# n00b001/neuro-genetic-pong-self-play

Measured on AMD Instinct MI355X. Metric: env-steps/sec (GA evaluation loop, self-play) + generations/sec at pop=65536 per GPU, higher is better.
Workload: dtype f32 hidden + certified f64 argmax; genomes f64

## Files before the change

include/pong_ga.h:

```cpp
#ifndef PONG_GA_H
#define PONG_GA_H

#include <stddef.h>
#include <stdint.h>

#ifdef __cplusplus
extern "C" {
#endif

#define PG_ABI_VERSION 12
#define PG_MAX_NODES 9

typedef enum pg_status {
  PG_OK = 0,
  PG_ERR_INVALID = -1,
  PG_ERR_HIP = -2,
  PG_ERR_UNSUPPORTED = -3
} pg_status;

typedef enum pg_dtype { PG_F32 = 0, PG_F64 = 1 } pg_dtype;

typedef enum pg_opp_kind {
  PG_OPP_HARDCODED = 0,
  PG_OPP_ROM_CPU = 1,
  PG_OPP_SCORE = 2,
  PG_OPP_NN = 3
} pg_opp_kind;

typedef enum pg_precision {
  PG_PREC_CERTIFIED = 0,
  PG_PREC_F64 = 1
} pg_precision;

typedef enum pg_kernel {
  PG_KERNEL_AUTO = 0,
  PG_KERNEL_GENERAL = 1,
  PG_KERNEL_RESIDENT = 2,
  PG_KERNEL_SPLIT = 3      ,
  PG_KERNEL_WIDE = 4,
  PG_KERNEL_STAGED = 5
} pg_kernel;

typedef enum pg_prep {
  PG_PREP_ALL = 0,
  PG_PREP_GENOMES = 1,
  PG_PREP_REST = 2
} pg_prep;

typedef struct pg_net {
  int32_t n_nodes;
  int32_t nodes[PG_MAX_NODES];
  int32_t bias;
  int32_t dtype;
} pg_net;

typedef struct pg_eval_args {
  uint32_t struct_size;
  pg_net net;
  int32_t n_genomes;
  int32_t n_games;
  const void *genomes;
  int64_t genome_stride;
  const void *opponents;
  int64_t opponent_stride;
  int32_t n_opponents;
  int32_t precision;
  const int32_t *game_kind;
  const int32_t *game_opp;
  const double *game_mult;
  uint64_t seed;
  double *fitness;
  double *rewards;
  int32_t *scores;
  int32_t *frames;
  double *total_frames;
  int32_t *status;
  uint64_t *counters;
  uint8_t *trace;
  int32_t trace_games;
  int32_t trace_cap;
  int32_t kernel;
  int32_t group_lanes;
  void *workspace;
  size_t workspace_bytes;
  uint32_t *hard_log;
  int32_t hard_cap;
  const int32_t *genome_rows;
  const int32_t *n_active;
  int32_t prep;
  int32_t horizon;
  int32_t timeout_thresh;
  int32_t win_score;
} pg_eval_args;


typedef struct pg_forward_args {
  pg_net net;
  int32_t n;
  const void *genomes;
  int64_t genome_stride;
  const int32_t *genome_index;
  const double *x;
  int32_t precision;
  int32_t *index;
  double *act;
  uint64_t *counters;
  double *z_all;
  double *h_all;
} pg_forward_args;

typedef struct pg_decide_args {
  pg_net net;
  int32_t n;
  const void *genomes;
  int64_t genome_stride;
  const int32_t *genome_index;
  const int32_t *k;
  int32_t *index;
  int32_t *stage;
} pg_decide_args;

typedef struct pg_wide_decide_args {
  pg_net net;
  int32_t n;
  const void *genomes;
  int64_t genome_stride;
  const int32_t *genome_index;
  const int32_t *k;
  int32_t *index;
  double *act;
  void *workspace;
  size_t workspace_bytes;
} pg_wide_decide_args;

enum {
  PG_S_BALL_X = 0, PG_S_BALL_Y, PG_S_BALL_VX, PG_S_BALL_VY, PG_S_BALL_VISIBLE,
  PG_S_SERVE_TIMER, PG_S_SERVE_DIR, PG_S_HITS, PG_S_POINT, PG_S_LEFT_Y, PG_S_RIGHT_Y,
  PG_S_SCORE1, PG_S_SCORE2, PG_S_ONE_PLAYER, PG_S_SEED_LO, PG_S_SEED_HI,
  PG_STATE_FIELDS
};

typedef struct pg_ga_args {
  int32_t n;
  int64_t genes;
  int32_t dtype;
  const void *parents;
  int64_t stride;
  int32_t n_parents;
  const int32_t *chosen;
  void *offspring;
  uint8_t *invalid;
  double cxpb, mutpb;
  double alpha;
  double mu, sigma, indpb;
  uint64_t seed;
  uint64_t generation;
  const uint8_t *pair_mask;
  const int32_t *pair_list;
  const int32_t *pair_count;
  int32_t pair_cap;
} pg_ga_args;

typedef struct pg_select_args {
  int32_t n_pop;
  int32_t k;
  int32_t tournsize;
  const double *fitness;
  int32_t *chosen;
  uint64_t seed;
  uint64_t generation;
} pg_select_args;

typedef enum pg_schedule_mode {
  PG_SCHED_REFERENCE = 0,
  PG_SCHED_SELFPLAY = 1
} pg_schedule_mode;

typedef struct pg_schedule_args {
  int32_t mode;
  int32_t n;
  int32_t n_games;
  int64_t row_offset;
  int32_t n_hof;
  const double *hof_fitness;
  uint64_t seed;
  uint64_t generation;
  int32_t *kind;
  int32_t *opp;
  double *mult;
  const int32_t *rows;
  int32_t hof_slices;
  int32_t block_rows;
  int32_t slice_local;
} pg_schedule_args;

typedef struct pg_hof_args {
  int32_t maxsize;
  int32_t hof_n;
  const double *hof_fitness;
  const uint64_t *hof_hash;
  int32_t pop_n;
  const double *pop_fitness;
  const uint64_t *pop_hash;
  const int32_t *rank;
  int32_t *new_n;
  int32_t *new_src;
  double *new_fitness;
} pg_hof_args;

typedef struct pg_hof_packed_args {
  int32_t maxsize;
  int32_t hof_n;
  const double *hof_fitness;
  int32_t k;
  const int64_t *packed;
  int32_t *new_n;
  int32_t *new_src;
  double *new_fitness;
  const int32_t *slot_in;
  int32_t *slot_out;
} pg_hof_packed_args;
int32_t pg_hof_update_packed(const pg_hof_packed_args *args);

typedef struct pg_hof_rank_args {
  int32_t hof_n;
  const double *hof_fitness;
  const uint64_t *hof_hash;
  int32_t k;
  const double *cand_fitness;
  const uint64_t *cand_hash;
  int64_t *packed;
  void *workspace;
  size_t workspace_bytes;
} pg_hof_rank_args;

typedef struct pg_hof_prepare_args {
  const double *fitness;
  int32_t pop_n;
  int32_t filter;
  double worst;
  const void *rows;
  int64_t stride;
  int64_t genes;
  int32_t dtype;
  int32_t hof_n;
  const double *hof_fitness;
  const uint64_t *hof_hash;
  int32_t *k;
  int64_t *cand;
  uint64_t *hashes;
  int64_t *packed;
  void *workspace;
  size_t workspace_bytes;
} pg_hof_prepare_args;

const char *pg_version(void);
int32_t pg_abi_version(void);
int32_t pg_build_flags(void);
const char *pg_last_error(void);
int32_t pg_device_count(void);
size_t pg_eval_workspace_bytes(const pg_eval_args *args);
int32_t pg_gene_count(const pg_net *net);

int32_t pg_eval_population(const pg_eval_args *args, void *stream);
int32_t pg_forward(const pg_forward_args *args, void *stream);
int32_t pg_decide(const pg_decide_args *args, void *stream);
size_t pg_wide_decide_workspace_bytes(const pg_wide_decide_args *args);
int32_t pg_wide_decide(const pg_wide_decide_args *args, void *stream);
int32_t pg_physics_reset(int32_t *state, int32_t n, const uint64_t *seeds,
                         const int32_t *one_player, void *stream);
int32_t pg_physics_step(int32_t *state, int32_t n, const uint8_t *actions, void *stream);
int32_t pg_ga_select_tournament(const pg_select_args *args, void *stream);
int32_t pg_ga_select_tournament_ranked(const pg_select_args *args, const double *sorted_fitness,
                                       const int32_t *order, void *stream);
int32_t pg_ga_vary(const pg_ga_args *args, void *stream);
int32_t pg_ga_mark_pairs(uint8_t *pair_mask, int32_t n_pairs, const int32_t *rows, int32_t n_rows,
                         int32_t skip_lo, int32_t skip_hi, const uint8_t *exclude, void *stream);
int32_t pg_ga_list_pairs(const uint8_t *pair_mask, int32_t n_pairs, int32_t *list, int32_t *count, void *stream);
int32_t pg_ga_schedule(const pg_schedule_args *args, void *stream);
int32_t pg_row_hash(const void *rows, int64_t stride, const int32_t *index, int32_t n, int64_t genes,
                    int32_t dtype, uint64_t *hash, void *stream);
int32_t pg_hof_update(const pg_hof_args *args);
size_t pg_hof_rank_classes_workspace_bytes(int32_t n);
int32_t pg_hof_rank_classes(const pg_hof_rank_args *args, void *stream);
size_t pg_hof_prepare_workspace_bytes(int32_t hof_n, int32_t pop_n);
int32_t pg_hof_prepare(const pg_hof_prepare_args *args, void *stream);

typedef struct pg_scatter_args {
  int32_t n;
  int32_t n_games;
  int32_t row_lo;
  const double *fitness;
  const int32_t *frames;
  const int32_t *rows;
  const int32_t *n_active;
  double *shard_fitness;
  float *lineage;
} pg_scatter_args;
int32_t pg_ga_scatter_fitness(const pg_scatter_args *args, void *stream);

typedef struct pg_merge_args {
  int32_t pop_n;
  const double *fitness;
  const uint8_t *invalid;
  const double *inherited;
  double *new_fitness;
  int32_t filter;
  double worst;
  int32_t *cand;
  double *cand_fitness;
  double *summary;
  void *workspace;
  size_t workspace_bytes;
} pg_merge_args;
size_t pg_ga_merge_workspace_bytes(int32_t pop_n);
int32_t pg_ga_merge_fitness(const pg_merge_args *args, void *stream);

size_t pg_ga_select_workspace_bytes(int32_t n_pop);
int32_t pg_ga_select_ranked(const pg_select_args *args, void *workspace, size_t workspace_bytes, void *stream);

int32_t pg_ga_inherit(const int32_t *chosen, int32_t n, const double *fitness, double *inherited,
                      const float *lineage_in, float *lineage_out, void *stream);

size_t pg_ga_order_workspace_bytes(int32_t n);
int32_t pg_ga_order(int32_t n, int32_t row_lo, const uint8_t *invalid, const float *lineage, int32_t by_length,
                    int32_t *rows, int32_t *count, void *workspace, size_t workspace_bytes, void *stream);

typedef struct pg_hof_cand_args {
  int32_t hof_n;
  const double *hof_fitness;
  const uint64_t *hof_hash;
  int32_t k;
  const int32_t *cand;
  const double *cand_fitness;
  const void *rows;
  int64_t stride;
  int64_t genes;
  int32_t dtype;
  uint64_t *cand_hash;
  int64_t *packed;
  void *workspace;
  size_t workspace_bytes;
} pg_hof_cand_args;
size_t pg_hof_prepare_cand_workspace_bytes(int32_t hof_n, int32_t k);
int32_t pg_hof_prepare_cand(const pg_hof_cand_args *args, void *stream);

typedef struct pg_hof_commit_args {
  void *dst;
  int64_t dst_stride;
  const void *old_rows;
  int64_t old_stride;
  const void *rows;
  int64_t rows_stride;
  const int32_t *cand;
  const int32_t *src;
  int32_t n_old;
  int32_t m;
  int64_t genes;
  int32_t dtype;
  const uint64_t *old_hash;
  const uint64_t *cand_hash;
  uint64_t *new_hash;
  const double *fitness_in;
  double *new_fitness;
  const int32_t *dst_slot;
} pg_hof_commit_args;
int32_t pg_hof_commit(const pg_hof_commit_args *args, void *stream);

int32_t pg_gather_rows(void *dst, int64_t dst_stride, const void *old_rows, int64_t old_stride, const void *rows,
                       int64_t rows_stride, const int64_t *index, const int32_t *src, int32_t n_old, int32_t n,
                       int64_t genes, int32_t dtype, void *stream);
int32_t pg_render_frames(const int32_t *state, int32_t n, uint8_t *frames, void *stream);
int32_t pg_find_stuff(const uint8_t *frames, int64_t frame_stride, int32_t n, double *out, void *stream);

#ifdef __cplusplus
}
#endif
#endif
```

neuro-genetic-pong-self-play_amd/csrc/pg_eval.hpp:

```cpp
#pragma once

#include <hip/hip_runtime.h>
#include <stdint.h>

#include "../../include/pong_ga.h"
#include "pg_device.hpp"

namespace pg {

int32_t fail(int32_t code, const char *fmt, ...);

#define PG_HIP(call)                                                                  \
  do {                                                                                \
    hipError_t e_ = (call);                                                           \
    if (e_ != hipSuccess)                                                             \
      return fail(PG_ERR_HIP, "%s failed: %s", #call, hipGetErrorString(e_));        \
  } while (0)

struct EvalParams {
  const void *genomes;
  const void *opponents;
  const int32_t *rows;
  const int32_t *n_active;
  const int32_t *kind;
  const int32_t *opp;
  const double *mult;
  double *rewards;
  int32_t *scores;
  int32_t *frames;
  double *total_frames;
  int32_t *status_game;
  uint64_t *counters;
  uint8_t *trace;
  uint32_t *hard_log;
  int hard_cap;
  unsigned int *work;
  int64_t gstride, ostride;
  uint64_t seed;
  int n_genomes, n_games, total, n_opponents;
  int trace_games, trace_cap;
  int nodes[PG_MAX_NODES];
  int n_nodes, bias, max_width;
  float *recs;
  int horizon;
  int timeout_thresh;
  int win_score;
  int prep;
  void *wide_scratch;
  int wide_w3_resident;
  const int32_t *wide_probe_k;
  int32_t *wide_probe_index;
  double *wide_probe_act;
};

__device__ inline int active_genomes(const EvalParams &p) {
  if (!p.n_active) return p.n_genomes;
  const int a = __builtin_amdgcn_readfirstlane(*p.n_active);
  return a < 0 ? 0 : (a < p.n_genomes ? a : p.n_genomes);
}
__device__ inline int active_total(const EvalParams &p) {
  return p.n_active ? active_genomes(p) * p.n_games : p.total;
}

__device__ inline int genome_row(const EvalParams &p, int i) { return p.rows ? p.rows[i] : i; }

template <class S>
__device__ inline double episode_reward(const S &st, int total, double mult, int &zero_div) {
  zero_div = 0;
  if (st.s1 == st.s2) return 0.0;
  const double tf = (double)total;
  if (tf == 0.0) {
    zero_div = 1;
    return __builtin_nan("");
  }
  const double diff = (double)(st.s2 - st.s1);
  const double bonus = __dmul_rn((double)st.s2, mult);
  return __dadd_rn(diff, bonus) / (tf / 100.0);
}

template <class S>
__device__ inline void finish_game(const EvalParams &p, int w, const S &st, int frames, int total) {
  int zero_div;
  const double reward = episode_reward(st, total, p.mult[w], zero_div);
  p.rewards[w] = reward;
  p.scores[2 * w] = st.s1;
  p.scores[2 * w + 1] = st.s2;
  p.frames[w] = frames;
  p.total_frames[w] = (double)total;
  p.status_game[w] = zero_div;
}

__device__ inline double feat64(int k) { return __dmul_rn(0.5, (double)k) / 160.0; }
__device__ inline double feat64_flip(int k) { return (160.0 - __dmul_rn(0.5, (double)k)) / 160.0; }


int num_cus();

__device__ inline void log_hard_raw(uint32_t *hard_log, uint64_t *counters, int hard_cap, int row, int is_opp, int idx,
                                    int source, const int k[6]) {
  if (!hard_log || !counters) return;
  const unsigned long long r = atomicAdd((unsigned long long *)&counters[9], 1ull);
  if (r >= (unsigned long long)hard_cap) return;
  uint32_t *rec = hard_log + r * 8;
  rec[0] = (uint32_t)row;
  rec[1] = (uint32_t)(is_opp & 1) | ((uint32_t)(idx & 255) << 8) | ((uint32_t)(source & 255) << 16);
  for (int i = 0; i < 6; ++i) rec[2 + i] = (uint32_t)k[i];
}
__device__ inline void log_hard(const EvalParams &p, int row, int is_opp, int idx, int source, const int k[6]) {
  log_hard_raw(p.hard_log, p.counters, p.hard_cap, row, is_opp, idx, source, k);
}

struct DecideParams {
  const void *genomes;
  const int32_t *gidx;
  const int32_t *k;
  int32_t *index;
  int32_t *stage;
  int64_t gstride;
  int n, H, b;
};
int32_t launch_decide(const DecideParams &p, int L, int O, bool f64, size_t lds, hipStream_t s);

bool wide_shape_ok(const pg_net &n, int n_games);
size_t wide_workspace_bytes(const pg_eval_args *a);
int32_t launch_wide(const EvalParams &p, int dtype, void *scratch, hipStream_t s);


}
```

neuro-genetic-pong-self-play_amd/csrc/pg_service.hpp:

```cpp
#pragma once

#include <hip/hip_runtime.h>

#include "../../include/pong_ga.h"
#include "pg_cascade.hpp"
#include "pg_device.hpp"
#include "pg_eval.hpp"
#include "pg_f64math.h"

namespace pg {

#ifndef PG_SVC_PRIO
#define PG_SVC_PRIO 3
#endif
#ifndef PG_SVC_BATCH
#define PG_SVC_BATCH 1
#endif

#ifndef PG_INLINE_SVC
#define PG_INLINE_SVC 1
#endif
#ifndef PG_INLINE_PRIO
#define PG_INLINE_PRIO 3
#endif
#ifndef PG_INLINE_FRAME_BOUND
#define PG_INLINE_FRAME_BOUND 1
#endif
#ifndef PG_HORIZON_INLINE
#define PG_HORIZON_INLINE 1
#endif
template <int L, int U, bool kHorizon>
__host__ __device__ constexpr bool inline_service() {
  return PG_INLINE_SVC && L == 8 && U == 16 && (PG_HORIZON_INLINE || !kHorizon);
}

struct InlineReq {
  int k[6];
  int kr[6];
  float z[4];
  float e;
  const float *rec;
};
template <int U, int HL, int O, typename WT>
__device__ __forceinline__ int serve_inline(const EvalParams &p, const WT *g, InlineReq r, double *lds,
                                                      int lane64, uint64_t *st_acc = nullptr) {
  const int H = p.nodes[1];
  const int b = p.bias;
  float zf[O];
#pragma unroll
  for (int o = 0; o < O; ++o) zf[o] = r.z[o];
#ifdef PG_INLINE_LOG
  float ef_log = -1.f;
  const auto log_req = [&](int stage, int idx) {
    if (p.hard_log && p.counters && lane64 == 0) {
      const unsigned long long q = atomicAdd((unsigned long long *)&p.counters[9], 1ull);
      if (q < (unsigned long long)p.hard_cap) {
        uint32_t *rec = p.hard_log + q * 8;
        for (int o = 0; o < 4; ++o) rec[o] = __float_as_uint(o < O ? zf[o] : 0.f);
        rec[4] = __float_as_uint(r.e);
        rec[5] = __float_as_uint(ef_log);
        rec[6] = (uint32_t)stage | ((uint32_t)(idx & 255) << 8) |
                 ((uint32_t)(blockIdx.x * (blockDim.x >> 6) + (threadIdx.x >> 6)) << 16);
        rec[7] = (uint32_t)((uint64_t)g >> 3);
      }
    }
  };
#define PG_LOG_REQ(stage, idx) log_req(stage, idx)
#else
#define PG_LOG_REQ(stage, idx)
#endif
#ifdef PG_SERVE_STAGES
  asm volatile("s_waitcnt vmcnt(0) lgkmcnt(0)" ::: "memory");
  uint64_t st_t = __builtin_amdgcn_s_memtime();
  const auto stage_mark = [&](int i) {
    asm volatile("s_waitcnt vmcnt(0) lgkmcnt(0)" ::: "memory");
    const uint64_t now = __builtin_amdgcn_s_memtime();
    st_acc[i] += now - st_t;
    st_acc[6 + i] += 1;
    st_t = now;
  };
#define PG_STAGE(i) stage_mark(i)
#else
#define PG_STAGE(i)
#endif
  int d = PG_INLINE_FRAME_BOUND ? -1 : plateau_decide<O>(zf, r.e, lane64);
  PG_STAGE(0);
  if (d >= 0) PG_LOG_REQ(1, d);
  if (PG_INLINE_FRAME_BOUND && d < 0 && r.e < __builtin_inff()) {
    const float ef = fminf(r.e, frame_bound_wave<HL, U, O>(r.rec, r.kr, lane64));
#ifdef PG_INLINE_LOG
    ef_log = ef;
#endif
    PG_STAGE(1);
    d = certify_c<O>(zf, make_cert(ef));
    if (d < 0) d = plateau_f32<O>(zf, ef);
    if (d < 0) d = plateau_decide<O>(zf, ef, lane64);
    PG_STAGE(2);
    if (d >= 0) {
      PG_LOG_REQ(2, d);
      return d | 1024;
    }
  }
  if (d < 0) {
    d = fast_f64_decide<O, WT>(g, H, b, r.k, lane64);
    PG_STAGE(3);
    if (d >= 0) PG_LOG_REQ(3, d);
  }
  if (d >= 0) return d | 512;
  d = forward_f64_group<64, (U * HL + 63) / 64, O, WT>(g, H, b, r.k, lds, lane64);
  PG_LOG_REQ(4, d);
  PG_STAGE(4);
#undef PG_LOG_REQ
#undef PG_STAGE
#if defined(PG_INLINE_LOG) || defined(PG_SERVE_STAGES)
  if (false) {
#else
  if (p.hard_log && lane64 == 0) {
#endif
    const long oo = g - (const WT *)p.opponents;
    const bool opp = p.opponents != p.genomes && oo >= 0 && oo < (long)p.n_opponents * p.ostride;
    log_hard(p, (int)(opp ? oo / p.ostride : (g - (const WT *)p.genomes) / p.gstride), opp ? 1 : 0, d, 0, r.k);
  }
  return d | 256;
}

template <int L, int U, int O, typename WT>
__global__ __launch_bounds__(256) void k_prep_records(EvalParams p) {
  constexpr int HL = L / 2;
  constexpr int F = rec_floats<U, O>();
  if (p.prep != PG_PREP_GENOMES && blockIdx.x == 0) {
    if (threadIdx.x < 64) p.work[threadIdx.x] = 0u;
    if (p.counters && threadIdx.x < 16) p.counters[threadIdx.x] = 0ull;
  }
  const long t = (long)blockIdx.x * 256 + threadIdx.x;
  const long net = t / HL + (p.prep == PG_PREP_REST ? p.n_genomes : 0);
  const int hl = (int)(t % HL);
  const long end = p.prep == PG_PREP_GENOMES ? (long)p.n_genomes : (long)p.n_genomes + p.n_opponents;
  if (net >= end) return;
  const WT *g;
  int flip;
  if (net < p.n_genomes) {
    if (net >= active_genomes(p)) return;
    g = (const WT *)p.genomes + (long)genome_row(p, (int)net) * p.gstride;
    flip = 0;
  } else {
    g = (const WT *)p.opponents + (net - p.n_genomes) * p.ostride;
    flip = 1;
  }
  NetP<U, O> n;
  load_net_pk<HL, U, O, WT>(n, g, p.nodes[1], p.bias, hl, flip);
  store_rec<U, O>(n, p.recs + (net * HL + hl) * F);
}

#ifdef PG_PROBE_EXTRA
template <int M>
__device__ __forceinline__ void pg_probe_extra(float2v w, float2v w2, float a, float b, float &v, float2v &pp,
                                               int &sv) {
#pragma unroll
  for (int r = 0; r < (M == 4 || M == 9 ? 48 : (M <= 2 ? 16 : 24)); ++r) {
    if constexpr (M == 1) asm volatile("v_rcp_f32 %0, %1" : "=v"(v) : "v"((r & 1) ? a : b));
    if constexpr (M == 2) asm volatile("v_exp_f32 %0, %1" : "=v"(v) : "v"((r & 1) ? a : b));
    if constexpr (M == 3) asm volatile("v_pk_fma_f32 %0, %1, %2, %3" : "=v"(pp) : "v"(w), "v"(w2), "v"((r & 1) ? w : w2));
    if constexpr (M == 4) asm volatile("v_fma_f32 %0, %1, %2, %3" : "=v"(v) : "v"(a), "v"(b), "v"((r & 1) ? a : b));
    if constexpr (M == 5) asm volatile("v_add_u32 %0, %1, %2" : "=v"(v) : "v"(a), "v"(b));
    if constexpr (M == 7) asm volatile("v_mov_b32 %0, %1" : "=v"(v) : "v"((r & 1) ? a : b));
    if constexpr (M == 8) asm volatile("v_pk_add_f32 %0, %1, %2" : "=v"(pp) : "v"(w), "v"((r & 1) ? w : w2));
    if constexpr (M == 9) asm volatile("v_add_f32 %0, %1, %2" : "=v"(v) : "v"(a), "v"((r & 1) ? a : b));
  }
}
#endif

template <int L, int U, int O, typename WT, bool kUntraced = false, bool kHorizon = false>
__global__ __launch_bounds__(svc_threads<U>()) void k_service(EvalParams p) {
  constexpr int kSvcThreads = svc_threads<U>();
  constexpr bool kInline = inline_service<L, U, kHorizon>();
  static_assert(!kInline || O <= 4, "InlineReq.z");
  constexpr int kSvcGameWaves = kSvcThreads / 64 - (kInline ? 0 : 1);
  constexpr int HL = L / 2;
  constexpr int kSlots = kSvcGameWaves * (64 / L) * 2;
  __shared__ SlowSlot slots[kSlots];
  __shared__ HorizonSlot hz[kHorizon ? kSlots / 2 : 1];
  __shared__ int waves_done;
  __shared__ int posted;
  __shared__ uint32_t serve_tab[kServeTabSlots * kServeTabPoints];
  extern __shared__ double lds_svc[];
  const int H = p.nodes[1];
  const int b = p.bias;
  const int wave = threadIdx.x >> 6;
  const int lane64 = threadIdx.x & 63;
  for (int i = threadIdx.x; i < kSlots; i += kSvcThreads) {
    lds_st(&slots[i].flag, 0);
    slots[i].rec = 0;
  }
  const bool tabbed = p.n_games <= kServeTabSlots;
  if (tabbed)
    for (int i = threadIdx.x; i < p.n_games * kServeTabPoints; i += kSvcThreads)
      serve_tab[i] = Pong::serve_entry(game_seed(p.seed, i / kServeTabPoints), i % kServeTabPoints);
  if (threadIdx.x == 0) {
    lds_st(&waves_done, 0);
    lds_st(&posted, 0);
  }
  __syncthreads();

  if (!kInline && wave == kSvcGameWaves) {
    if constexpr (PG_SVC_PRIO > 0) __builtin_amdgcn_s_setprio(PG_SVC_PRIO);
    constexpr int kSvcBatch = U * HL <= 64 ? PG_SVC_BATCH : 1;
    const WT *genomes_svc = (const WT *)p.genomes;
    int seen = 0;
    for (;;) {
      const int now = __builtin_amdgcn_readfirstlane(lds_ld(&posted));
      if (now == seen) {
        if (lds_ld(&waves_done) == kSvcGameWaves) break;
        __builtin_amdgcn_s_sleep(2);
        continue;
      }
      seen = now;
      for (int base = 0; base < kSlots; base += 64) {
        const int sidx = base + lane64;
        const bool posted = sidx < kSlots && lds_ld(&slots[sidx].flag) == 1;
        unsigned long long mask = __ballot(posted);
        while (mask) {
          int sl[kSvcBatch], idx[kSvcBatch], k[kSvcBatch][6];
          const WT *g[kSvcBatch];
          bool need[kSvcBatch];
#pragma unroll
          for (int q = 0; q < kSvcBatch; ++q) {
            sl[q] = -1;
            if (mask) {
              sl[q] = base + __builtin_ctzll(mask);
              mask &= mask - 1;
            }
          }
          __threadfence_block();
#pragma unroll
          for (int q = 0; q < kSvcBatch; ++q) {
            need[q] = false;
            idx[q] = -1;
            g[q] = genomes_svc;
            if (sl[q] >= 0) {
              g[q] = (const WT *)slots[sl[q]].g;
#pragma unroll
              for (int i = 0; i < 6; ++i) k[q][i] = slots[sl[q]].k[i];
              float zf[O];
#pragma unroll
              for (int o = 0; o < O; ++o) zf[o] = slots[sl[q]].z[o];
              idx[q] = plateau_decide<O>(zf, slots[sl[q]].e, lane64);
              need[q] = idx[q] < 0;
            }
          }
          if constexpr (kSvcBatch > 1) {
            int f[kSvcBatch];
            fast_f64_decide_batch<O, WT, kSvcBatch>(g, k, need, H, b, lane64, f);
#pragma unroll
            for (int q = 0; q < kSvcBatch; ++q)
              if (need[q]) idx[q] = f[q];
          } else {
            if (need[0]) idx[0] = fast_f64_decide<O, WT>(g[0], H, b, k[0], lane64);
          }
#pragma unroll
          for (int q = 0; q < kSvcBatch; ++q) {
            if (sl[q] < 0) continue;
            int d = idx[q];
            if (d < 0) {
              d = forward_f64_group<64, (U * HL + 63) / 64, O, WT>(g[q], H, b, k[q], lds_svc, lane64);
              if (p.hard_log && lane64 == 0) {
                const long oo = g[q] - (const WT *)p.opponents;
                const bool opp = p.opponents != p.genomes && oo >= 0 && oo < (long)p.n_opponents * p.ostride;
                log_hard(p, (int)(opp ? oo / p.ostride : (g[q] - (const WT *)p.genomes) / p.gstride), opp ? 1 : 0,
                         d, 0, k[q]);
              }
              d |= 256;
            } else {
              d |= 512;
            }
            if (lane64 == 0) {
              slots[sl[q]].idx = d;
              __threadfence_block();
              lds_st(&slots[sl[q]].flag, 2);
            }
          }
        }
      }
    }
    return;
  }

  const int lig = threadIdx.x & (L - 1);
  const int side = lig >= HL ? 1 : 0;
  const int hl = lig & (HL - 1);
  const int leader = lane64 & ~(L - 1);
  const int wave_slot0 = __builtin_amdgcn_readfirstlane((int)(threadIdx.x >> 6)) * (64 / L) * 2;
  const auto slot_grp = [&]() { return wave_slot0 + (fresh_lane64() / L) * 2; };
  const auto slot_me = [&]() {
    const int l = fresh_lane64();
    return wave_slot0 + (l / L) * 2 + ((l & (L - 1)) >= HL ? 1 : 0);
  };
  const WT *genomes = (const WT *)p.genomes;
  const WT *opponents = (const WT *)p.opponents;

  NetP<U, O> net;
  PongK st;
  int kind = 0, act_r = 0, act_l = 0, total = 0, fstart = 0, tend = 0, c_vis = 0, tab_off = 0;
  int sframe = 0;
#ifndef PG_NO_HIDDEN_JUMP
  constexpr bool kVisByFrames = kUntraced && !kHorizon;
#else
  constexpr bool kVisByFrames = false;
#endif
  const WT *gm = genomes;
  uint32_t slow = 0, c_fwd = 0, c_steps = 0, c_games = 0, fails = 0, plateau = 0, inwave = 0, skipped = 0, hidden = 0;

  const int games_total = active_total(p);
  int w;
  {
    int ww = 0;
    if (lig == 0) ww = (int)atomicAdd(p.work, 1u);
    w = group_broadcast<L>(ww, leader);
  }
  bool fresh = true;
  bool live = w < games_total;
  const auto park = [&]() {
    st.bx2 = 2 * 79 + kBallW - 1;
    st.by2 = 2 * 78 + kBallH - 1;
    st.vx2 = st.vy2 = 0;
    st.vis = 2;
    st.one_player = 0;
    kind = kOppNN;
    tend = 0x7fffffff;
    fstart = 0x3fffffff;
    fresh = false;
  };
  if (kInline && !live) park();
  int w_scripted = 1, w_onep = 1;
  int top = 1;
#ifdef PG_PROBE_EXTRA
  float probe_v = 0.f;
  float2v probe_p = float2v{0.f, 0.f};
  int probe_s = 0;
#endif
#ifdef PG_START_PROBE
  uint64_t probe_fresh = 0;
  const uint64_t probe_t0 = __builtin_amdgcn_s_memtime();
#endif
#ifdef PG_SERVE_STAGES
  uint64_t st_acc[24];
#pragma unroll
  for (int i = 0; i < 24; ++i) st_acc[i] = 0;
#endif
#ifdef PG_DECIDE_PROBE
  uint64_t probe_dec = 0;
  const uint64_t probe_t0 = __builtin_amdgcn_s_memtime();
#endif
#ifdef PG_TIMELINE
  uint64_t t_start = 0;
  uint32_t g_fails = 0, g_slow = 0;
#endif
#ifdef PG_PATH_PROBE
  uint32_t pp_frames = 0, pp_rally = 0, pp_face = 0, pp_fail = 0, pp_hidden = 0;
#define PG_PP(cnt, cond) \
  if (__builtin_amdgcn_ballot_w64(cond) != 0) cnt += 1
#else
#define PG_PP(cnt, cond)
#endif
  if (kInline ? __builtin_amdgcn_ballot_w64(live) != 0 : live) for (;;) {
#ifdef PG_START_PROBE
    const bool any_fresh = __builtin_amdgcn_ballot_w64(fresh) != 0;
    const uint64_t probe_f0 = __builtin_amdgcn_s_memtime();
#endif
    PG_PP(pp_frames, true);
    sframe += 1;
#ifdef PG_TIMELINE
    constexpr bool kJumps = !kHorizon;
#else
    const bool kJumps = !kHorizon && (kUntraced || p.trace == nullptr);
#endif
    if (top) {
    if (fresh) {
      const int i = w / p.n_games;
      const int g = w - i * p.n_games;
      kind = p.kind[w];
      const WT *gr = genomes + (long)genome_row(p, i) * p.gstride;
      const bool nn = side && kind == kOppNN && p.n_opponents > 0;
      const int oj = nn ? min(max(p.opp[w], 0), p.n_opponents - 1) : 0;
      gm = nn ? opponents + (long)oj * p.ostride : gr;
      const int rec = nn ? p.n_genomes + oj : i;
      load_rec<U, O>(net, p.recs + ((long)rec * HL + hl) * rec_floats<U, O>());
      const int sx = slot_me();
      if (kInline && hl == 0) slots[sx].rec = rec;
#pragma unroll
      for (int o = 0; o < O; ++o) net.c[o] = hl == 0 ? 0.5f * net.c[o] : 0.f;
      st.reset(0, kind == kOppRomCpu);
      if (kHorizon || !tabbed) st.seed = game_seed(p.seed, g);
      tab_off = g * kServeTabPoints;
      act_r = act_l = total = 0;
      c_vis = kVisByFrames ? sframe - 1 : 0;
      fstart = sframe - 1;
      tend = sframe + p.timeout_thresh;
      fresh = false;
      if (hl == 0) slots[sx].n_memo = 0;
      if (lig == 0) slots[sx].rally_at = -1;
      if (kHorizon && lig == 0) {
        const int gx = threadIdx.x / L;
        hz[gx].sum = 0.0;
        hz[gx].eps = hz[gx].s1 = hz[gx].s2 = hz[gx].zd = 0;
      }
#ifdef PG_TIMELINE
      t_start = wall_clock64();
      g_fails = g_slow = 0;
#endif
    }
#ifdef PG_START_PROBE
    if (any_fresh) probe_fresh += __builtin_amdgcn_s_memtime() - probe_f0;
#endif
#ifndef PG_NO_HIDDEN_JUMP
    {
      const bool hid = !st.vis && st.timer >= 2;
      PG_PP(pp_hidden, hid);
      if (kJumps && hid) {
        const int h = st.timer - 1;
        st.rc2 = PongK::drift2(st.rc2, h);
        if (!st.one_player) st.lc2 = PongK::drift2(st.lc2, h);
        st.timer = 1;
        act_r = clamp_move(st.rc2, 0);
        act_l = clamp_move(st.lc2, 0);
        fstart -= h;
        tend -= h;
        hidden += h;
      }
    }
#endif
    w_scripted = __builtin_amdgcn_readfirstlane(__builtin_amdgcn_ballot_w64(kind != kOppNN) != 0);
    w_onep = __builtin_amdgcn_readfirstlane(__builtin_amdgcn_ballot_w64(st.one_player != 0) != 0);
    top = 0;
    }
    const int pvis = st.vis, pbx2 = st.bx2, pby2 = st.by2;
#ifdef PG_PATH_PROBE
    const int pt_b = st.point, hits_b = st.hits;
#endif
    const int ev = st.step(act_r, act_l, [&](int pt) {
      return tabbed && pt < kServeTabPoints ? serve_tab[tab_off + pt] : Pong::serve_entry(st.seed, pt);
    }, w_onep != 0);
    PG_PP(pp_face, ev != kStepFly || st.hits != hits_b || st.point != pt_b);
    const int vis = st.vis;
    const int bx2 = st.bx2, by2 = st.by2;
    const int rc2 = st.rc2;
    int lc2 = st.lc2;
    if (__builtin_expect(w_onep, 0)) lc2 = PongK::c2_clip(st.lc2);
    int left, right;
    {
      const int lbx2 = pvis ? pbx2 : bx2, lby2 = pvis ? pby2 : by2;
      const int k[6] = {bx2, by2, lbx2, lby2, rc2, lc2};
      float acc[O], z[O];
      partial_pk<U, O, true>(net, k, acc);
#pragma unroll
      for (int o = 0; o < O; ++o) z[o] = group_sum<HL>(acc[o]);
      int code = certify_c8<O>(z, net.ct);
#ifdef PG_PROBE_EXTRA
      pg_probe_extra<PG_PROBE_EXTRA>(net.w1[0][0], net.w1[1][1], z[0], z[1], probe_v, probe_p, probe_s);
#endif
      const bool left_nn = kind == kOppNN;
      if (side && !left_nn) code = 0;
      if (vis != 1) code = 0;
#ifdef PG_ABLATE_SLOW
      if (code == -1) code = z[1] > z[0] ? 6 : -6;
#endif
      PG_PP(pp_fail, code == -1);
      if (PG_ANY(code == -1)) {
      if (code == -1) {
        fails += 1;
#ifdef PG_TIMELINE
        g_fails += 1;
#endif
#ifndef PG_NO_TIGHT
        int mv = tight_gap_move<O>(z, net.e, net.ct);
        if (mv == -1)
#else
        int mv = -1;
#endif
        {
          const int idx = plateau_f32<O>(z, net.e);
          mv = idx >= 0 ? index_to_move(idx) : -1;
        }
        inwave += mv != -1 ? 1 : 0;
        code = mv;
      }
#ifdef PG_ABLATE_SERVE
      if (code == -1) code = z[1] > z[0] ? 6 : -6;
#endif
      if (kInline && PG_ANY(code == -1)) {
        uint64_t key = 0;
        int nm = 0;
        const int sx = slot_me();
        if (code == -1) {
          key = memo_key(k);
          nm = slots[sx].n_memo;
          int hit = -1;
#pragma unroll 1
          for (int c = 0; c < kMemo && c < nm; ++c)
            if (slots[sx].memo_key[c] == key) hit = slots[sx].memo_idx[c];
          code = hit;
        }
        const int kn[6] = {side ? 320 - bx2 : bx2, by2, side ? 320 - lbx2 : lbx2, lby2, side ? lc2 : rc2,
                           side ? rc2 : lc2};
        const float my_e = net.e;
        uint64_t need = __builtin_amdgcn_ballot_w64(code == -1 && hl == 0);
        if (need) {
#ifdef PG_DECIDE_PROBE
        const uint64_t probe_d0 = __builtin_amdgcn_s_memtime();
#endif
        if constexpr (PG_INLINE_PRIO > 0) __builtin_amdgcn_s_setprio(PG_INLINE_PRIO);
#pragma unroll 1
        do {
          const int src = (int)__builtin_ctzll(need);
          need &= need - 1;
          InlineReq r;
#pragma unroll
          for (int i = 0; i < 6; ++i) r.k[i] = __builtin_amdgcn_readlane(kn[i], src);
#pragma unroll
          for (int i = 0; i < 6; ++i) r.kr[i] = __builtin_amdgcn_readlane(k[i], src);
          r.rec = p.recs + (long)__builtin_amdgcn_readlane(slots[sx].rec, src) * HL * rec_floats<U, O>();
#pragma unroll
          for (int o = O; o < 4; ++o) r.z[o] = 0.f;
#pragma unroll
          for (int o = 0; o < O; ++o) r.z[o] = __int_as_float(__builtin_amdgcn_readlane(__float_as_int(z[o]), src));
          r.e = __int_as_float(__builtin_amdgcn_readlane(__float_as_int(my_e), src));
          const uint64_t ga = (uint64_t)gm;
          const WT *g = (const WT *)(((uint64_t)__builtin_amdgcn_readlane((int)(ga >> 32), src) << 32) |
                                     (uint32_t)__builtin_amdgcn_readlane((int)(uint32_t)ga, src));
#if defined(PG_SERVE_TWICE)
          serve_inline<U, HL, O, WT>(p, g, r, lds_svc + wave * f64_lds_doubles(H, O), lane64, st_acc);
          const int ans = serve_inline<U, HL, O, WT>(p, g, r, lds_svc + wave * f64_lds_doubles(H, O), lane64, st_acc + 12);
#elif defined(PG_SERVE_STAGES)
          const int ans = serve_inline<U, HL, O, WT>(p, g, r, lds_svc + wave * f64_lds_doubles(H, O), lane64, st_acc);
#else
          const int ans = serve_inline<U, HL, O, WT>(p, g, r, lds_svc + wave * f64_lds_doubles(H, O), lane64);
#endif
          if ((lane64 & ~(HL - 1)) == src) {
            slow += (ans >> 8) & 1;
// ... 146 lines not shown
    over = over || sframe > tend;
#endif
    if constexpr (kHorizon) {
      if (over) {
        const int gx = threadIdx.x / L;
        const bool ep_end = st.s1 >= p.win_score || st.s2 >= p.win_score || st.done() || sframe > tend;
        if (lig == 0) {
          if (ep_end) {
            int zd;
            hz[gx].sum = __dadd_rn(hz[gx].sum, episode_reward(st, total, p.mult[w], zd));
            hz[gx].zd |= zd;
            hz[gx].eps += 1;
          }
          hz[gx].s1 += st.s1;
          hz[gx].s2 += st.s2;
        }
        if (ep_end && sframe - fstart < p.horizon) {
          const int pt = st.point;
          st.reset(st.seed, st.one_player);
          st.point = pt;
          act_r = act_l = total = 0;
          tend = sframe + 1 + p.timeout_thresh;
          over = false;
        }
      }
    }
    if (over) {
      if constexpr (kHorizon) {
        if (lig == 0) {
          const int gx = threadIdx.x / L;
          p.rewards[w] = hz[gx].sum;
          p.scores[2 * w] = hz[gx].s1;
          p.scores[2 * w + 1] = hz[gx].s2;
          p.frames[w] = sframe - fstart;
          p.total_frames[w] = (double)hz[gx].eps;
          p.status_game[w] = hz[gx].zd;
        }
      } else {
        if (lig == 0) finish_game(p, w, st, sframe - fstart, total);
      }
#ifdef PG_TIMELINE
      if (p.trace && w < p.trace_games && lig == 0) {
        uint32_t *tl = (uint32_t *)(p.trace + (long)w * p.trace_cap);
        tl[0] = (uint32_t)t_start;
        tl[1] = (uint32_t)wall_clock64();
        tl[2] = g_fails;
        tl[3] = g_slow;
        if (p.trace_cap >= 24) {
          tl[4] = blockIdx.x;
          tl[5] = (uint32_t)wave;
        }
      }
#endif
      c_steps += sframe - fstart;
      const int vis_frames = kVisByFrames ? sframe - c_vis - (st.s1 + st.s2) : c_vis;
      c_fwd += (kind == kOppNN ? 2u : 1u) * (uint32_t)vis_frames;
      c_games += 1;
      int ww = 0;
      if (lig == 0) ww = (int)atomicAdd(p.work, 1u);
      w = group_broadcast<L>(ww, leader);
      if constexpr (kInline) {
        if (w >= games_total) {
          live = false;
          park();
        } else {
          fresh = true;
        }
      } else {
        if (w >= games_total) break;
        fresh = true;
      }
    }
    if constexpr (kInline) {
      if (__builtin_amdgcn_ballot_w64(live) == 0) break;
    }
    top = __builtin_amdgcn_readfirstlane(__builtin_amdgcn_ballot_w64(fresh || (kJumps && !st.vis && st.timer >= 2)) != 0);
    }
  }
  if (p.counters && c_games) {
    if (lig == 0) {
      atomicAdd((unsigned long long *)&p.counters[0], (unsigned long long)(c_steps - skipped - hidden));
      if (hidden) atomicAdd((unsigned long long *)&p.counters[12], (unsigned long long)hidden);
      atomicAdd((unsigned long long *)&p.counters[1], (unsigned long long)c_fwd);
      atomicAdd((unsigned long long *)&p.counters[3], (unsigned long long)c_games);
      if (skipped) atomicAdd((unsigned long long *)&p.counters[8], (unsigned long long)skipped);
    }
    if (hl == 0 && slow) atomicAdd((unsigned long long *)&p.counters[2], (unsigned long long)slow);
    if (hl == 0 && fails) atomicAdd((unsigned long long *)&p.counters[4], (unsigned long long)fails);
    if (hl == 0 && plateau) atomicAdd((unsigned long long *)&p.counters[5], (unsigned long long)plateau);
    if (hl == 0 && inwave) atomicAdd((unsigned long long *)&p.counters[6], (unsigned long long)inwave);
  }
#ifdef PG_DECIDE_PROBE
  if (p.counters && lane64 == 0) {
    atomicAdd((unsigned long long *)&p.counters[13], (unsigned long long)probe_dec);
    atomicAdd((unsigned long long *)&p.counters[14], (unsigned long long)(__builtin_amdgcn_s_memtime() - probe_t0));
    atomicAdd((unsigned long long *)&p.counters[15], 1ull);
  }
#endif
#ifdef PG_START_PROBE
  if (p.counters && lane64 == 0) {
    atomicAdd((unsigned long long *)&p.counters[13], (unsigned long long)probe_fresh);
    atomicAdd((unsigned long long *)&p.counters[14], (unsigned long long)(__builtin_amdgcn_s_memtime() - probe_t0));
    atomicAdd((unsigned long long *)&p.counters[15], 1ull);
  }
#endif
#ifdef PG_PATH_PROBE
  if (p.counters && lane64 == 0) {
    atomicAdd((unsigned long long *)&p.counters[11], (unsigned long long)pp_frames);
    atomicAdd((unsigned long long *)&p.counters[10], (unsigned long long)pp_rally);
    atomicAdd((unsigned long long *)&p.counters[13], (unsigned long long)pp_face);
    atomicAdd((unsigned long long *)&p.counters[14], (unsigned long long)pp_fail);
    atomicAdd((unsigned long long *)&p.counters[15], (unsigned long long)pp_hidden);
  }
#endif
#ifdef PG_PROBE_EXTRA
  if (p.counters && probe_v == 1234.5f && probe_p.x == 1234.5f && probe_s == 1234567) p.counters[15] = 1;
#endif
#ifdef PG_SERVE_STAGES
  if (p.hard_log && lane64 == 0)
#pragma unroll
    for (int i = 0; i < 24; ++i)
      if (st_acc[i]) atomicAdd((unsigned long long *)&((uint64_t *)p.hard_log)[i], (unsigned long long)st_acc[i]);
#endif
  if (lane64 == 0) atomicAdd(&waves_done, 1);
}

inline size_t service_records_bytes(int n_genomes, int n_opponents, int L, int U, int O) {
  const int F = ((U + 1) / 2 * 2 * (7 + O) + O + 1 + 3) / 4 * 4;
  return ((size_t)n_genomes + (size_t)(n_opponents > 0 ? n_opponents : 0)) * (size_t)(L / 2) * F * sizeof(float);
}

template <int L, int U, int O, typename WT, bool kSplitTrace = false>
inline int32_t launch_service(const EvalParams &p, hipStream_t s) {
  constexpr int kSvcThreads = svc_threads<U>();
  const bool inl = p.horizon > 0 ? inline_service<L, U, true>() : inline_service<L, U, false>();
  const int GPB = (kSvcThreads / 64 - (inl ? 0 : 1)) * (64 / L);
  const size_t lds = (size_t)f64_lds_doubles(p.nodes[1], O) * sizeof(double) * (inl ? kSvcThreads / 64 : 1);
  const int want = (p.total + GPB - 1) / GPB;
  const int cap = num_cus() * 2;
  const int grid = want < cap ? want : cap;
  if (grid <= 0) return PG_OK;
  if (!p.recs) return fail(PG_ERR_INVALID, "split kernel: no lane-record workspace");
  if (!kSplitTrace && p.horizon > 0)
    return fail(PG_ERR_UNSUPPORTED, "horizon mode: [6, 33..64, 3] networks on 8-lane groups only");
  const long nets = p.prep == PG_PREP_GENOMES ? (long)p.n_genomes
                   : (p.prep == PG_PREP_REST ? (long)p.n_opponents : (long)p.n_genomes + p.n_opponents);
  const long prep_threads = nets * (L / 2);
  const unsigned prep_blocks = (unsigned)((prep_threads + 255) / 256);
  hipLaunchKernelGGL((k_prep_records<L, U, O, WT>), dim3(prep_blocks > 0 ? prep_blocks : 1u), dim3(256), 0, s, p);
  if (p.prep == PG_PREP_GENOMES) {
    PG_HIP(hipGetLastError());
    return PG_OK;
  }
  if (kSplitTrace && p.horizon > 0)
    hipLaunchKernelGGL((k_service<L, U, O, WT, true, true>), dim3(grid), dim3(kSvcThreads), lds, s, p);
  else if (kSplitTrace && !p.trace)
    hipLaunchKernelGGL((k_service<L, U, O, WT, true>), dim3(grid), dim3(kSvcThreads), lds, s, p);
  else
    hipLaunchKernelGGL((k_service<L, U, O, WT, false>), dim3(grid), dim3(kSvcThreads), lds, s, p);
  PG_HIP(hipGetLastError());
  return PG_OK;
}

int32_t launch_service_more(const EvalParams &p, int L, int O, bool f64, hipStream_t s);

inline int service_units(int L, int H) {
  if (L == 8 && H > 32 && H <= 64) return 16;
  for (int u = 1; u <= 8; u *= 2)
    if ((L / 2) * u >= H) return u;
  return 0;
}

}
```

neuro-genetic-pong-self-play_amd/csrc/pong_ga.hip:

```cpp
#include <hip/hip_runtime.h>

#include <cmath>
#include <cstdarg>
#include <cstdio>
#include <cstring>
#include <string>
#include <algorithm>
#include <memory>
#include <unordered_map>
#include <utility>
#include <vector>

#include "../../include/pong_ga.h"
#include "pg_device.hpp"
#include "pg_eval.hpp"
#include "pg_f64math.h"
#include "pg_cascade.hpp"
#include "pg_service.hpp"

#ifndef PG_VERSION_STRING
#define PG_VERSION_STRING "pong_ga 0.1.0 (gfx950)"
#endif

namespace pg {
// ... 159 lines not shown
template <typename WT>
__global__ __launch_bounds__(64) void k_forward_general(FwdParams p) {
  extern __shared__ double lds[];
  const int lane = threadIdx.x;
  const int W = p.max_width + 1;
  const int n_in = p.nodes[0], n_out = p.nodes[p.n_nodes - 1];
  for (int t = blockIdx.x; t < p.n; t += gridDim.x) {
    const long row = p.gidx ? p.gidx[t] : t;
    const WT *gw = (const WT *)p.genomes + row * p.gstride;
    double *cur = lds, *nxt = lds + W;
    for (int i = lane; i < n_in; i += 64) cur[i] = p.x[(long)t * n_in + i];
    if (p.bias && lane == 0) cur[n_in] = 1.0;
    wave_lds_sync();
    const int idx = forward_f64_wave(gw, p.nodes, p.n_nodes, p.bias, cur, nxt, lane,
                                     p.z_all ? p.z_all + (long)t * p.n_units : nullptr,
                                     p.h_all ? p.h_all + (long)t * p.n_units : nullptr);
    if (lane == 0) p.index[t] = idx;
    if (p.act)
      for (int j = lane; j < n_out; j += 64) p.act[(long)t * n_out + j] = cur[j];
    wave_lds_sync();
  }
}

template <int L, int U, int O, typename WT>
__global__ __launch_bounds__(256) void k_forward_resident(FwdParams p) {
  constexpr int GPB = 256 / L;
  const int H = p.nodes[1], b = p.bias;
  extern __shared__ double lds_all[];
  const int lig = threadIdx.x & (L - 1);
  const int grp = threadIdx.x / L;
  double *lds = lds_all + grp * f64_lds_doubles(H, O);
  uint32_t slow = 0;
  for (int t = blockIdx.x * GPB + grp; t < p.n; t += gridDim.x * GPB) {
    const long row = p.gidx ? p.gidx[t] : t;
    const WT *gw = (const WT *)p.genomes + row * p.gstride;
    Net<U, O> net;
    load_net<L, U, O, WT>(net, gw, H, b, lig);
    float x[6], acc[O], z[O];
#pragma unroll
    for (int i = 0; i < 6; ++i) x[i] = (float)p.x[(long)t * 6 + i];
    partial_f32<U, O>(net, x, acc);
#pragma unroll
    for (int o = 0; o < O; ++o) z[o] = group_sum<L>(acc[o]) + net.c[o];
    int idx = certify<O>(z, net.e);
    if (idx >= 0 && p.act) {
      bool tight = true;
#pragma unroll
      for (int o = 0; o < O; ++o) {
        const float tt = fmaxf(fabsf(z[o]) - net.e, 0.f);
        const float sp = __expf(-tt) / ((1.f + __expf(-tt)) * (1.f + __expf(-tt)));
        tight = tight && (net.e * sp <= 2e-6f);
      }
      if (!tight) idx = -1;
    }
    if (idx < 0) {
      double xd[6];
#pragma unroll
      for (int i = 0; i < 6; ++i) xd[i] = p.x[(long)t * 6 + i];
      idx = forward_f64_group<L, U, O, WT>(gw, H, b, (const double *)xd, lds, lig);
      if (p.act && lig < O) p.act[(long)t * O + lig] = lds[f64_out_offset(H, O) + lig];
      wave_lds_sync();
      slow += (lig == 0);
    } else if (p.act && lig < O) {
      float zz = z[0];
#pragma unroll
      for (int o = 1; o < O; ++o) zz = (lig == o) ? z[o] : zz;
      p.act[(long)t * O + lig] = sigmoid_f64((double)zz);
    }
    if (lig == 0) p.index[t] = idx;
  }
  if (p.counters && slow) atomicAdd((unsigned long long *)&p.counters[2], (unsigned long long)slow);
}

__global__ void k_physics_reset(int32_t *s, int n, const uint64_t *seeds, const int32_t *one_player) {
  const int i = blockIdx.x * blockDim.x + threadIdx.x;
  if (i >= n) return;
  Pong st;
  st.reset(seeds ? seeds[i] : 0ull, one_player ? one_player[i] : 0);
  const int f[PG_STATE_FIELDS] = {st.bx, st.by, st.vx, st.vy, st.vis, st.timer, st.dir, st.hits,
                                  st.point, st.lpy, st.rpy, st.s1, st.s2, st.one_player,
                                  (int)(uint32_t)st.seed, (int)(uint32_t)(st.seed >> 32)};
#pragma unroll
  for (int k = 0; k < PG_STATE_FIELDS; ++k) s[(long)k * n + i] = f[k];
}

__global__ void k_physics_step(int32_t *s, int n, const uint8_t *actions) {
  const int i = blockIdx.x * blockDim.x + threadIdx.x;
  if (i >= n) return;
  Pong st;
  st.bx = s[0L * n + i]; st.by = s[1L * n + i]; st.vx = s[2L * n + i]; st.vy = s[3L * n + i];
  st.vis = s[4L * n + i]; st.timer = s[5L * n + i]; st.dir = s[6L * n + i]; st.hits = s[7L * n + i];
  st.point = s[8L * n + i]; st.lpy = s[9L * n + i]; st.rpy = s[10L * n + i];
  st.s1 = s[11L * n + i]; st.s2 = s[12L * n + i]; st.one_player = s[13L * n + i];
  st.seed = (uint64_t)(uint32_t)s[14L * n + i] | ((uint64_t)(uint32_t)s[15L * n + i] << 32);
  const int a = actions[i];
  st.step(a & 3, (a >> 2) & 3);
  s[0L * n + i] = st.bx; s[1L * n + i] = st.by; s[2L * n + i] = st.vx; s[3L * n + i] = st.vy;
  s[4L * n + i] = st.vis; s[5L * n + i] = st.timer; s[6L * n + i] = st.dir; s[7L * n + i] = st.hits;
  s[8L * n + i] = st.point; s[9L * n + i] = st.lpy; s[10L * n + i] = st.rpy;
  s[11L * n + i] = st.s1; s[12L * n + i] = st.s2;
}

__device__ __forceinline__ double u01(uint64_t seed, uint64_t gen, uint64_t stream, uint64_t a,
                                      uint64_t b) {
  uint64_t k = splitmix64(seed + 0x9E3779B97F4A7C15ull * (gen + 1));
  k = splitmix64(k ^ (stream * 0xD6E8FEB86659FD93ull + a));
  k = splitmix64(k ^ b);
  return (double)(k >> 11) * 0x1.0p-53;
}

__global__ void k_select(pg_select_args a) {
  const int j = blockIdx.x * blockDim.x + threadIdx.x;
  if (j >= a.k) return;
  int best = -1;
  double bf = 0.0;
  for (int t = 0; t < a.tournsize; ++t) {
    const int idx = (int)(u01(a.seed, a.generation, 1, (uint64_t)j, (uint64_t)t) * (double)a.n_pop);
    const double f = a.fitness[idx];
    if (best < 0 || f > bf) {
      best = idx;
      bf = f;
    }
  }
  a.chosen[j] = best;
}

__global__ void k_select_ranked(pg_select_args a, const double *sorted, const int32_t *order) {
  const int j = blockIdx.x * blockDim.x + threadIdx.x;
  if (j >= a.k) return;
  const int n = a.n_pop;
  const double v = u01(a.seed, a.generation, 8, (uint64_t)j, 0);
  int r = (int)((double)n * exp(log(v) / (double)a.tournsize));
  r = r < 0 ? 0 : (r > n - 1 ? n - 1 : r);
  const double f = sorted[r];
  int lo = 0, hi = n;
  int a0 = 0, b0 = r;
  while (a0 < b0) { const int m = (a0 + b0) >> 1; if (sorted[m] < f) a0 = m + 1; else b0 = m; }
  lo = a0;
  a0 = r; b0 = n;
  while (a0 < b0) { const int m = (a0 + b0) >> 1; if (sorted[m] <= f) a0 = m + 1; else b0 = m; }
  hi = a0;
  const int pick = lo + (int)(u01(a.seed, a.generation, 9, (uint64_t)j, 0) * (double)(hi - lo));
  a.chosen[j] = order[pick < hi ? pick : hi - 1];
}

__device__ __forceinline__ uint64_t rng_key(uint64_t seed, uint64_t gen, uint64_t stream, uint64_t a) {
  const uint64_t k = splitmix64(seed + 0x9E3779B97F4A7C15ull * (gen + 1));
  return splitmix64(k ^ (stream * 0xD6E8FEB86659FD93ull + a));
}
__device__ __forceinline__ double rng_u01(uint64_t key, uint64_t b) {
  return (double)(splitmix64(key ^ b) >> 11) * 0x1.0p-53;
}

template <typename WT>
__device__ __forceinline__ void vary_pair(const pg_ga_args &a, int pair);

template <typename WT>
__global__ __launch_bounds__(256) void k_vary(pg_ga_args a) {
  const int wave = (int)blockIdx.x * 4 + __builtin_amdgcn_readfirstlane((int)(threadIdx.x >> 6));
  if (a.pair_list) {
    const int count = __builtin_amdgcn_readfirstlane(*a.pair_count);
    const int waves = (int)gridDim.x * 4;
#pragma unroll 1
    for (int w = wave; w < count; w += waves) vary_pair<WT>(a, __builtin_amdgcn_readfirstlane(a.pair_list[w]));
    return;
  }
  vary_pair<WT>(a, wave);
}

template <typename WT>
__device__ __forceinline__ void vary_pair(const pg_ga_args &a, int pair) {
  const int pairs = (a.n + 1) / 2;
  if (pair >= pairs) return;
  const int lane = threadIdx.x & 63;
  const int i0 = 2 * pair, i1 = 2 * pair + 1;
  const bool has1 = i1 < a.n;
  const bool cx = has1 && rng_u01(rng_key(a.seed, a.generation, 2, (uint64_t)pair), 0) < a.cxpb;
  const bool mut0 = rng_u01(rng_key(a.seed, a.generation, 4, (uint64_t)i0), 0) < a.mutpb;
  const bool mut1 = has1 && rng_u01(rng_key(a.seed, a.generation, 4, (uint64_t)i1), 0) < a.mutpb;
  if (lane == 0) {
    a.invalid[i0] = (uint8_t)(cx || mut0);
    if (has1) a.invalid[i1] = (uint8_t)(cx || mut1);
  }
  if (!a.pair_list && a.pair_mask && !a.pair_mask[pair]) return;
  const uint64_t k3 = rng_key(a.seed, a.generation, 3, (uint64_t)pair);
  const uint64_t k5 = rng_key(a.seed, a.generation, 5, (uint64_t)pair);
  const uint64_t k6 = rng_key(a.seed, a.generation, 6, (uint64_t)pair);
  const WT *p1 = (const WT *)a.parents + (long)a.chosen[i0] * a.stride;
  const WT *p2 = (const WT *)a.parents + (long)(has1 ? a.chosen[i1] : a.chosen[i0]) * a.stride;
  WT *o1 = (WT *)a.offspring + (long)i0 * a.stride;
  WT *o2 = (WT *)a.offspring + (long)i1 * a.stride;
  const auto one = [&](long gene, double x1, double x2) {
    if (cx) {
      const double u = rng_u01(k3, (uint64_t)gene);
      const double gamma = __dadd_rn(__dmul_rn(1.0 + 2.0 * a.alpha, u), -a.alpha);
      const double y1 = __dadd_rn(__dmul_rn(1.0 - gamma, x1), __dmul_rn(gamma, x2));
      const double y2 = __dadd_rn(__dmul_rn(gamma, x1), __dmul_rn(1.0 - gamma, x2));
      x1 = y1;
      x2 = y2;
    }
    const uint64_t hb = splitmix64(k5 ^ (uint64_t)gene);
    const bool h0 = mut0 && (double)(uint32_t)hb * 0x1.0p-32 < a.indpb;
    const bool h1 = mut1 && (double)(uint32_t)(hb >> 32) * 0x1.0p-32 < a.indpb;
    if (h0 || h1) {
      const uint64_t nb = splitmix64(k6 ^ (uint64_t)gene);
      const float u1 = 1.0f - (float)(nb >> 40) * 0x1.0p-24f;
      const float u2 = (float)((nb >> 8) & 0xFFFFFFu) * 0x1.0p-24f;
      const float r = sqrtf(-2.0f * logf(u1));
      float sn, cs;
      sincosf(6.2831853f * u2, &sn, &cs);
      if (h0) x1 = __dadd_rn(x1, __dadd_rn(a.mu, __dmul_rn(a.sigma, (double)(r * cs))));
      if (h1) x2 = __dadd_rn(x2, __dadd_rn(a.mu, __dmul_rn(a.sigma, (double)(r * sn))));
    }
    o1[gene] = (WT)x1;
    if (has1) o2[gene] = (WT)x2;
  };
  constexpr int kVaryChunk = 4;
  for (long g0 = 0; g0 < a.genes; g0 += 128 * kVaryChunk) {
    double x[kVaryChunk][2][2];
#pragma unroll
    for (int c = 0; c < kVaryChunk; ++c) {
#pragma unroll
      for (int h = 0; h < 2; ++h) {
        const long g = g0 + c * 128 + h * 64 + lane;
        const bool v = g < a.genes;
        x[c][h][0] = v ? (double)p1[g] : 0.0;
        x[c][h][1] = v && has1 ? (double)p2[g] : 0.0;
      }
    }
#pragma unroll
    for (int c = 0; c < kVaryChunk; ++c) {
#pragma unroll
      for (int h = 0; h < 2; ++h) {
        const long g = g0 + c * 128 + h * 64 + lane;
        if (g < a.genes) one(g, x[c][h][0], x[c][h][1]);
      }
    }
  }
}

__global__ void k_mark_pairs(uint8_t *mask, int n_pairs, const int32_t *rows, int n_rows, int skip_lo, int skip_hi,
                             const uint8_t *exclude) {
  const int i = blockIdx.x * blockDim.x + threadIdx.x;
  if (i >= n_rows) return;
  const int r = rows[i];
  if (r < 0 || r >= 2 * n_pairs) return;
  const int j = r >> 1;
  if ((j < skip_lo || j >= skip_hi) && !(exclude && exclude[j])) mask[j] = 1;
}

__global__ void k_list_pairs(const uint8_t *mask, int n_pairs, int32_t *list, int32_t *count) {
  const int j = blockIdx.x * blockDim.x + threadIdx.x;
  if (j < n_pairs && mask[j]) list[atomicAdd(count, 1)] = j;
}

__global__ void k_schedule(pg_schedule_args a) {
  const long w = (long)blockIdx.x * blockDim.x + threadIdx.x;
  if (w >= (long)a.n * a.n_games) return;
  const long i = w / a.n_games;
  const int g = (int)(w % a.n_games);
  const long row = a.rows ? (long)a.rows[i] : a.row_offset + i;
  int kind = kOppHard, opp = 0;
  double mult = 1.0;
  if (a.mode == PG_SCHED_SELFPLAY) {
    if (a.n_hof > 0) {
      kind = kOppNN;
      const int K = a.hof_slices > 1 && a.n_hof >= a.hof_slices ? a.hof_slices : 1;
      if (K == 1) {
        opp = (int)((row * a.n_games + g) % a.n_hof);
      } else {
        const int b = (int)((row / a.block_rows) % K);
        const long m = (a.n_hof - b + K - 1) / K;
        const int k = (int)((row * a.n_games + g) % m);
        opp = a.slice_local ? k : k * K + b;
      }
    }
  } else if (g < 3) {
    kind = g == 0 ? kOppHard : (g == 1 ? kOppRomCpu : kOppScore);
  } else if (a.n_hof > 0) {
    kind = kOppNN;
    opp = (int)(u01(a.seed, a.generation, 10, (uint64_t)row, (uint64_t)g) * (double)a.n_hof);
    opp = opp < a.n_hof ? opp : a.n_hof - 1;
    mult = a.hof_fitness[opp];
  }
  a.kind[w] = kind;
  a.opp[w] = opp;
  a.mult[w] = mult;
}

template <typename WT>
__global__ __launch_bounds__(256) void k_gather_rows(WT *dst, int64_t dst_stride, const WT *old_rows, int64_t old_stride,
                                                     const WT *rows, int64_t rows_stride, const int64_t *index,
                                                     const int32_t *src, int n_old, int64_t genes) {
  const int j = blockIdx.x;
  const int s = src[j];
  const WT *from = s < n_old ? old_rows + (long)s * old_stride
                             : rows + (index ? index[s - n_old] : (long)(s - n_old)) * rows_stride;
  WT *to = dst + (long)j * dst_stride;
  for (int64_t g = threadIdx.x; g < genes; g += 256) to[g] = from[g];
}

template <typename WT>
__global__ __launch_bounds__(256) void k_row_hash(const WT *rows, int64_t stride, const int32_t *index, int n,
                                                  int64_t genes, uint64_t *out) {
  __shared__ uint64_t part[4];
  const int r = blockIdx.x;
  if (r >= n) return;
  const WT *row = rows + (long)(index ? index[r] : r) * stride;
  uint64_t h = 0;
  for (int64_t j = threadIdx.x; j < genes; j += 256) {
    uint64_t bits;
    if constexpr (sizeof(WT) == 8) {
      const double v = row[j];
      bits = v == 0.0 ? 0ull : (uint64_t)__double_as_longlong(v);
    } else {
      const float v = row[j];
      bits = v == 0.0f ? 0ull : (uint64_t)__float_as_uint(v);
    }
    h += splitmix64(bits ^ ((uint64_t)j * 0x9E3779B97F4A7C15ull));
  }
  for (int off = 32; off > 0; off >>= 1) h += __shfl_xor(h, off, 64);
  if ((threadIdx.x & 63) == 0) part[threadIdx.x >> 6] = h;
  __syncthreads();
  if (threadIdx.x == 0) out[r] = splitmix64(part[0] + part[1] + part[2] + part[3] + (uint64_t)genes);
}

static int gene_count(const pg_net &n) {
  const int b = n.bias ? 1 : 0;
  long t = 0;
  for (int i = 0; i + 1 < n.n_nodes; ++i) t += (long)(n.nodes[i] + b) * n.nodes[i + 1];
  return t > 0x7fffffff ? -1 : (int)t;
}

static int32_t check_net(const pg_net &n, bool game) {
  if (n.n_nodes < 2 || n.n_nodes > PG_MAX_NODES)
    return fail(PG_ERR_INVALID, "net.n_nodes=%d must be in [2, %d]", n.n_nodes, PG_MAX_NODES);
  for (int i = 0; i < n.n_nodes; ++i)
    if (n.nodes[i] < 1 || n.nodes[i] > 65536)
      return fail(PG_ERR_INVALID, "net.nodes[%d]=%d out of range", i, n.nodes[i]);
  if (game && n.nodes[0] != 6)
    return fail(PG_ERR_INVALID, "the game feeds 6 inputs (utils.py:146-152); nodes[0]=%d", n.nodes[0]);
  if (n.dtype != PG_F32 && n.dtype != PG_F64) return fail(PG_ERR_INVALID, "net.dtype=%d", n.dtype);
  if (gene_count(n) < 0) return fail(PG_ERR_INVALID, "network too large");
  return PG_OK;
}

static int max_width(const pg_net &n) {
  int m = 0;
  for (int i = 0; i < n.n_nodes; ++i) m = n.nodes[i] > m ? n.nodes[i] : m;
  return m;
}

static int g_num_cus = 0;
int num_cus() {
  if (g_num_cus == 0) {
    int dev = 0;
    hipDeviceProp_t prop;
    if (hipGetDevice(&dev) == hipSuccess && hipGetDeviceProperties(&prop, dev) == hipSuccess)
      g_num_cus = prop.multiProcessorCount;
    if (g_num_cus <= 0) g_num_cus = 256;
  }
  return g_num_cus;
}

struct ResidentChoice {
  int L, U;
};
static ResidentChoice choose_resident(int H, int requested_L) {
  static const ResidentChoice table[] = {{4, 1}, {8, 1}, {16, 1}, {32, 1}, {16, 4}, {32, 4}, {64, 4}};
  static const ResidentChoice all[] = {{4, 1}, {8, 1}, {16, 1}, {32, 1}, {64, 1}, {16, 2}, {32, 2},
                                       {64, 2}, {16, 4}, {32, 4}, {64, 4}};
  if (requested_L > 0) {
    for (const auto &c : all)
      if (c.L == requested_L && c.L * c.U >= H) return c;
    return {0, 0};
  }
  for (const auto &c : table)
    if (c.L * c.U >= H) return c;
  return {0, 0};
}


static int choose_split_lanes(int H) {
  if (H <= 64) return 8;
  if (H <= 128) return 32;
  return 64;
}

template <typename WT>
static int32_t launch_service_any(const EvalParams &p, int L, int O, hipStream_t s) {
  const int H = p.nodes[1];
#ifdef PG_DEV_MIN
  const bool here = L == 8 && H <= 64;
#else
  const bool here = L == 8 && H > 32 && H <= 64;
#endif
  if (here && O == 3) return launch_service<8, 16, 3, WT, true>(p, s);
#ifdef PG_DEV_MIN
  return fail(PG_ERR_UNSUPPORTED, "no service kernel for L=%d H=%d O=%d", L, H, O);
#else
  return launch_service_more(p, L, O, sizeof(WT) == 8, s);
#endif
}


template <int L, int U, int O, typename WT>
static int32_t launch_fwd_resident(const FwdParams &p, hipStream_t s) {
  constexpr int GPB = 256 / L;
  const size_t lds = (size_t)GPB * f64_lds_doubles(p.nodes[1], O) * sizeof(double);
  const int want = (p.n + GPB - 1) / GPB;
  const int cap = num_cus() * 8;
  const int grid = want < cap ? want : cap;
  if (grid <= 0) return PG_OK;
  hipLaunchKernelGGL((k_forward_resident<L, U, O, WT>), dim3(grid), dim3(256), lds, s, p);
  PG_HIP(hipGetLastError());
  return PG_OK;
}

template <typename WT>
static int32_t launch_fwd_resident_any(const FwdParams &p, ResidentChoice c, int O, hipStream_t s) {
#define PG_FRES(LL, UU)                                                  \
  if (c.L == LL && c.U == UU) {                                          \
    if (O == 2) return launch_fwd_resident<LL, UU, 2, WT>(p, s);         \
    if (O == 3) return launch_fwd_resident<LL, UU, 3, WT>(p, s);         \
    if (O == 4) return launch_fwd_resident<LL, UU, 4, WT>(p, s);         \
  }
#ifndef PG_DEV_MIN
  PG_FRES(4, 1) PG_FRES(8, 1) PG_FRES(16, 1) PG_FRES(32, 1) PG_FRES(64, 1)
  PG_FRES(16, 2) PG_FRES(32, 2) PG_FRES(64, 2) PG_FRES(16, 4) PG_FRES(32, 4) PG_FRES(64, 4)
#endif
#undef PG_FRES
  return fail(PG_ERR_UNSUPPORTED, "no resident forward kernel for L=%d U=%d O=%d", c.L, c.U, O);
}

static bool resident_shape_ok(const pg_net &n) {
  return n.n_nodes == 3 && n.nodes[0] == 6 && n.nodes[1] <= 256 && n.nodes[2] >= 2 && n.nodes[2] <= 4;
}

}

using namespace pg;

extern "C" {

const char *pg_version(void) { return PG_VERSION_STRING; }
int32_t pg_abi_version(void) { return PG_ABI_VERSION; }
int32_t pg_build_flags(void) { return 0; }
const char *pg_last_error(void) { return g_last_error.c_str(); }

int32_t pg_device_count(void) {
  int n = 0;
  hipError_t e = hipGetDeviceCount(&n);
  if (e != hipSuccess) return fail(PG_ERR_HIP, "hipGetDeviceCount: %s", hipGetErrorString(e));
  return n;
}

static size_t eval_base_workspace(const pg_eval_args *a) {
  const size_t games = a ? (size_t)(a->n_genomes > 0 ? a->n_genomes : 0) * (size_t)(a->n_games > 0 ? a->n_games : 0) : 0;
  return 256 + ((games * sizeof(int32_t) + 255) / 256) * 256;
}

static int resolve_kernel(const pg_eval_args *a) {
  if (a->kernel != PG_KERNEL_AUTO) return a->kernel;
  if (resident_shape_ok(a->net) && a->precision == PG_PREC_CERTIFIED) return PG_KERNEL_SPLIT;
  if (wide_shape_ok(a->net, a->n_games) && (a->net.nodes[1] >= 64 || a->net.nodes[2] >= 64)) return PG_KERNEL_WIDE;
  return PG_KERNEL_GENERAL;
}

static size_t split_records_bytes(const pg_eval_args *a) {
  if (!resident_shape_ok(a->net) || a->n_genomes <= 0) return 0;
  const int H = a->net.nodes[1];
  const int L = a->group_lanes > 0 ? a->group_lanes : choose_split_lanes(H);
  const int U = (L == 8 && H <= 64) ? 16 : service_units(L, H);
  if (U <= 0) return 0;
  return (service_records_bytes(a->n_genomes, a->opponents ? a->n_opponents : 0, L, U, a->net.nodes[2]) + 255) /
         256 * 256;
}

static int32_t check_struct_size(const pg_eval_args *a) {
  if (a->struct_size != sizeof(pg_eval_args))
    return fail(PG_ERR_INVALID, "pg_eval_args.struct_size=%u, this library's struct is %zu bytes (ABI %d)",
                a->struct_size, sizeof(pg_eval_args), PG_ABI_VERSION);
  return PG_OK;
}

size_t pg_eval_workspace_bytes(const pg_eval_args *a) {
  if (a && check_struct_size(a) != PG_OK) return 0;
  size_t n = eval_base_workspace(a);
  if (!a) return n;
  const int kernel = resolve_kernel(a);
  if (kernel == PG_KERNEL_SPLIT) n += split_records_bytes(a);
  if (kernel == PG_KERNEL_WIDE && wide_shape_ok(a->net, a->n_games)) n += (wide_workspace_bytes(a) + 255) / 256 * 256;
  return n;
}

int32_t pg_gene_count(const pg_net *net) {
  if (!net) return fail(PG_ERR_INVALID, "net is NULL");
  int32_t rc = check_net(*net, false);
  if (rc != PG_OK) return rc;
  return gene_count(*net);
}

int32_t pg_eval_population(const pg_eval_args *a, void *stream) {
  if (!a) return fail(PG_ERR_INVALID, "args is NULL");
  int32_t rc = check_struct_size(a);
  if (rc != PG_OK) return rc;
  rc = check_net(a->net, true);
  if (rc != PG_OK) return rc;
  if (a->n_genomes < 0) return fail(PG_ERR_INVALID, "n_genomes=%d < 0", a->n_genomes);
  if (a->n_games < 1 || a->n_games > 64) return fail(PG_ERR_INVALID, "n_games=%d not in [1, 64]", a->n_games);
  if (a->horizon < 0) return fail(PG_ERR_INVALID, "horizon=%d < 0", a->horizon);
  if (a->timeout_thresh != 0 && (a->timeout_thresh < 32 || a->timeout_thresh > (1 << 20)))
    return fail(PG_ERR_INVALID, "timeout_thresh=%d not 0 or in [32, 1048576]", a->timeout_thresh);
  if (a->win_score < 0) return fail(PG_ERR_INVALID, "win_score=%d < 0", a->win_score);
  if (a->n_genomes == 0) {
    if (a->counters) PG_HIP(hipMemsetAsync(a->counters, 0, 16 * sizeof(uint64_t), (hipStream_t)stream));
    return PG_OK;
  }
  const long total = (long)a->n_genomes * a->n_games;
  if (total > 0x7fffffffL) return fail(PG_ERR_INVALID, "too many games (%ld)", total);
  const int G = gene_count(a->net);
  if (!a->genomes || a->genome_stride < G)
    return fail(PG_ERR_INVALID, "genomes NULL or genome_stride=%lld < gene count %d", (long long)a->genome_stride, G);
  if (!a->game_kind || !a->game_opp || !a->game_mult || !a->fitness || !a->rewards || !a->scores ||
      !a->frames || !a->total_frames || !a->status)
    return fail(PG_ERR_INVALID, "a required per-game array is NULL");
  if (a->n_opponents > 0 && (!a->opponents || a->opponent_stride < G))
    return fail(PG_ERR_INVALID, "opponents NULL or opponent_stride < gene count");
  if (a->precision != PG_PREC_CERTIFIED && a->precision != PG_PREC_F64)
    return fail(PG_ERR_INVALID, "precision=%d", a->precision);
  if (a->trace && (a->trace_games < 0 || a->trace_cap < 1))
    return fail(PG_ERR_INVALID, "trace needs trace_games >= 0 and trace_cap >= 1");
  if (a->prep < PG_PREP_ALL || a->prep > PG_PREP_REST) return fail(PG_ERR_INVALID, "prep=%d", a->prep);
  if (a->horizon > 0 && a->trace) return fail(PG_ERR_INVALID, "horizon mode runs untraced (trace must be NULL)");
  if (a->horizon > 0 && resolve_kernel(a) != PG_KERNEL_SPLIT)
    return fail(PG_ERR_UNSUPPORTED, "horizon mode runs on the SPLIT kernel ([6, H<=64, 3], certified)");
  const size_t need = pg_eval_workspace_bytes(a);
  if (!a->workspace || a->workspace_bytes < need)
    return fail(PG_ERR_INVALID, "workspace of %zu bytes required (got %zu)", need, a->workspace_bytes);

  hipStream_t s = (hipStream_t)stream;
  EvalParams p;
  memset(&p, 0, sizeof(p));
  p.genomes = a->genomes;
  p.opponents = a->opponents ? a->opponents : a->genomes;
  p.kind = a->game_kind;
  p.opp = a->game_opp;
  p.mult = a->game_mult;
  p.rewards = a->rewards;
  p.scores = a->scores;
  p.frames = a->frames;
  p.total_frames = a->total_frames;
  p.counters = a->counters;
  p.trace = a->trace;
  p.trace_games = a->trace ? a->trace_games : 0;
  p.trace_cap = a->trace_cap;
  p.hard_log = a->hard_cap > 0 ? a->hard_log : nullptr;
  p.hard_cap = a->hard_cap;
  p.work = (unsigned int *)a->workspace;
  p.status_game = (int32_t *)((char *)a->workspace + 256);
  p.gstride = a->genome_stride;
  p.ostride = a->opponent_stride;
  p.n_opponents = a->opponents ? a->n_opponents : 0;
  p.rows = a->genome_rows;
  p.n_active = a->n_active;
  p.seed = a->seed;
  p.n_genomes = a->n_genomes;
  p.n_games = a->n_games;
  p.total = (int)total;
  for (int i = 0; i < a->net.n_nodes; ++i) p.nodes[i] = a->net.nodes[i];
  p.n_nodes = a->net.n_nodes;
  p.bias = a->net.bias ? 1 : 0;
  p.max_width = max_width(a->net);

  p.prep = a->prep;
  p.horizon = a->horizon;
  p.timeout_thresh = a->timeout_thresh > 0 ? a->timeout_thresh : kTimeoutThresh;
  p.win_score = a->win_score > 0 ? (a->win_score < kDoneScore ? a->win_score : kDoneScore) : kWinScore;
  const int kernel = resolve_kernel(a);
  if (kernel != PG_KERNEL_SPLIT) {
    if (a->prep == PG_PREP_GENOMES) return PG_OK;
    p.prep = PG_PREP_ALL;
    PG_HIP(hipMemsetAsync(a->workspace, 0, 256, s));
    if (a->counters) PG_HIP(hipMemsetAsync(a->counters, 0, 16 * sizeof(uint64_t), s));
  }
  const bool res_ok = resident_shape_ok(a->net);
  const bool wide_ok = wide_shape_ok(a->net, a->n_games);
  if (kernel == PG_KERNEL_WIDE) {
    if (!wide_ok)
      return fail(PG_ERR_UNSUPPORTED, "wide kernel needs NETWORK_SHAPE [6, H1<=512, H2<=512, 1..4] and n_games <= 8");
    rc = launch_wide(p, a->net.dtype, (char *)a->workspace + eval_base_workspace(a), s);
    if (rc != PG_OK) return rc;
  } else if (kernel == PG_KERNEL_SPLIT) {
    if (!res_ok) return fail(PG_ERR_UNSUPPORTED, "split kernel needs NETWORK_SHAPE [6, H<=256, 2..4]");
    if (a->precision != PG_PREC_CERTIFIED) return fail(PG_ERR_UNSUPPORTED, "split kernel is the certified-precision path");
    const int H = a->net.nodes[1];
    const int L = a->group_lanes > 0 ? a->group_lanes : choose_split_lanes(H);
    p.recs = (float *)((char *)a->workspace + eval_base_workspace(a));
    rc = a->net.dtype == PG_F64 ? launch_service_any<double>(p, L, a->net.nodes[2], s)
                                : launch_service_any<float>(p, L, a->net.nodes[2], s);
    if (rc != PG_OK) return rc;
    if (a->prep == PG_PREP_GENOMES) return PG_OK;
  } else if (kernel == PG_KERNEL_RESIDENT || kernel == PG_KERNEL_STAGED) {
    return fail(PG_ERR_UNSUPPORTED, "the %s kernel was retired (DESIGN 4.1b-c); use SPLIT",
                kernel == PG_KERNEL_RESIDENT ? "resident" : "staged");
  } else if (kernel == PG_KERNEL_GENERAL) {
    const size_t lds = 2 * (size_t)(p.max_width + 1) * sizeof(double);
    if (lds > 160 * 1024) return fail(PG_ERR_UNSUPPORTED, "layer width %d too large for LDS", p.max_width);
    const int cap = num_cus() * 16;
    const int grid = total < cap ? (int)total : cap;
    if (a->net.dtype == PG_F64)
      hipLaunchKernelGGL(k_general<double>, dim3(grid), dim3(64), lds, s, p);
    else
      hipLaunchKernelGGL(k_general<float>, dim3(grid), dim3(64), lds, s, p);
    PG_HIP(hipGetLastError());
  } else {
    return fail(PG_ERR_INVALID, "kernel=%d", a->kernel);
  }
  hipLaunchKernelGGL(k_fitness, dim3((a->n_genomes + 255) / 256), dim3(256), 0, s, a->rewards,
                     p.status_game, a->n_genomes, a->n_active, a->n_games, a->fitness, a->status);
  PG_HIP(hipGetLastError());
  return PG_OK;
}

int32_t pg_forward(const pg_forward_args *a, void *stream) {
  if (!a) return fail(PG_ERR_INVALID, "args is NULL");
  int32_t rc = check_net(a->net, false);
  if (rc != PG_OK) return rc;
  if (a->n < 0) return fail(PG_ERR_INVALID, "n=%d < 0", a->n);
  if (a->n == 0) return PG_OK;
  const int G = gene_count(a->net);
  if (!a->genomes || a->genome_stride < G || !a->x || !a->index)
    return fail(PG_ERR_INVALID, "genomes/x/index NULL or genome_stride < gene count %d", G);
  hipStream_t s = (hipStream_t)stream;
  FwdParams p;
  memset(&p, 0, sizeof(p));
  p.genomes = a->genomes;
  p.gidx = a->genome_index;
  p.x = a->x;
  p.index = a->index;
  p.act = a->act;
  p.z_all = a->z_all;
  p.h_all = a->h_all;
  p.counters = a->counters;
  p.gstride = a->genome_stride;
  p.n = a->n;
  for (int i = 0; i < a->net.n_nodes; ++i) p.nodes[i] = a->net.nodes[i];
  for (int i = 1; i < a->net.n_nodes; ++i) p.n_units += a->net.nodes[i];
  if ((a->z_all || a->h_all) && a->precision != PG_PREC_F64)
    return fail(PG_ERR_INVALID, "z_all/h_all need precision PG_PREC_F64");
  p.n_nodes = a->net.n_nodes;
  p.bias = a->net.bias ? 1 : 0;
  p.max_width = max_width(a->net);
  if (a->precision == PG_PREC_CERTIFIED && resident_shape_ok(a->net)) {
    const ResidentChoice c = choose_resident(a->net.nodes[1], 0);
    return a->net.dtype == PG_F64 ? launch_fwd_resident_any<double>(p, c, a->net.nodes[2], s)
                                  : launch_fwd_resident_any<float>(p, c, a->net.nodes[2], s);
  }
  if (a->precision != PG_PREC_CERTIFIED && a->precision != PG_PREC_F64)
    return fail(PG_ERR_INVALID, "precision=%d", a->precision);
  const size_t lds = 2 * (size_t)(p.max_width + 1) * sizeof(double);
  if (lds > 160 * 1024) return fail(PG_ERR_UNSUPPORTED, "layer width %d too large for LDS", p.max_width);
  const int cap = num_cus() * 16;
  const int grid = a->n < cap ? a->n : cap;
  if (a->net.dtype == PG_F64)
    hipLaunchKernelGGL(k_forward_general<double>, dim3(grid), dim3(64), lds, s, p);
  else
    hipLaunchKernelGGL(k_forward_general<float>, dim3(grid), dim3(64), lds, s, p);
  PG_HIP(hipGetLastError());
  return PG_OK;
}

int32_t pg_decide(const pg_decide_args *a, void *stream) {
  if (!a) return fail(PG_ERR_INVALID, "args is NULL");
  int32_t rc = check_net(a->net, false);
  if (rc != PG_OK) return rc;
  if (!resident_shape_ok(a->net)) return fail(PG_ERR_UNSUPPORTED, "pg_decide: the split kernel's shapes only");
  if (a->n < 0) return fail(PG_ERR_INVALID, "n=%d < 0", a->n);
  if (a->n == 0) return PG_OK;
  const int G = gene_count(a->net);
  if (!a->genomes || a->genome_stride < G || !a->k || !a->index)
    return fail(PG_ERR_INVALID, "genomes/k/index NULL or genome_stride < gene count %d", G);
  DecideParams p;
  memset(&p, 0, sizeof(p));
  p.genomes = a->genomes;
  p.gidx = a->genome_index;
  p.k = a->k;
  p.index = a->index;
  p.stage = a->stage;
  p.gstride = a->genome_stride;
  p.n = a->n;
  p.H = a->net.nodes[1];
  p.b = a->net.bias ? 1 : 0;
  const int H = p.H, O = a->net.nodes[2];
  const int L = choose_split_lanes(H);
  const size_t lds = (size_t)f64_lds_doubles(H, O) * sizeof(double);
  return launch_decide(p, L, O, a->net.dtype == PG_F64, lds, (hipStream_t)stream);
}

static pg_eval_args wide_decide_eval(const pg_wide_decide_args *a) {
  pg_eval_args e;
  memset(&e, 0, sizeof(e));
  e.struct_size = sizeof(e);
  e.net = a->net;
  e.n_genomes = a->n;
  e.n_games = 1;
  return e;
}

size_t pg_wide_decide_workspace_bytes(const pg_wide_decide_args *a) {
  if (!a || a->n <= 0 || !wide_shape_ok(a->net, 1)) return 256;
  const pg_eval_args e = wide_decide_eval(a);
  return 256 + (wide_workspace_bytes(&e) + 255) / 256 * 256;
}

int32_t pg_wide_decide(const pg_wide_decide_args *a, void *stream) {
  if (!a) return fail(PG_ERR_INVALID, "args is NULL");
  int32_t rc = check_net(a->net, false);
  if (rc != PG_OK) return rc;
  if (!wide_shape_ok(a->net, 1))
    return fail(PG_ERR_UNSUPPORTED, "pg_wide_decide: the wide kernel's shapes [6, H1<=512, H2<=512, 1..4] only");
  if (a->n < 0) return fail(PG_ERR_INVALID, "n=%d < 0", a->n);
  if (a->n == 0) return PG_OK;
  const int G = gene_count(a->net);
  if (!a->genomes || a->genome_stride < G || !a->k || !a->index)
    return fail(PG_ERR_INVALID, "genomes/k/index NULL or genome_stride < gene count %d", G);
  const size_t need = pg_wide_decide_workspace_bytes(a);
  if (!a->workspace || a->workspace_bytes < need)
    return fail(PG_ERR_INVALID, "workspace of %zu bytes required (got %zu)", need, a->workspace_bytes);
  hipStream_t s = (hipStream_t)stream;
  EvalParams p;
  memset(&p, 0, sizeof(p));
  p.genomes = a->genomes;
  p.opponents = a->genomes;
  p.rows = a->genome_index;
  p.work = (unsigned int *)a->workspace;
  p.gstride = a->genome_stride;
  p.ostride = a->genome_stride;
  p.n_genomes = a->n;
  p.n_games = 1;
  p.total = a->n;
  for (int i = 0; i < a->net.n_nodes; ++i) p.nodes[i] = a->net.nodes[i];
  p.n_nodes = a->net.n_nodes;
  p.bias = a->net.bias ? 1 : 0;
  p.max_width = max_width(a->net);
  p.wide_probe_k = a->k;
  p.wide_probe_index = a->index;
  p.wide_probe_act = a->act;
  PG_HIP(hipMemsetAsync(a->workspace, 0, 256, s));
  return launch_wide(p, a->net.dtype, (char *)a->workspace + 256, s);
}

int32_t pg_physics_reset(int32_t *state, int32_t n, const uint64_t *seeds, const int32_t *one_player,
                         void *stream) {
  if (n < 0 || (n > 0 && !state)) return fail(PG_ERR_INVALID, "state NULL or n < 0");
  if (n == 0) return PG_OK;
  hipLaunchKernelGGL(k_physics_reset, dim3((n + 255) / 256), dim3(256), 0, (hipStream_t)stream, state, n,
                     seeds, one_player);
  PG_HIP(hipGetLastError());
  return PG_OK;
}

int32_t pg_physics_step(int32_t *state, int32_t n, const uint8_t *actions, void *stream) {
  if (n < 0 || (n > 0 && (!state || !actions))) return fail(PG_ERR_INVALID, "state/actions NULL or n < 0");
  if (n == 0) return PG_OK;
  hipLaunchKernelGGL(k_physics_step, dim3((n + 255) / 256), dim3(256), 0, (hipStream_t)stream, state, n,
                     actions);
  PG_HIP(hipGetLastError());
  return PG_OK;
}

int32_t pg_ga_select_tournament(const pg_select_args *a, void *stream) {
  if (!a) return fail(PG_ERR_INVALID, "args is NULL");
  if (a->k < 0 || a->n_pop < 1 || a->tournsize < 1 || !a->fitness || !a->chosen)
    return fail(PG_ERR_INVALID, "selTournament needs k >= 0, n_pop >= 1, tournsize >= 1 and buffers");
  if (a->k == 0) return PG_OK;
  hipLaunchKernelGGL(k_select, dim3((a->k + 255) / 256), dim3(256), 0, (hipStream_t)stream, *a);
  PG_HIP(hipGetLastError());
  return PG_OK;
}

int32_t pg_ga_select_tournament_ranked(const pg_select_args *a, const double *sorted_fitness,
                                       const int32_t *order, void *stream) {
  if (!a || !sorted_fitness || !order) return fail(PG_ERR_INVALID, "args/sorted_fitness/order is NULL");
  if (a->k < 0 || a->n_pop < 1 || a->tournsize < 1 || !a->chosen)
    return fail(PG_ERR_INVALID, "selTournament needs k >= 0, n_pop >= 1, tournsize >= 1 and buffers");
  if (a->k == 0) return PG_OK;
  hipLaunchKernelGGL(k_select_ranked, dim3((a->k + 255) / 256), dim3(256), 0, (hipStream_t)stream, *a,
                     sorted_fitness, order);
  PG_HIP(hipGetLastError());
  return PG_OK;
}

int32_t pg_ga_vary(const pg_ga_args *a, void *stream) {
  if (!a) return fail(PG_ERR_INVALID, "args is NULL");
  if (a->n < 0 || a->genes < 1 || a->stride < a->genes || !a->parents || !a->chosen || !a->offspring ||
      !a->invalid || (a->dtype != PG_F32 && a->dtype != PG_F64))
    return fail(PG_ERR_INVALID, "varAnd: bad sizes or NULL buffers");
  if (a->n == 0) return PG_OK;
  const int pairs = (a->n + 1) / 2;
  if (a->pair_list && (!a->pair_count || a->pair_cap < 0)) return fail(PG_ERR_INVALID, "varAnd: pair_list needs pair_count and pair_cap >= 0");
  constexpr int kListWaves = 8192;
  int waves = a->pair_list ? (a->pair_cap < pairs ? a->pair_cap : pairs) : pairs;
  if (a->pair_list && waves > kListWaves) waves = kListWaves;
  if (waves == 0) return PG_OK;
  const dim3 grid((unsigned)((waves + 3) / 4));
  if (a->dtype == PG_F64)
    hipLaunchKernelGGL(k_vary<double>, grid, dim3(256), 0, (hipStream_t)stream, *a);
  else
    hipLaunchKernelGGL(k_vary<float>, grid, dim3(256), 0, (hipStream_t)stream, *a);
  PG_HIP(hipGetLastError());
  return PG_OK;
}

int32_t pg_ga_list_pairs(const uint8_t *mask, int32_t n_pairs, int32_t *list, int32_t *count, void *stream) {
  if (n_pairs < 0 || !count || (n_pairs && (!mask || !list))) return fail(PG_ERR_INVALID, "list_pairs: bad sizes or NULL buffers");
  PG_HIP(hipMemsetAsync(count, 0, sizeof(int32_t), (hipStream_t)stream));
  if (n_pairs == 0) return PG_OK;
  hipLaunchKernelGGL(k_list_pairs, dim3((unsigned)((n_pairs + 255) / 256)), dim3(256), 0, (hipStream_t)stream, mask,
                     n_pairs, list, count);
  PG_HIP(hipGetLastError());
  return PG_OK;
}

int32_t pg_ga_mark_pairs(uint8_t *mask, int32_t n_pairs, const int32_t *rows, int32_t n_rows, int32_t skip_lo,
                         int32_t skip_hi, const uint8_t *exclude, void *stream) {
  if (n_pairs < 0 || n_rows < 0 || (n_rows && (!mask || !rows)))
    return fail(PG_ERR_INVALID, "mark_pairs: bad sizes or NULL buffers");
  if (n_rows == 0) return PG_OK;
  hipLaunchKernelGGL(k_mark_pairs, dim3((unsigned)((n_rows + 255) / 256)), dim3(256), 0, (hipStream_t)stream, mask,
                     n_pairs, rows, n_rows, skip_lo, skip_hi, exclude);
  PG_HIP(hipGetLastError());
  return PG_OK;
}

int32_t pg_ga_schedule(const pg_schedule_args *a, void *stream) {
  if (!a) return fail(PG_ERR_INVALID, "args is NULL");
  if (a->n < 0 || a->n_games < 1 || a->n_hof < 0 || a->row_offset < 0 ||
      (a->mode != PG_SCHED_REFERENCE && a->mode != PG_SCHED_SELFPLAY))
    return fail(PG_ERR_INVALID, "schedule: bad sizes or mode");
  if (a->n == 0) return PG_OK;
  if (!a->kind || !a->opp || !a->mult || (a->mode == PG_SCHED_REFERENCE && a->n_hof > 0 && !a->hof_fitness))
    return fail(PG_ERR_INVALID, "schedule: NULL output or hof_fitness");
  const long total = (long)a->n * a->n_games;
  if (a->hof_slices > 1 && a->block_rows < 1) return fail(PG_ERR_INVALID, "schedule: hof_slices > 1 needs block_rows >= 1");
  hipLaunchKernelGGL(k_schedule, dim3((unsigned)((total + 255) / 256)), dim3(256), 0, (hipStream_t)stream, *a);
  PG_HIP(hipGetLastError());
  return PG_OK;
}

int32_t pg_gather_rows(void *dst, int64_t dst_stride, const void *old_rows, int64_t old_stride, const void *rows,
                       int64_t rows_stride, const int64_t *index, const int32_t *src, int32_t n_old, int32_t n,
                       int64_t genes, int32_t dtype, void *stream) {
  if (n < 0 || n_old < 0 || genes < 1 || (dtype != PG_F32 && dtype != PG_F64) ||
      (n > 0 && (!dst || !src || (n_old > 0 && !old_rows) || dst_stride < genes || old_stride < genes ||
                 rows_stride < genes)))
    return fail(PG_ERR_INVALID, "gather_rows: bad sizes, dtype or NULL buffers");
  if (n == 0) return PG_OK;
  if (dtype == PG_F64)
    hipLaunchKernelGGL(k_gather_rows<double>, dim3(n), dim3(256), 0, (hipStream_t)stream, (double *)dst, dst_stride,
                       (const double *)old_rows, old_stride, (const double *)rows, rows_stride, index, src, n_old,
                       genes);
  else
    hipLaunchKernelGGL(k_gather_rows<float>, dim3(n), dim3(256), 0, (hipStream_t)stream, (float *)dst, dst_stride,
                       (const float *)old_rows, old_stride, (const float *)rows, rows_stride, index, src, n_old,
                       genes);
  PG_HIP(hipGetLastError());
  return PG_OK;
}

int32_t pg_row_hash(const void *rows, int64_t stride, const int32_t *index, int32_t n, int64_t genes,
                    int32_t dtype, uint64_t *hash, void *stream) {
  if (n < 0 || genes < 0 || (n > 0 && (!rows || !hash || stride < genes)) || (dtype != PG_F32 && dtype != PG_F64))
    return fail(PG_ERR_INVALID, "row_hash: bad sizes, dtype or NULL buffers");
  if (n == 0) return PG_OK;
  if (dtype == PG_F64)
    hipLaunchKernelGGL(k_row_hash<double>, dim3(n), dim3(256), 0, (hipStream_t)stream, (const double *)rows, stride,
                       index, n, genes, hash);
  else
    hipLaunchKernelGGL(k_row_hash<float>, dim3(n), dim3(256), 0, (hipStream_t)stream, (const float *)rows, stride,
                       index, n, genes, hash);
  PG_HIP(hipGetLastError());
  return PG_OK;
}

int32_t pg_hof_update(const pg_hof_args *a) {
  if (!a) return fail(PG_ERR_INVALID, "args is NULL");
  if (a->maxsize < 0 || a->hof_n < 0 || a->hof_n > a->maxsize || a->pop_n < 0 || !a->new_n ||
      (a->maxsize > 0 && (!a->new_src || !a->new_fitness)) || (a->hof_n > 0 && (!a->hof_fitness || !a->hof_hash)) ||
      (a->pop_n > 0 && (!a->pop_fitness || !a->pop_hash)))
    return fail(PG_ERR_INVALID, "hof_update: bad sizes or NULL buffers");
  const int hn = a->hof_n, pn = a->pop_n, n = hn + pn;
  auto fit_of = [&](int e) { return e < hn ? a->hof_fitness[e] : a->pop_fitness[e - hn]; };
  auto hash_of = [&](int e) { return e < hn ? a->hof_hash[e] : a->pop_hash[e - hn]; };
  auto age_of = [&](int e) { return e < hn ? (hn - 1 - e) : e; };
  std::vector<int32_t> rank_v, by_rank((size_t)n);
  const int32_t *rank = a->rank;
  if (!rank) {
    std::vector<int32_t> order((size_t)n);
    for (int e = 0; e < n; ++e) order[e] = e;
    std::sort(order.begin(), order.end(), [&](int x, int y) {
      const double fx = fit_of(x), fy = fit_of(y);
      return fx < fy || (fx == fy && age_of(x) < age_of(y));
    });
    rank_v.resize((size_t)n);
    for (int r = 0; r < n; ++r) rank_v[order[r]] = r;
    rank = rank_v.data();
  }
  for (int e = 0; e < n; ++e) {
    if (rank[e] < 0 || rank[e] >= n) return fail(PG_ERR_INVALID, "hof_update: rank[%d]=%d out of range", e, rank[e]);
    by_rank[rank[e]] = e;
  }
  std::vector<uint64_t> present(((size_t)n + 63) / 64, 0);
  bool dense = true;
  for (int e = 0; e < n && dense; ++e) dense = (uint64_t)hash_of(e) < (uint64_t)n;
  std::vector<int32_t> dense_count(dense ? (size_t)n : 0, 0);
  size_t cap = 1;
  if (!dense)
    while (cap < 2 * (size_t)n + 16) cap <<= 1;
  struct Slot {
    uint64_t key;
    int32_t count, used;
  };
  std::vector<Slot> table(dense ? 0 : cap, Slot{0, 0, 0});
  auto count_of = [&](uint64_t key) -> int32_t & {
    if (dense) return dense_count[key];
    size_t i = (size_t)(key * 0x9E3779B97F4A7C15ull) & (cap - 1);
    while (table[i].used && table[i].key != key) i = (i + 1) & (cap - 1);
    if (!table[i].used) table[i] = Slot{key, 0, 1};
    return table[i].count;
  };
  int size = 0, worst = n;
  auto add = [&](int e) {
    const int r = rank[e];
    present[r >> 6] |= 1ull << (r & 63);
    count_of(hash_of(e)) += 1;
    size += 1;
    worst = r < worst ? r : worst;
  };
  for (int e = 0; e < hn; ++e) add(e);
  for (int i = 0; i < pn; ++i) {
    if (size == 0 && a->maxsize != 0) {
      add(hn);
      continue;
    }
    if (a->maxsize == 0) continue;
    const double f = a->pop_fitness[i];
    if (size >= a->maxsize && !(f > fit_of(by_rank[worst]))) continue;
    if (count_of(a->pop_hash[i]) > 0) continue;
    if (size >= a->maxsize) {
      present[worst >> 6] &= ~(1ull << (worst & 63));
      count_of(hash_of(by_rank[worst])) -= 1;
      size -= 1;
      size_t wd = (size_t)worst >> 6;
      uint64_t bits = present[wd] & (~0ull << (worst & 63));
      while (!bits && ++wd < present.size()) bits = present[wd];
      worst = bits ? (int)(wd * 64 + __builtin_ctzll(bits)) : n;
    }
    add(hn + i);
  }
  int j = 0;
  for (size_t wd = present.size(); wd-- > 0;) {
    uint64_t bits = present[wd];
// ... 176 lines not shown
```

neuro-genetic-pong-self-play_amd/pong_amd/_lib.py:

```python
from __future__ import annotations

import ctypes
import os
import threading

PKG_DIR = os.path.dirname(os.path.dirname(os.path.abspath(__file__)))
REPO_DIR = os.path.dirname(PKG_DIR)
LIB_NAME = "libpong_ga.so"
LIB_PATH = os.environ.get("PONG_GA_LIB") or os.path.join(PKG_DIR, LIB_NAME)
HEADER_PATH = os.path.join(REPO_DIR, "include", "pong_ga.h")

PG_ABI_VERSION = 12
PG_MAX_NODES = 9

PG_OK, PG_ERR_INVALID, PG_ERR_HIP, PG_ERR_UNSUPPORTED = 0, -1, -2, -3
PG_F32, PG_F64 = 0, 1
PG_OPP_HARDCODED, PG_OPP_ROM_CPU, PG_OPP_SCORE, PG_OPP_NN = 0, 1, 2, 3
PG_PREP_ALL, PG_PREP_GENOMES, PG_PREP_REST = 0, 1, 2
PG_PREC_CERTIFIED, PG_PREC_F64 = 0, 1
PG_SCHED_REFERENCE, PG_SCHED_SELFPLAY = 0, 1
PG_KERNEL_AUTO, PG_KERNEL_GENERAL, PG_KERNEL_RESIDENT, PG_KERNEL_SPLIT, PG_KERNEL_WIDE, PG_KERNEL_STAGED = 0, 1, 2, 3, 4, 5
PG_STATE_FIELDS = 16
STATE_FIELD_NAMES = ("ball_x", "ball_y", "ball_vx", "ball_vy", "ball_visible", "serve_timer",
                     "serve_dir", "hits", "point", "lpy", "rpy", "score1", "score2",
                     "one_player", "seed_lo", "seed_hi")

_vp = ctypes.c_void_p


class PgNet(ctypes.Structure):
    _fields_ = [("n_nodes", ctypes.c_int32), ("nodes", ctypes.c_int32 * PG_MAX_NODES),
                ("bias", ctypes.c_int32), ("dtype", ctypes.c_int32)]


class PgEvalArgs(ctypes.Structure):
    _fields_ = [
        ("struct_size", ctypes.c_uint32),
        ("net", PgNet),
        ("n_genomes", ctypes.c_int32), ("n_games", ctypes.c_int32),
        ("genomes", _vp), ("genome_stride", ctypes.c_int64),
        ("opponents", _vp), ("opponent_stride", ctypes.c_int64), ("n_opponents", ctypes.c_int32),
        ("precision", ctypes.c_int32),
        ("game_kind", _vp), ("game_opp", _vp), ("game_mult", _vp),
        ("seed", ctypes.c_uint64),
        ("fitness", _vp), ("rewards", _vp), ("scores", _vp), ("frames", _vp),
        ("total_frames", _vp), ("status", _vp), ("counters", _vp),
        ("trace", _vp), ("trace_games", ctypes.c_int32), ("trace_cap", ctypes.c_int32),
        ("kernel", ctypes.c_int32), ("group_lanes", ctypes.c_int32),
        ("workspace", _vp), ("workspace_bytes", ctypes.c_size_t),
        ("hard_log", _vp), ("hard_cap", ctypes.c_int32), ("genome_rows", _vp),
        ("n_active", _vp),
        ("prep", ctypes.c_int32), ("horizon", ctypes.c_int32),
        ("timeout_thresh", ctypes.c_int32), ("win_score", ctypes.c_int32),
    ]

    def __init__(self, *args, **kw):
        super().__init__(*args, **kw)
        self.struct_size = ctypes.sizeof(PgEvalArgs)


class PgForwardArgs(ctypes.Structure):
    _fields_ = [
        ("net", PgNet), ("n", ctypes.c_int32), ("genomes", _vp), ("genome_stride", ctypes.c_int64),
        ("genome_index", _vp), ("x", _vp), ("precision", ctypes.c_int32), ("index", _vp),
        ("act", _vp), ("counters", _vp), ("z_all", _vp), ("h_all", _vp),
    ]


class PgDecideArgs(ctypes.Structure):
    _fields_ = [
        ("net", PgNet), ("n", ctypes.c_int32), ("genomes", _vp), ("genome_stride", ctypes.c_int64),
        ("genome_index", _vp), ("k", _vp), ("index", _vp), ("stage", _vp),
    ]


class PgWideDecideArgs(ctypes.Structure):
    _fields_ = [
        ("net", PgNet), ("n", ctypes.c_int32), ("genomes", _vp), ("genome_stride", ctypes.c_int64),
        ("genome_index", _vp), ("k", _vp), ("index", _vp), ("act", _vp),
        ("workspace", _vp), ("workspace_bytes", ctypes.c_size_t),
    ]


class PgGaArgs(ctypes.Structure):
    _fields_ = [
        ("n", ctypes.c_int32), ("genes", ctypes.c_int64), ("dtype", ctypes.c_int32),
        ("parents", _vp), ("stride", ctypes.c_int64), ("n_parents", ctypes.c_int32),
        ("chosen", _vp), ("offspring", _vp), ("invalid", _vp),
        ("cxpb", ctypes.c_double), ("mutpb", ctypes.c_double), ("alpha", ctypes.c_double),
        ("mu", ctypes.c_double), ("sigma", ctypes.c_double), ("indpb", ctypes.c_double),
        ("seed", ctypes.c_uint64), ("generation", ctypes.c_uint64), ("pair_mask", _vp),
        ("pair_list", _vp), ("pair_count", _vp), ("pair_cap", ctypes.c_int32),
    ]


class PgSelectArgs(ctypes.Structure):
    _fields_ = [
        ("n_pop", ctypes.c_int32), ("k", ctypes.c_int32), ("tournsize", ctypes.c_int32),
        ("fitness", _vp), ("chosen", _vp), ("seed", ctypes.c_uint64), ("generation", ctypes.c_uint64),
    ]


class PgScheduleArgs(ctypes.Structure):
    _fields_ = [
        ("mode", ctypes.c_int32), ("n", ctypes.c_int32), ("n_games", ctypes.c_int32),
        ("row_offset", ctypes.c_int64), ("n_hof", ctypes.c_int32), ("hof_fitness", _vp),
        ("seed", ctypes.c_uint64), ("generation", ctypes.c_uint64),
        ("kind", _vp), ("opp", _vp), ("mult", _vp), ("rows", _vp),
        ("hof_slices", ctypes.c_int32), ("block_rows", ctypes.c_int32), ("slice_local", ctypes.c_int32),
    ]


class PgHofPackedArgs(ctypes.Structure):
    _fields_ = [("maxsize", ctypes.c_int32), ("hof_n", ctypes.c_int32), ("hof_fitness", _vp), ("k", ctypes.c_int32),
                ("packed", _vp), ("new_n", _vp), ("new_src", _vp), ("new_fitness", _vp),
                ("slot_in", _vp), ("slot_out", _vp)]


class PgHofArgs(ctypes.Structure):
    _fields_ = [
        ("maxsize", ctypes.c_int32), ("hof_n", ctypes.c_int32), ("hof_fitness", _vp), ("hof_hash", _vp),
        ("pop_n", ctypes.c_int32), ("pop_fitness", _vp), ("pop_hash", _vp), ("rank", _vp),
        ("new_n", _vp), ("new_src", _vp), ("new_fitness", _vp),
    ]


class PgHofRankArgs(ctypes.Structure):
    _fields_ = [
        ("hof_n", ctypes.c_int32), ("hof_fitness", _vp), ("hof_hash", _vp), ("k", ctypes.c_int32),
        ("cand_fitness", _vp), ("cand_hash", _vp), ("packed", _vp), ("workspace", _vp),
        ("workspace_bytes", ctypes.c_size_t),
    ]


class PgHofPrepareArgs(ctypes.Structure):
    _fields_ = [
        ("fitness", _vp), ("pop_n", ctypes.c_int32), ("filter", ctypes.c_int32), ("worst", ctypes.c_double),
        ("rows", _vp), ("stride", ctypes.c_int64), ("genes", ctypes.c_int64), ("dtype", ctypes.c_int32),
        ("hof_n", ctypes.c_int32), ("hof_fitness", _vp), ("hof_hash", _vp), ("k", _vp), ("cand", _vp),
        ("hashes", _vp), ("packed", _vp), ("workspace", _vp), ("workspace_bytes", ctypes.c_size_t),
    ]


class PgScatterArgs(ctypes.Structure):
    _fields_ = [
        ("n", ctypes.c_int32), ("n_games", ctypes.c_int32), ("row_lo", ctypes.c_int32),
        ("fitness", _vp), ("frames", _vp), ("rows", _vp), ("n_active", _vp), ("shard_fitness", _vp),
        ("lineage", _vp),
    ]


class PgMergeArgs(ctypes.Structure):
    _fields_ = [
        ("pop_n", ctypes.c_int32), ("fitness", _vp), ("invalid", _vp), ("inherited", _vp), ("new_fitness", _vp),
        ("filter", ctypes.c_int32), ("worst", ctypes.c_double), ("cand", _vp), ("cand_fitness", _vp),
        ("summary", _vp), ("workspace", _vp), ("workspace_bytes", ctypes.c_size_t),
    ]


class PgHofCandArgs(ctypes.Structure):
    _fields_ = [
        ("hof_n", ctypes.c_int32), ("hof_fitness", _vp), ("hof_hash", _vp), ("k", ctypes.c_int32),
        ("cand", _vp), ("cand_fitness", _vp), ("rows", _vp), ("stride", ctypes.c_int64),
        ("genes", ctypes.c_int64), ("dtype", ctypes.c_int32), ("cand_hash", _vp), ("packed", _vp),
        ("workspace", _vp), ("workspace_bytes", ctypes.c_size_t),
    ]


class PgHofCommitArgs(ctypes.Structure):
    _fields_ = [
        ("dst", _vp), ("dst_stride", ctypes.c_int64), ("old_rows", _vp), ("old_stride", ctypes.c_int64),
        ("rows", _vp), ("rows_stride", ctypes.c_int64), ("cand", _vp), ("src", _vp), ("n_old", ctypes.c_int32),
        ("m", ctypes.c_int32), ("genes", ctypes.c_int64), ("dtype", ctypes.c_int32), ("old_hash", _vp),
        ("cand_hash", _vp), ("new_hash", _vp), ("fitness_in", _vp), ("new_fitness", _vp),
        ("dst_slot", _vp),
    ]


SIGNATURES = {
    "pg_version": (ctypes.c_char_p, []),
    "pg_abi_version": (ctypes.c_int32, []),
    "pg_build_flags": (ctypes.c_int32, []),
    "pg_last_error": (ctypes.c_char_p, []),
    "pg_device_count": (ctypes.c_int32, []),
    "pg_eval_workspace_bytes": (ctypes.c_size_t, [ctypes.POINTER(PgEvalArgs)]),
    "pg_gene_count": (ctypes.c_int32, [ctypes.POINTER(PgNet)]),
    "pg_eval_population": (ctypes.c_int32, [ctypes.POINTER(PgEvalArgs), _vp]),
    "pg_forward": (ctypes.c_int32, [ctypes.POINTER(PgForwardArgs), _vp]),
    "pg_decide": (ctypes.c_int32, [ctypes.POINTER(PgDecideArgs), _vp]),
    "pg_wide_decide_workspace_bytes": (ctypes.c_size_t, [ctypes.POINTER(PgWideDecideArgs)]),
    "pg_wide_decide": (ctypes.c_int32, [ctypes.POINTER(PgWideDecideArgs), _vp]),
    "pg_physics_reset": (ctypes.c_int32, [_vp, ctypes.c_int32, _vp, _vp, _vp]),
    "pg_physics_step": (ctypes.c_int32, [_vp, ctypes.c_int32, _vp, _vp]),
    "pg_ga_select_tournament": (ctypes.c_int32, [ctypes.POINTER(PgSelectArgs), _vp]),
    "pg_ga_select_tournament_ranked": (ctypes.c_int32, [ctypes.POINTER(PgSelectArgs), _vp, _vp, _vp]),
    "pg_ga_vary": (ctypes.c_int32, [ctypes.POINTER(PgGaArgs), _vp]),
    "pg_ga_list_pairs": (ctypes.c_int32, [_vp, ctypes.c_int32, _vp, _vp, _vp]),
    "pg_ga_mark_pairs": (ctypes.c_int32, [_vp, ctypes.c_int32, _vp, ctypes.c_int32, ctypes.c_int32, ctypes.c_int32,
                                          _vp, _vp]),
    "pg_ga_schedule": (ctypes.c_int32, [ctypes.POINTER(PgScheduleArgs), _vp]),
    "pg_row_hash": (ctypes.c_int32, [_vp, ctypes.c_int64, _vp, ctypes.c_int32, ctypes.c_int64, ctypes.c_int32, _vp,
                                     _vp]),
    "pg_hof_update": (ctypes.c_int32, [ctypes.POINTER(PgHofArgs)]),
    "pg_hof_update_packed": (ctypes.c_int32, [ctypes.POINTER(PgHofPackedArgs)]),
    "pg_hof_rank_classes_workspace_bytes": (ctypes.c_size_t, [ctypes.c_int32]),
    "pg_hof_rank_classes": (ctypes.c_int32, [ctypes.POINTER(PgHofRankArgs), _vp]),
    "pg_hof_prepare_workspace_bytes": (ctypes.c_size_t, [ctypes.c_int32, ctypes.c_int32]),
    "pg_hof_prepare": (ctypes.c_int32, [ctypes.POINTER(PgHofPrepareArgs), _vp]),
    "pg_gather_rows": (ctypes.c_int32, [_vp, ctypes.c_int64, _vp, ctypes.c_int64, _vp, ctypes.c_int64, _vp, _vp,
                                        ctypes.c_int32, ctypes.c_int32, ctypes.c_int64, ctypes.c_int32, _vp]),
    "pg_ga_scatter_fitness": (ctypes.c_int32, [ctypes.POINTER(PgScatterArgs), _vp]),
    "pg_ga_merge_workspace_bytes": (ctypes.c_size_t, [ctypes.c_int32]),
    "pg_ga_merge_fitness": (ctypes.c_int32, [ctypes.POINTER(PgMergeArgs), _vp]),
    "pg_ga_select_workspace_bytes": (ctypes.c_size_t, [ctypes.c_int32]),
    "pg_ga_select_ranked": (ctypes.c_int32, [ctypes.POINTER(PgSelectArgs), _vp, ctypes.c_size_t, _vp]),
    "pg_ga_inherit": (ctypes.c_int32, [_vp, ctypes.c_int32, _vp, _vp, _vp, _vp, _vp]),
    "pg_ga_order_workspace_bytes": (ctypes.c_size_t, [ctypes.c_int32]),
    "pg_ga_order": (ctypes.c_int32, [ctypes.c_int32, ctypes.c_int32, _vp, _vp, ctypes.c_int32, _vp, _vp, _vp,
                                     ctypes.c_size_t, _vp]),
    "pg_hof_prepare_cand_workspace_bytes": (ctypes.c_size_t, [ctypes.c_int32, ctypes.c_int32]),
    "pg_hof_prepare_cand": (ctypes.c_int32, [ctypes.POINTER(PgHofCandArgs), _vp]),
    "pg_hof_commit": (ctypes.c_int32, [ctypes.POINTER(PgHofCommitArgs), _vp]),
    "pg_render_frames": (ctypes.c_int32, [_vp, ctypes.c_int32, _vp, _vp]),
    "pg_find_stuff": (ctypes.c_int32, [_vp, ctypes.c_int64, ctypes.c_int32, _vp, _vp]),
}

_lock = threading.Lock()
_lib = None


class PongGAError(RuntimeError):

    def __init__(self, func: str, code: int, message: str):
        super().__init__(f"{func} failed ({code}): {message}")
        self.code = code


def lib() -> ctypes.CDLL:
    global _lib
    if _lib is not None:
        return _lib
    with _lock:
        if _lib is None:
            if not os.path.exists(LIB_PATH):
                raise RuntimeError(
                    f"{LIB_PATH} is missing: build it with `python -c 'import __graft_entry__ as g; g.build()'` "
                    "(hipcc --offload-arch=gfx950). There is no CPU fallback.")
            L = ctypes.CDLL(LIB_PATH)
            for name, (res, args) in SIGNATURES.items():
                fn = getattr(L, name)
                fn.restype = res
                fn.argtypes = args
            if L.pg_abi_version() != PG_ABI_VERSION:
                raise RuntimeError(f"{LIB_PATH}: ABI {L.pg_abi_version()} != {PG_ABI_VERSION}")
            _lib = L
    return _lib


def check(func: str, rc: int) -> None:
    if rc != PG_OK:
        msg = lib().pg_last_error()
        raise PongGAError(func, rc, msg.decode() if msg else "")


def make_net(nodes, bias=True, dtype=PG_F64) -> PgNet:
    nodes = [int(n) for n in nodes]
    if not 2 <= len(nodes) <= PG_MAX_NODES:
        raise ValueError(f"NETWORK_SHAPE must have 2..{PG_MAX_NODES} entries, got {nodes}")
    arr = (ctypes.c_int32 * PG_MAX_NODES)(*(nodes + [0] * (PG_MAX_NODES - len(nodes))))
    return PgNet(len(nodes), arr, 1 if bias else 0, dtype)
```

neuro-genetic-pong-self-play_amd/pong_amd/device.py:

```python
from __future__ import annotations

import ctypes
from dataclasses import dataclass
from typing import Optional

import torch

from . import _lib as L

PRECISIONS = {"certified": L.PG_PREC_CERTIFIED, "f64": L.PG_PREC_F64}
PREPS = {"all": L.PG_PREP_ALL, "genomes": L.PG_PREP_GENOMES, "rest": L.PG_PREP_REST}
KERNELS = {"auto": L.PG_KERNEL_AUTO, "general": L.PG_KERNEL_GENERAL, "split": L.PG_KERNEL_SPLIT,
           "wide": L.PG_KERNEL_WIDE}
DTYPES = {torch.float32: L.PG_F32, torch.float64: L.PG_F64}


def gene_count(nodes, bias=True) -> int:
    b = 1 if bias else 0
    return sum((int(nodes[i]) + b) * int(nodes[i + 1]) for i in range(len(nodes) - 1))


def _ptr(t: Optional[torch.Tensor]):
    return ctypes.c_void_p(t.data_ptr()) if t is not None else None


def _stream(device) -> ctypes.c_void_p:
    return ctypes.c_void_p(torch.cuda.current_stream(device).cuda_stream)


def _need(t: torch.Tensor, name: str, dtype, device, shape=None):
    if t.dtype != dtype:
        raise TypeError(f"{name} must be {dtype}, got {t.dtype}")
    if t.device != device:
        raise ValueError(f"{name} must live on {device}, got {t.device}")
    if not t.is_contiguous():
        raise ValueError(f"{name} must be contiguous")
    if shape is not None and tuple(t.shape) != tuple(shape):
        raise ValueError(f"{name} must have shape {tuple(shape)}, got {tuple(t.shape)}")


def _need_rows(t: torch.Tensor, name: str, dtype, device):
    if t.dtype != dtype:
        raise TypeError(f"{name} must be {dtype}, got {t.dtype}")
    if t.device != device:
        raise ValueError(f"{name} must live on {device}, got {t.device}")
    if t.dim() != 2 or (t.shape[1] > 1 and t.stride(1) != 1) or (t.shape[0] > 1 and t.stride(0) < t.shape[1]):
        raise ValueError(f"{name} must be row-major rows (unit column stride, row stride >= row length)")


@dataclass
class EvalResult:

    fitness: torch.Tensor
    rewards: torch.Tensor
    scores: torch.Tensor
    frames: torch.Tensor
    total_frames: torch.Tensor
    status: torch.Tensor
    counters: torch.Tensor


class Evaluator:

    def __init__(self, nodes, bias=True, dtype=torch.float64, device=None, n_games=6,
                 precision="certified", kernel="auto", group_lanes=0, seed=0, horizon=0,
                 timeout_thresh=0, win_score=0):
        if not torch.cuda.is_available():
            raise RuntimeError("pong_amd.Evaluator needs a HIP device (no CPU fallback)")
        L.lib()
        self.nodes = [int(n) for n in nodes]
        self.bias = bool(bias)
        self.dtype = dtype
        self.device = torch.device(device) if device is not None else torch.device("cuda", torch.cuda.current_device())
        self.n_games = int(n_games)
        self.precision = precision
        self.kernel = kernel
        self.group_lanes = int(group_lanes)
        self.seed = int(seed)
        self.horizon = int(horizon)
        self.timeout_thresh = int(timeout_thresh)
        self.win_score = int(win_score)
        self.genes = gene_count(self.nodes, self.bias)
        self.net = L.make_net(self.nodes, self.bias, DTYPES[dtype])
        self._ws = None
        self._prep_key = self._prep_ws = None

    def selfplay_schedule(self, n: int, n_opponents: int, offset: int = 0):
        dev = self.device
        gi = (torch.arange(n, device=dev, dtype=torch.int64) + offset)[:, None] * self.n_games
        gi = gi + torch.arange(self.n_games, device=dev, dtype=torch.int64)[None, :]
        kind = torch.full((n, self.n_games), L.PG_OPP_NN, dtype=torch.int32, device=dev)
        opp = (gi % max(n_opponents, 1)).to(torch.int32)
        mult = torch.ones((n, self.n_games), dtype=torch.float64, device=dev)
        return kind, opp, mult

    def _workspace(self, args: L.PgEvalArgs) -> torch.Tensor:
        need = L.lib().pg_eval_workspace_bytes(ctypes.byref(args))
        if self._ws is None or self._ws.numel() < need:
            self._ws = torch.empty(max(need, 4096), dtype=torch.uint8, device=self.device)
        return self._ws

    def evaluate(self, genomes: torch.Tensor, kind: torch.Tensor, opp: torch.Tensor, mult: torch.Tensor,
                 opponents: Optional[torch.Tensor] = None, trace_games: int = 0, trace_cap: int = 0,
                 out: Optional[EvalResult] = None, precision: Optional[str] = None,
                 kernel: Optional[str] = None, group_lanes: Optional[int] = None, validate: bool = True,
                 hard_log: Optional[torch.Tensor] = None, rows: Optional[torch.Tensor] = None,
                 n_active: Optional[torch.Tensor] = None, prep: str = "all", horizon: Optional[int] = None):
        dev = self.device
        n = genomes.shape[0] if rows is None else rows.shape[0]
        games = self.n_games
        _need(genomes, "genomes", self.dtype, dev)
        if genomes.dim() != 2 or genomes.shape[1] < self.genes:
            raise ValueError(f"genomes must be [n, >= {self.genes}], got {tuple(genomes.shape)}")
        _need(kind, "kind", torch.int32, dev, (n, games))
        _need(opp, "opp", torch.int32, dev, (n, games))
        _need(mult, "mult", torch.float64, dev, (n, games))
        if opponents is not None:
            _need_rows(opponents, "opponents", self.dtype, dev)
            if opponents.dim() != 2 or opponents.shape[1] < self.genes:
                raise ValueError(f"opponents must be [H, >= {self.genes}], got {tuple(opponents.shape)}")
        if rows is not None:
            _need(rows, "rows", torch.int32, dev, (n,))
        if validate and n:
            if rows is not None and bool(((rows < 0) | (rows >= genomes.shape[0])).any()):
                raise ValueError(f"rows must index the {genomes.shape[0]}-row genomes tensor")
            nn_games = kind == L.PG_OPP_NN
            if bool(((kind < 0) | (kind > L.PG_OPP_NN)).any()):
                raise ValueError("kind values must be pg_opp_kind codes 0..3")
            if bool(nn_games.any()):
                h = 0 if opponents is None else opponents.shape[0]
                bad = nn_games & ((opp < 0) | (opp >= h))
                if bool(bad.any()):
                    raise ValueError(f"opp rows must index the {h}-row opponents tensor")
        if out is None:
            out = EvalResult(
                fitness=torch.empty(n, dtype=torch.float64, device=dev),
                rewards=torch.empty((n, games), dtype=torch.float64, device=dev),
                scores=torch.empty((n, games, 2), dtype=torch.int32, device=dev),
                frames=torch.empty((n, games), dtype=torch.int32, device=dev),
                total_frames=torch.empty((n, games), dtype=torch.float64, device=dev),
                status=torch.empty(n, dtype=torch.int32, device=dev),
                counters=torch.empty(16, dtype=torch.int64, device=dev))
        trace = None
        if trace_games and trace_cap:
            trace = torch.zeros((trace_games, trace_cap), dtype=torch.uint8, device=dev)
        a = L.PgEvalArgs()
        a.net = self.net
        a.n_genomes = n
        a.n_games = games
        a.genomes = _ptr(genomes)
        a.genome_stride = genomes.stride(0) if genomes.shape[0] > 1 else genomes.shape[1]
        a.genome_rows = _ptr(rows)
        if n_active is not None:
            _need(n_active, "n_active", torch.int32, dev, (1,))
            a.n_active = _ptr(n_active)
        if opponents is not None and opponents.shape[0] > 0:
            a.opponents = _ptr(opponents)
            a.opponent_stride = opponents.stride(0) if opponents.shape[0] > 1 else opponents.shape[1]
            a.n_opponents = opponents.shape[0]
        a.precision = PRECISIONS[precision or self.precision]
        a.game_kind, a.game_opp, a.game_mult = _ptr(kind), _ptr(opp), _ptr(mult)
        a.seed = self.seed
        a.fitness, a.rewards, a.scores = _ptr(out.fitness), _ptr(out.rewards), _ptr(out.scores)
        a.frames, a.total_frames, a.status = _ptr(out.frames), _ptr(out.total_frames), _ptr(out.status)
        a.counters = _ptr(out.counters)
        if trace is not None:
            a.trace, a.trace_games, a.trace_cap = _ptr(trace), trace_games, trace_cap
        if hard_log is not None:
            _need(hard_log, "hard_log", torch.int32, dev)
            if hard_log.dim() != 2 or hard_log.shape[1] != 8:
                raise ValueError("hard_log must be [cap, 8] int32")
            a.hard_log, a.hard_cap = _ptr(hard_log), hard_log.shape[0]
        a.prep = PREPS[prep]
        if prep == "rest" and n and self._prep_key != self._prep_of(genomes, rows, n_active, n):
            raise ValueError("prep='rest' needs a preceding prep='genomes' call with the same genomes, rows, "
                             "n_active and row count on this evaluator")
        a.horizon = self.horizon if horizon is None else int(horizon)
        a.timeout_thresh, a.win_score = self.timeout_thresh, self.win_score
        a.kernel = KERNELS[kernel or self.kernel]
        a.group_lanes = self.group_lanes if group_lanes is None else int(group_lanes)
        ws = self._workspace(a)
        a.workspace, a.workspace_bytes = _ptr(ws), ws.numel()
        if prep == "rest" and n and self._prep_ws != ws.data_ptr():
            raise ValueError("prep='rest': the workspace holding the genome records was reallocated")
        with torch.cuda.device(dev):
            L.check("pg_eval_population", L.lib().pg_eval_population(ctypes.byref(a), _stream(dev)))
        self._prep_key = self._prep_of(genomes, rows, n_active, n) if prep == "genomes" else None
        self._prep_ws = ws.data_ptr() if prep == "genomes" else None
        return out, trace

    @staticmethod
    def _prep_of(genomes, rows, n_active, n):
        return (genomes.data_ptr(), genomes.stride(0), None if rows is None else rows.data_ptr(),
                None if n_active is None else n_active.data_ptr(), int(n))

    def forward(self, genomes: torch.Tensor, x: torch.Tensor, genome_index: Optional[torch.Tensor] = None,
                precision: Optional[str] = None, want_act: bool = True, want_layers: bool = False):
        dev = self.device
        _need(genomes, "genomes", self.dtype, dev)
        n = x.shape[0]
        _need(x, "x", torch.float64, dev, (n, self.nodes[0]))
        if genome_index is not None:
            _need(genome_index, "genome_index", torch.int32, dev, (n,))
        index = torch.empty(n, dtype=torch.int32, device=dev)
        act = torch.empty((n, self.nodes[-1]), dtype=torch.float64, device=dev) if want_act else None
        counters = torch.zeros(4, dtype=torch.int64, device=dev)
        a = L.PgForwardArgs()
        a.net = self.net
        a.n = n
        a.genomes = _ptr(genomes)
        a.genome_stride = genomes.stride(0) if genomes.shape[0] > 1 else genomes.shape[1]
        a.genome_index = _ptr(genome_index)
        a.x = _ptr(x)
        a.precision = PRECISIONS[precision or self.precision]
        a.index = _ptr(index)
        a.act = _ptr(act)
        a.counters = _ptr(counters)
        if want_layers:
            units = sum(self.nodes[1:])
            z_all = torch.empty((n, units), dtype=torch.float64, device=dev)
            h_all = torch.empty((n, units), dtype=torch.float64, device=dev)
            a.z_all, a.h_all = _ptr(z_all), _ptr(h_all)
            self.last_layers = (z_all, h_all)
        with torch.cuda.device(dev):
            L.check("pg_forward", L.lib().pg_forward(ctypes.byref(a), _stream(dev)))
        self.last_forward_counters = counters
        return index, act

    def decide(self, genomes: torch.Tensor, k: torch.Tensor, genome_index: Optional[torch.Tensor] = None):
        dev = self.device
        _need(genomes, "genomes", self.dtype, dev)
        n = k.shape[0]
        _need(k, "k", torch.int32, dev, (n, 6))
        if genome_index is not None:
            _need(genome_index, "genome_index", torch.int32, dev, (n,))
        index = torch.empty(n, dtype=torch.int32, device=dev)
        stage = torch.empty(n, dtype=torch.int32, device=dev)
        a = L.PgDecideArgs()
        a.net = self.net
        a.n = n
        a.genomes = _ptr(genomes)
        a.genome_stride = genomes.stride(0) if genomes.shape[0] > 1 else genomes.shape[1]
        a.genome_index = _ptr(genome_index)
        a.k = _ptr(k)
        a.index = _ptr(index)
        a.stage = _ptr(stage)
        with torch.cuda.device(dev):
            L.check("pg_decide", L.lib().pg_decide(ctypes.byref(a), _stream(dev)))
        return index, stage

    def wide_decide(self, genomes: torch.Tensor, k: torch.Tensor, genome_index: Optional[torch.Tensor] = None):
        dev = self.device
        _need(genomes, "genomes", self.dtype, dev)
        n = k.shape[0]
        _need(k, "k", torch.int32, dev, (n, 6))
        if genome_index is not None:
            _need(genome_index, "genome_index", torch.int32, dev, (n,))
        index = torch.empty(n, dtype=torch.int32, device=dev)
        act = torch.empty((n, self.nodes[-1]), dtype=torch.float64, device=dev)
        a = L.PgWideDecideArgs()
        a.net = self.net
        a.n = n
        a.genomes = _ptr(genomes)
        a.genome_stride = genomes.stride(0) if genomes.shape[0] > 1 else genomes.shape[1]
        a.genome_index = _ptr(genome_index)
        a.k = _ptr(k)
        a.index = _ptr(index)
        a.act = _ptr(act)
        nbytes = L.lib().pg_wide_decide_workspace_bytes(ctypes.byref(a))
        ws = torch.empty(nbytes, dtype=torch.uint8, device=dev)
        a.workspace, a.workspace_bytes = _ptr(ws), nbytes
        with torch.cuda.device(dev):
            L.check("pg_wide_decide", L.lib().pg_wide_decide(ctypes.byref(a), _stream(dev)))
        return index, act


class Physics:

    def __init__(self, n: int, device=None):
        L.lib()
        self.n = int(n)
        self.device = torch.device(device) if device is not None else torch.device("cuda", torch.cuda.current_device())
        self.state = torch.zeros((L.PG_STATE_FIELDS, self.n), dtype=torch.int32, device=self.device)

    def reset(self, seeds: torch.Tensor, one_player: Optional[torch.Tensor] = None):
        _need(seeds, "seeds", torch.int64, self.device, (self.n,))
        if one_player is not None:
            _need(one_player, "one_player", torch.int32, self.device, (self.n,))
        with torch.cuda.device(self.device):
            L.check("pg_physics_reset", L.lib().pg_physics_reset(
                _ptr(self.state), self.n, _ptr(seeds), _ptr(one_player), _stream(self.device)))

    def step(self, actions: torch.Tensor):
        _need(actions, "actions", torch.uint8, self.device, (self.n,))
        with torch.cuda.device(self.device):
            L.check("pg_physics_step", L.lib().pg_physics_step(
                _ptr(self.state), self.n, _ptr(actions), _stream(self.device)))

    def fields(self) -> dict:
        s = self.state.cpu()
        return {name: s[i] for i, name in enumerate(L.STATE_FIELD_NAMES)}


def select_tournament(fitness: torch.Tensor, k: int, tournsize: int, seed: int, generation: int) -> torch.Tensor:
    _need(fitness, "fitness", torch.float64, fitness.device)
    chosen = torch.empty(k, dtype=torch.int32, device=fitness.device)
    a = L.PgSelectArgs(fitness.shape[0], k, tournsize, _ptr(fitness), _ptr(chosen), seed, generation)
    with torch.cuda.device(fitness.device):
        L.check("pg_ga_select_tournament", L.lib().pg_ga_select_tournament(ctypes.byref(a), _stream(fitness.device)))
    return chosen


def select_tournament_ranked(fitness: torch.Tensor, k: int, tournsize: int, seed: int, generation: int) -> torch.Tensor:
    _need(fitness, "fitness", torch.float64, fitness.device)
    sorted_fit, order = torch.sort(fitness, stable=True)
    order = order.to(torch.int32)
    chosen = torch.empty(k, dtype=torch.int32, device=fitness.device)
    a = L.PgSelectArgs(fitness.shape[0], k, tournsize, _ptr(fitness), _ptr(chosen), seed, generation)
    with torch.cuda.device(fitness.device):
        L.check("pg_ga_select_tournament_ranked", L.lib().pg_ga_select_tournament_ranked(
            ctypes.byref(a), _ptr(sorted_fit), _ptr(order), _stream(fitness.device)))
    return chosen


def vary(parents: torch.Tensor, chosen: torch.Tensor, genes: int, cxpb: float, mutpb: float, alpha: float,
         mu: float, sigma: float, indpb: float, seed: int, generation: int, out: Optional[torch.Tensor] = None,
         pair_mask: Optional[torch.Tensor] = None, invalid: Optional[torch.Tensor] = None,
         pair_list: Optional[tuple] = None):
    dev = parents.device
    n = chosen.shape[0]
    _need(chosen, "chosen", torch.int32, dev, (n,))
    if pair_mask is not None:
        _need(pair_mask, "pair_mask", torch.uint8, dev, ((n + 1) // 2,))
    if out is None:
        out = torch.empty((n, parents.shape[1]), dtype=parents.dtype, device=dev)
    if invalid is None:
        invalid = torch.empty(n, dtype=torch.uint8, device=dev)
    _need(invalid, "invalid", torch.uint8, dev, (n,))
    a = L.PgGaArgs()
    a.n, a.genes, a.dtype = n, genes, DTYPES[parents.dtype]
    a.parents, a.stride, a.n_parents = _ptr(parents), parents.stride(0), parents.shape[0]
    a.chosen, a.offspring, a.invalid = _ptr(chosen), _ptr(out), _ptr(invalid)
    a.cxpb, a.mutpb, a.alpha, a.mu, a.sigma, a.indpb = cxpb, mutpb, alpha, mu, sigma, indpb
    a.seed, a.generation = seed, generation
    a.pair_mask = _ptr(pair_mask)
    if pair_list is not None:
        lst, cnt, cap = pair_list
        _need(lst, "pair_list", torch.int32, dev)
        _need(cnt, "pair_count", torch.int32, dev, (1,))
        a.pair_list, a.pair_count, a.pair_cap = _ptr(lst), _ptr(cnt), int(min(cap, lst.numel()))
    if out.stride(0) != parents.stride(0):
        raise ValueError("offspring and parents must share the row stride")
    with torch.cuda.device(dev):
        L.check("pg_ga_vary", L.lib().pg_ga_vary(ctypes.byref(a), _stream(dev)))
    return out, invalid


def list_pairs(mask: torch.Tensor, out: torch.Tensor, count: torch.Tensor) -> None:
    dev = mask.device
    _need(mask, "pair_mask", torch.uint8, dev)
    _need(out, "pair_list", torch.int32, dev)
    _need(count, "pair_count", torch.int32, dev, (1,))
    if out.numel() < mask.numel():
        raise ValueError("pair_list must hold every pair")
    with torch.cuda.device(dev):
        L.check("pg_ga_list_pairs", L.lib().pg_ga_list_pairs(_ptr(mask), mask.numel(), _ptr(out), _ptr(count),
                                                             _stream(dev)))


def mark_pairs(mask: torch.Tensor, rows: torch.Tensor, skip: tuple = (0, 0),
               exclude: Optional[torch.Tensor] = None) -> None:
    dev = mask.device
    _need(mask, "pair_mask", torch.uint8, dev)
    _need(rows, "rows", torch.int32, dev)
    if exclude is not None:
        _need(exclude, "exclude", torch.uint8, dev, tuple(mask.shape))
    with torch.cuda.device(dev):
        L.check("pg_ga_mark_pairs", L.lib().pg_ga_mark_pairs(_ptr(mask), mask.shape[0], _ptr(rows), rows.numel(),
                                                             int(skip[0]), int(skip[1]), _ptr(exclude), _stream(dev)))


SCHEDULES = {"reference": L.PG_SCHED_REFERENCE, "selfplay": L.PG_SCHED_SELFPLAY}


def schedule(mode: str, n: int, n_games: int, row_offset: int, hof_fitness: Optional[torch.Tensor], n_hof: int,
             seed: int, generation: int, device, rows: Optional[torch.Tensor] = None, hof_slices: int = 1,
             block_rows: int = 0, slice_local: bool = False, out: Optional[tuple] = None):
    dev = torch.device(device)
    if out is None:
        kind = torch.empty((n, n_games), dtype=torch.int32, device=dev)
        opp = torch.empty((n, n_games), dtype=torch.int32, device=dev)
        mult = torch.empty((n, n_games), dtype=torch.float64, device=dev)
    else:
        kind, opp, mult = out
        _need(kind, "kind", torch.int32, dev, (n, n_games))
        _need(opp, "opp", torch.int32, dev, (n, n_games))
        _need(mult, "mult", torch.float64, dev, (n, n_games))
    if hof_fitness is not None:
        _need(hof_fitness, "hof_fitness", torch.float64, dev)
        if hof_fitness.numel() < n_hof:
            raise ValueError(f"hof_fitness holds {hof_fitness.numel()} values, n_hof={n_hof}")
    elif n_hof and mode == "reference":
        raise ValueError("reference schedule with a hall of fame needs hof_fitness")
    if rows is not None:
        _need(rows, "rows", torch.int32, dev, (n,))
    a = L.PgScheduleArgs(SCHEDULES[mode], n, n_games, row_offset, n_hof, _ptr(hof_fitness), seed, generation,
                         _ptr(kind), _ptr(opp), _ptr(mult), _ptr(rows), int(hof_slices), int(block_rows),
                         1 if slice_local else 0)
    with torch.cuda.device(dev):
        L.check("pg_ga_schedule", L.lib().pg_ga_schedule(ctypes.byref(a), _stream(dev)))
    return kind, opp, mult


def row_hash(rows: torch.Tensor, genes: Optional[int] = None, index: Optional[torch.Tensor] = None) -> torch.Tensor:
    if rows.dim() != 2 or rows.dtype not in DTYPES or rows.stride(1) != 1:
        raise ValueError("rows must be a row-major [n, G] f32/f64 tensor")
    genes = rows.shape[1] if genes is None else int(genes)
    n = rows.shape[0] if index is None else index.shape[0]
    if index is not None:
        _need(index, "index", torch.int32, rows.device, (n,))
    out = torch.empty(n, dtype=torch.int64, device=rows.device)
    stride = rows.stride(0) if rows.shape[0] > 1 else rows.shape[1]
    with torch.cuda.device(rows.device):
        L.check("pg_row_hash", L.lib().pg_row_hash(_ptr(rows), stride, _ptr(index), n, genes, DTYPES[rows.dtype],
                                                   _ptr(out), _stream(rows.device)))
    return out


def gather_rows(dst: torch.Tensor, old_rows: torch.Tensor, rows: torch.Tensor, src: torch.Tensor, n_old: int,
                index: Optional[torch.Tensor] = None, genes: Optional[int] = None) -> torch.Tensor:
    dev = dst.device
    n = src.shape[0]
    _need(src, "src", torch.int32, dev, (n,))
    if index is not None:
        _need(index, "index", torch.int64, dev, (index.shape[0],))
    for name, t in (("dst", dst), ("old_rows", old_rows), ("rows", rows)):
        if t.dim() != 2 or t.dtype != dst.dtype or t.device != dev or t.stride(1) != 1:
            raise ValueError(f"{name} must be a row-major [n, G] tensor of dst's dtype on dst's device")
    genes = dst.shape[1] if genes is None else int(genes)
    if n > dst.shape[0]:
        raise ValueError("more source indices than destination rows")
    with torch.cuda.device(dev):
        L.check("pg_gather_rows", L.lib().pg_gather_rows(
            _ptr(dst), dst.stride(0), _ptr(old_rows), old_rows.stride(0), _ptr(rows), rows.stride(0), _ptr(index),
            _ptr(src), int(n_old), n, genes, DTYPES[dst.dtype], _stream(dev)))
    return dst


def hof_rank_classes(hof_fitness: torch.Tensor, hof_hash: torch.Tensor, cand_fitness: torch.Tensor,
                     cand_hash: torch.Tensor) -> torch.Tensor:
    dev = cand_fitness.device
    hn, k = hof_fitness.shape[0], cand_fitness.shape[0]
    _need(hof_fitness, "hof_fitness", torch.float64, dev, (hn,))
    _need(hof_hash, "hof_hash", torch.int64, dev, (hn,))
    _need(cand_fitness, "cand_fitness", torch.float64, dev, (k,))
    _need(cand_hash, "cand_hash", torch.int64, dev, (k,))
    packed = torch.empty(hn + 2 * k, dtype=torch.int64, device=dev)
    nbytes = int(L.lib().pg_hof_rank_classes_workspace_bytes(hn + k))
    if nbytes == 0:
        msg = L.lib().pg_last_error()
        raise L.PongGAError("pg_hof_rank_classes_workspace_bytes", -1, msg.decode() if msg else "")
    ws = torch.empty(nbytes, dtype=torch.uint8, device=dev)
    a = L.PgHofRankArgs(hn, _ptr(hof_fitness), _ptr(hof_hash), k, _ptr(cand_fitness), _ptr(cand_hash),
                        _ptr(packed), _ptr(ws), nbytes)
    with torch.cuda.device(dev):
        L.check("pg_hof_rank_classes", L.lib().pg_hof_rank_classes(ctypes.byref(a), _stream(dev)))
    return packed


def hof_prepare(fitness: torch.Tensor, worst: Optional[float], rows: torch.Tensor, genes: int,
                hof_fitness: torch.Tensor, hof_hash: torch.Tensor):
    dev = fitness.device
    pn, hn = fitness.shape[0], hof_fitness.shape[0]
    _need(fitness, "fitness", torch.float64, dev, (pn,))
    _need(hof_fitness, "hof_fitness", torch.float64, dev, (hn,))
    _need(hof_hash, "hof_hash", torch.int64, dev, (hn,))
    if rows.dim() != 2 or rows.shape[0] != pn or rows.dtype not in DTYPES or rows.stride(1) != 1 or rows.device != dev:
        raise ValueError("rows must be a row-major [pop_n, G] f32/f64 tensor on fitness's device")
    cand = torch.empty(pn, dtype=torch.int64, device=dev)
    hashes = torch.empty(hn + pn, dtype=torch.int64, device=dev)
    packed = torch.empty(hn + 2 * pn, dtype=torch.int64, device=dev)
    nbytes = int(L.lib().pg_hof_prepare_workspace_bytes(hn, pn))
    if nbytes == 0:
        msg = L.lib().pg_last_error()
        raise L.PongGAError("pg_hof_prepare_workspace_bytes", -1, msg.decode() if msg else "")
    ws = torch.empty(nbytes, dtype=torch.uint8, device=dev)
    k = ctypes.c_int32(0)
    stride = rows.stride(0) if pn > 1 else rows.shape[1]
    a = L.PgHofPrepareArgs(_ptr(fitness), pn, 0 if worst is None else 1, 0.0 if worst is None else float(worst),
                           _ptr(rows), stride, int(genes), DTYPES[rows.dtype], hn, _ptr(hof_fitness), _ptr(hof_hash),
                           ctypes.addressof(k), _ptr(cand), _ptr(hashes), _ptr(packed), _ptr(ws), nbytes)
    with torch.cuda.device(dev):
        L.check("pg_hof_prepare", L.lib().pg_hof_prepare(ctypes.byref(a), _stream(dev)))
    k = k.value
    return k, cand[:k], hashes[: hn + k], packed[: hn + 2 * k]


def hof_update(maxsize: int, hof_fitness, hof_hash, pop_fitness, pop_hash, rank=None):
    import numpy as np
    hf = np.ascontiguousarray(hof_fitness, dtype=np.float64)
    hh = np.ascontiguousarray(np.asarray(hof_hash, dtype=np.int64)).view(np.uint64)
    pf = np.ascontiguousarray(pop_fitness, dtype=np.float64)
    ph = np.ascontiguousarray(np.asarray(pop_hash, dtype=np.int64)).view(np.uint64)
# ... 223 lines not shown
```

neuro-genetic-pong-self-play_amd/pong_amd/evolve.py:

```python
from __future__ import annotations

from typing import Optional

import numpy as np
import torch
import torch.distributed as dist

from . import device as D
from . import dist as PD

STAT_FIELDS = ("avg", "std", "min", "max")


class DeviceGA:

    def __init__(self, nodes, population_size: int, hof_size: Optional[int] = None,
                 tournsize: Optional[int] = None, *, bias: bool = True, dtype=torch.float64, device=None,
                 n_games: int = 6, schedule: str = "reference", cxpb: float = 0.9, mutpb: float = 0.9,
                 alpha: float = 0.9, mu: float = 0.0, sigma: float = 0.9, indpb: float = 0.9,
                 seed: int = 0, physics_seed: int = 0, precision: str = "certified", kernel: str = "auto",
                 group=None, hof_block_rows: int = 0, timeout_thresh: int = 0, win_score: int = 0):
        if schedule not in D.SCHEDULES:
            raise ValueError(f"schedule must be one of {sorted(D.SCHEDULES)}")
        self.nodes = [int(v) for v in nodes]
        self.P = int(population_size)
        self.H = int(hof_size) if hof_size is not None else max(self.P // 4, 1)
        self.tournsize = int(tournsize) if tournsize is not None else max(self.P // 4, 1)
        if self.P < 1 or self.H < 0 or self.tournsize < 1:
            raise ValueError("population_size >= 1, hof_size >= 0 and tournsize >= 1 required")
        self.ev = D.Evaluator(self.nodes, bias=bias, dtype=dtype, device=device, n_games=n_games,
                              precision=precision, kernel=kernel, seed=physics_seed,
                              timeout_thresh=timeout_thresh, win_score=win_score)
        self.device, self.dtype, self.G = self.ev.device, dtype, self.ev.genes
        self.bias, self.n_games, self.schedule = bool(bias), int(n_games), schedule
        self.cxpb, self.mutpb, self.alpha = float(cxpb), float(mutpb), float(alpha)
        self.mu, self.sigma, self.indpb = float(mu), float(sigma), float(indpb)
        self.seed, self.physics_seed = int(seed), int(physics_seed)
        self.precision, self.kernel = precision, kernel
        self.group = group
        self.world = dist.get_world_size(group) if dist.is_initialized() else 1
        self.rank = dist.get_rank(group) if dist.is_initialized() else 0
        self.lo, self.hi = PD.shard_range(self.P, self.rank, self.world)
        self.hof_block_rows = int(hof_block_rows)
        self.hof_slices = 1
        if self.hof_block_rows > 0 and schedule == "selfplay":
            self.hof_slices = max(1, min(-(-self.P // self.hof_block_rows), max(self.H, 1)))
        B = self.hof_block_rows
        self._slice = ((self.lo // B) % self.hof_slices
                       if self.hof_slices > 1 and self.hi > self.lo and self.lo // B == (self.hi - 1) // B else None)
        self.store = torch.zeros((self.H + self.P, self.G), dtype=dtype, device=self.device)
        self.spare = torch.empty_like(self.store)
        self.in_place_hall = True
        self._hall_buf = self.store[: self.H]
        M = max(self.H, 1)
        self._up_dev = torch.zeros(4 * M, dtype=torch.int32, device=self.device)
        self.hof_slot = self._up_dev[3 * M:]
        self.hof_slot.copy_(torch.arange(M, dtype=torch.int32, device=self.device))
        self._hof_slot_h = np.zeros(0, np.int32)
        self._slots_identity = True
        self._up_keep = None
        self.fitness = torch.zeros(self.P, dtype=torch.float64, device=self.device)
        self.valid = torch.zeros(self.P, dtype=torch.bool, device=self.device)
        self.hof_fitness = torch.zeros(max(self.H, 1), dtype=torch.float64, device=self.device)
        self.hof_n = 0
        self._hof_fit_host = np.zeros(0, np.float64)
        self.hof_hash = torch.zeros(max(self.H, 1), dtype=torch.int64, device=self.device)
        self.generation = -1
        self.logbook = []
        self.last = None
        self.last_rows = None
        self.last_count = None
        self.eval_events = None
        self.profile = None
        self._t_mark = self._t_sub = 0.0
        self._next = None
        self.early_prep = True
        self.hard_log = None
        self.on_evaluate = None
        self.order_by_length = True
        self.lineage_frames = torch.zeros(self.P, dtype=torch.float32, device=self.device)
        self.native_prepare = True
        self.fused = True
        self.side_stream = True
        self._side = None
        self.prepare_first = True
        self.presubmit = True
        self._pinned = {}
        self.persistent_bufs = True
        self._up_flip = 0
        self._iota_P = None
        self.shard_vary = self.world > 1
        self.balance_shards = False
        self._dealt = {}
        self._n_pairs = (self.P + 1) // 2
        self._skip = (self.lo >> 1, (self.hi + 1) >> 1) if self.hi > self.lo else (0, 0)
        self._shard_pairs = None
        self.ws = D.Workspaces(self.device)
        self._lineage_alt = torch.zeros_like(self.lineage_frames)
        self._hof_hash_alt = torch.zeros_like(self.hof_hash)
        self._hof_fitness_alt = torch.zeros_like(self.hof_fitness)
        self._fit_alt = torch.zeros_like(self.fitness)
        self._summary_h = torch.zeros(8, dtype=torch.float64, pin_memory=True)

    def _sliced(self, n_hof: int) -> bool:
        return self._slice is not None and n_hof >= self.hof_slices

    def _opponents(self, buf: torch.Tensor, n_hof: int) -> Optional[torch.Tensor]:
        if not n_hof:
            return None
        if self._in_place():
            if self._sliced(n_hof):
                idx = self.hof_slot[self._slice:n_hof:self.hof_slices].long()
                out = self._buf("hall_slice", (idx.shape[0], self.G), self.dtype)
                torch.index_select(self._hall_buf, 0, idx, out=out)
                return out
            return self._hall_buf[:n_hof]
        return buf[self._slice:n_hof:self.hof_slices] if self._sliced(n_hof) else buf[:n_hof]

    def _in_place(self) -> bool:
        return bool(self.in_place_hall and self.fused and self.H > 0)

    def _opp_slots(self, opp: torch.Tensor, n_hof: int) -> torch.Tensor:
        if not self._in_place() or not n_hof or self._sliced(n_hof) or self._slots_identity:
            return opp
        out = self._buf("opp_slots", opp.numel(), torch.int32) if self.persistent_bufs else None
        return torch.index_select(self.hof_slot[:n_hof], 0, opp.reshape(-1), out=out).view_as(opp)

    def _opponents_by_position(self, n_hof: int) -> Optional[torch.Tensor]:
        if not n_hof:
            return None
        if self._in_place() and not self._sliced(n_hof):
            return self.hall_of_fame[:n_hof]
        return self._opponents(self.store, n_hof)

    def eval_schedule(self, g: int, n_hof: Optional[int] = None, rows="last", out: Optional[tuple] = None):
        n_hof = self.hof_n if n_hof is None else n_hof
        rows = self.last_rows if isinstance(rows, str) else rows
        kw = {}
        if self.hof_slices > 1:
            kw = dict(hof_slices=self.hof_slices, block_rows=self.hof_block_rows, slice_local=self._sliced(n_hof))
        n = rows.shape[0] if rows is not None else self.hi - self.lo
        return D.schedule(self.schedule, n, self.n_games, self.lo, self.hof_fitness, n_hof, self.seed,
                          g, self.device, rows=rows, out=out, **kw)

    def _sched_bufs(self, g: int, n: int) -> tuple:
        if not self.persistent_bufs:
            return None
        return (self._buf("sched_kind%d" % (g & 1), (n, self.n_games), torch.int32),
                self._buf("sched_opp%d" % (g & 1), (n, self.n_games), torch.int32),
                self._buf("sched_mult%d" % (g & 1), (n, self.n_games), torch.float64))

    def _balanced(self) -> bool:
        return bool(self.balance_shards and self.fused and self.world > 1 and dist.is_initialized()
                    and self.hof_slices == 1)

    @property
    def _n_eval(self) -> int:
        return -(-self.P // self.world) if self._balanced() else self.hi - self.lo

    @property
    def _rows(self) -> torch.Tensor:
        return self.store[self.H:]

    @property
    def population(self) -> torch.Tensor:
        if self._sharded():
            raise RuntimeError("DeviceGA.population: with sharded variation this rank holds only its shard "
                               "current; use shard_rows() or population_full() (a collective)")
        return self._rows

    def shard_rows(self) -> torch.Tensor:
        return self._rows[self.lo:self.hi]

    def population_full(self) -> torch.Tensor:
        if not self._sharded():
            return self._rows
        return PD.gather_rows(self._rows[self.lo:self.hi].contiguous(), self.P, self.group)

    def population_hash(self) -> torch.Tensor:
        if not self._sharded():
            return D.row_hash(self._rows, self.G)
        return PD.gather_rows(D.row_hash(self._rows[self.lo:self.hi], self.G), self.P, self.group)

    def _sharded(self) -> bool:
        return bool(self.shard_vary and self.fused and self.world > 1 and dist.is_initialized())

    @property
    def hall_of_fame(self) -> torch.Tensor:
        if self._in_place():
            return self._hall_buf[self.hof_slot[: self.hof_n].long()]
        return self.store[: self.hof_n]

    @property
    def hof_member_fitness(self) -> np.ndarray:
        return self._hof_fit_host.copy()

    def initialize(self, init: str = "uniform", init_sigma: float = 3.0):
        gen = torch.Generator(device=self.device).manual_seed(self.seed)
        rows = max(1, (1 << 28) // (8 * self.G))
        for r0 in range(0, self.P, rows):
            r1 = min(self.P, r0 + rows)
            if init == "uniform":
                blk = torch.rand((r1 - r0, self.G), generator=gen, dtype=torch.float64, device=self.device)
            elif init == "normal":
                blk = torch.randn((r1 - r0, self.G), generator=gen, dtype=torch.float64,
                                  device=self.device).mul_(init_sigma)
            else:
                raise ValueError("init must be 'uniform' or 'normal'")
            self.store[self.H + r0:self.H + r1] = blk.to(self.dtype)
        self.valid.zero_()
        self.fitness.zero_()
        self._set_hof_empty()
        self._next = None
        self.generation = -1
        self.logbook = []

    def set_population(self, genomes: torch.Tensor, fitness: Optional[torch.Tensor] = None,
                       valid: Optional[torch.Tensor] = None):
        if tuple(genomes.shape) != (self.P, self.G):
            raise ValueError(f"genomes must be [{self.P}, {self.G}], got {tuple(genomes.shape)}")
        self._next = None
        self._rows.copy_(genomes.to(device=self.device, dtype=self.dtype))
        if fitness is None:
            self.valid.zero_()
            self.fitness.zero_()
        else:
            self.fitness.copy_(fitness.to(device=self.device, dtype=torch.float64))
            v = torch.ones(self.P, dtype=torch.bool) if valid is None else valid.to(torch.bool)
            self.valid.copy_(v.to(self.device))
# ... 113 lines not shown
            h = D.row_hash(rows, self.G, index=cand.to(torch.int32))
            fc = fit[cand]
            hashes = torch.cat([self.hof_hash[:old_n], h])
            by_age = torch.cat([self.hof_fitness[:old_n].flip(0), fc])
            order = torch.sort(by_age, stable=True).indices
            rank_age = torch.empty_like(order)
            rank_age[order] = torch.arange(n, device=self.device)
            rank = torch.cat([rank_age[:old_n].flip(0), rank_age[old_n:]])
            cls = torch.unique(hashes, return_inverse=True)[1]
            packed_d = torch.cat([rank | (cls << 32), fc.view(torch.int64)])
        packed_h = torch.empty(packed_d.shape, dtype=torch.int64, pin_memory=True)
        packed_h.copy_(packed_d, non_blocking=True)
        copied = torch.cuda.Event()
        copied.record()
        if overlap:
            overlap()
        copied.synchronize()
        packed = packed_h.numpy()
        self._mark("hof_prepare", sub=True)
        rank_np = (packed[:n] & 0xFFFFFFFF).astype(np.int32)
        cls_np = packed[:n] >> 32
        src, new_fit = D.hof_update(self.H, self._hof_fit_host, cls_np[:old_n], packed[n:].view(np.float64),
                                    cls_np[old_n:], rank=rank_np)
        self._mark("hof_scan", sub=True)
        m = src.shape[0]
        up = torch.empty(3 * m, dtype=torch.int32, pin_memory=True)
        upn = up.numpy()
        upn[: 2 * m].view(np.float64)[:] = new_fit
        upn[2 * m:] = src
        up_d = up.to(self.device, non_blocking=True)
        src_t = up_d[2 * m:]
        D.gather_rows(dst, self.store, rows, src_t, old_n, index=cand)
        self.hof_hash[:m] = hashes.index_select(0, src_t.long())
        self.hof_fitness[:m] = up_d[: 2 * m].view(torch.float64)
        self.hof_n = int(m)
        self._hof_fit_host = new_fit

    @staticmethod
    def _summary(fit: torch.Tensor, invalid: torch.Tensor):
        v = torch.stack([torch.isnan(fit).any().double(), fit.mean(), fit.std(unbiased=False), fit.min(), fit.max(),
                         invalid.sum().double()]).tolist()
        if v[0]:
            raise ZeroDivisionError("float division by zero (calculate_reward with total_frames == 0)")
        return v[1:5], int(v[5])

    def _record(self, g: int, nevals: int, vals=None) -> dict:
        if vals is None:
            f = self.fitness
            vals = torch.stack([f.mean(), f.std(unbiased=False), f.min(), f.max()]).tolist()
        rec = {"gen": g, "nevals": nevals, **dict(zip(STAT_FIELDS, vals))}
        self.logbook.append(rec)
        return rec

    def step(self) -> dict:
        return self._step_fused() if self.fused else self._step_torch()

    def _step_torch(self) -> dict:
        if self.generation < 0:
            fit = self._evaluate(0, self._rows, ~self.valid)
            nevals = int((~self.valid).sum())
            new_fit = torch.where(self.valid, self.fitness, fit)
            self._check(new_fit)
            self.fitness, self.valid = new_fit, torch.ones_like(self.valid)
            self._hof_update(new_fit, self._rows, self.spare,
                             overlap=lambda: self._prefetch(1, self._rows, new_fit, self.spare))
            self.store[: self.hof_n] = self.spare[: self.hof_n]
            self.generation = 0
            return self._record(0, nevals)
        g = self.generation + 1
        self._mark(None)
        off = self.spare[self.H:]
        if self._next is not None and self._next[0] == g:
            inv, inherited = self._next[1:]
        else:
            inv, inherited = self._select_vary(g, self._rows, self.fitness, off)
        self._next = None
        self._mark("select_vary")
        fit = self._evaluate(g, off, inv)
        new_fit = torch.where(inv, fit, inherited)
        self._mark("evaluate")
        stats, nevals = self._summary(new_fit, inv)
        self._hof_update(new_fit, off, self.spare, overlap=lambda: self._prefetch(g + 1, off, new_fit, self.store))
        self._mark("hall_of_fame")
        self.fitness = new_fit
        self.store, self.spare = self.spare, self.store
        self.generation = g
        rec = self._record(g, nevals, stats)
        self._mark("record")
        return rec

    def _buf(self, name, shape, dtype):
        return self.ws.tensor(name, shape, dtype)

    def _select(self, g: int, fitness: torch.Tensor) -> torch.Tensor:
        chosen = self._buf("chosen%d" % (g & 1), self.P, torch.int32)
        D.select_ranked(fitness, self.P, self.tournsize, self.seed, g, self.ws, chosen=chosen)
        return chosen

    def _shard_mask(self) -> torch.Tensor:
        if self._shard_pairs is None:
            self._shard_pairs = torch.zeros(self._n_pairs, dtype=torch.uint8, device=self.device)
            self._shard_pairs[self._skip[0]:self._skip[1]] = 1
        return self._shard_pairs

    def _complete(self, g: int, off: torch.Tensor, parents: torch.Tensor, rows: torch.Tensor, name: str,
                  exclude: Optional[torch.Tensor] = None) -> torch.Tensor:
        mask = self._buf("complete_" + name, self._n_pairs, torch.uint8)
        mask.zero_()
        D.mark_pairs(mask, rows, skip=self._skip, exclude=exclude)
        lst = self._buf("complete_list_" + name, self._n_pairs, torch.int32)
        cnt = self._buf("complete_count_" + name, 1, torch.int32)
        D.list_pairs(mask, lst, cnt)
        chosen = self._buf("chosen%d" % (g & 1), self.P, torch.int32)
        D.vary(parents, chosen, self.G, self.cxpb, self.mutpb, self.alpha, self.mu, self.sigma, self.indpb,
               seed=self.seed, generation=g, out=off, pair_list=(lst, cnt, min(rows.numel(), self._n_pairs)),
               invalid=self._buf("complete_inv_" + name, self.P, torch.uint8))
        return mask

    def _deal(self, inv_u8: torch.Tensor, g: int):
        P = self.P
        grows = self._buf("deal_rows", P, torch.int32)
        gcount = self._buf("deal_count", 1, torch.int32)
        D.order(P, 0, inv_u8, self.lineage_frames, True, grows, gcount, self.ws)
        n = self._n_eval
        pos = PD.deal_positions(n, self.rank, self.world, self.device)
        local = self._buf("local_rows%d" % (g & 1), n, torch.int32)
        local.copy_(grows[pos.clamp(max=P - 1)])
        count = self._buf("local_count%d" % (g & 1), 1, torch.int32)
        count.copy_((pos < gcount.long()).sum().to(torch.int32).reshape(1))
        return local, count

    def _gather_dealt(self, res, local: torch.Tensor, count: torch.Tensor) -> torch.Tensor:
        P, n = self.P, local.shape[0]
        played = torch.arange(n, device=self.device) < count
        rid = torch.where(played, local.long(), torch.full_like(local, P, dtype=torch.int64))
        longest = res.frames.max(dim=1).values.double()
        pack = torch.stack([rid.double(), res.fitness, longest], dim=1)
        allp = PD.gather_equal(pack, self.group)
        at = allp[:, 0].long()
        fit = torch.zeros(P + 1, dtype=torch.float64, device=self.device)
        fit.index_copy_(0, at, allp[:, 1])
        lin = torch.cat([self.lineage_frames, self.lineage_frames.new_zeros(1)])
        lin.index_copy_(0, at, allp[:, 2].float())
        self.lineage_frames.copy_(lin[:P])
        return fit[:P]

    def _next_gen_prep(self, g: int, parents: torch.Tensor, fitness: torch.Tensor, store: torch.Tensor,
                       cand_pairs: Optional[torch.Tensor] = None):
        chosen = self._select(g, fitness)
        if cand_pairs is not None:
            prev = self._dealt.get((g - 1) & 1)
            self._complete(g - 1, parents, store[self.H:], chosen, "parents",
                           exclude=cand_pairs if prev is None else (cand_pairs | prev))
        _, inv = D.vary(parents, chosen, self.G, self.cxpb, self.mutpb, self.alpha, self.mu, self.sigma, self.indpb,
                        seed=self.seed, generation=g, out=store[self.H:],
                        pair_mask=self._shard_mask() if self._sharded() else None,
                        invalid=self._buf("invalid%d" % (g & 1), self.P, torch.uint8) if self.persistent_bufs else None)
        inherited = self._buf("inherited", self.P, torch.float64)
        D.inherit(chosen, fitness, inherited, self.lineage_frames, self._lineage_alt)
        self.lineage_frames, self._lineage_alt = self._lineage_alt, self.lineage_frames
        if self._balanced():
            order = self._deal(inv, g)
            if self._sharded():
                self._dealt[g & 1] = self._complete(g, store[self.H:], parents, order[0], "dealt%d" % (g & 1))
        else:
            order = self._order(inv, g)
        self._next = (g, inv, inherited, order, self._early_prep(g, store[self.H:], order))

    def _early_prep(self, g: int, off: torch.Tensor, order):
        n = self._n_eval
        if (not self.early_prep or self.schedule != "selfplay" or self.H == 0 or self.hof_n != self.H or self.last is None
                or self.last.fitness.shape[0] != n):
            return None
        local, count = order
        sched = self.eval_schedule(g, n_hof=self.H, rows=local, out=self._sched_bufs(g, n))
        opponents = self._hall_buf[: self.H] if self._in_place() else self._opponents(self.spare, self.H)
        if self._in_place() and self._sliced(self.H):
            opponents = self._hall_buf[self._slice:self.H:self.hof_slices]
        self.ev.evaluate(off, *sched, opponents=opponents, out=self.last, validate=False,
                         hard_log=self.hard_log, rows=local, n_active=count, prep="genomes")
        return sched

    def _order(self, inv_u8: Optional[torch.Tensor], g: int = 0):
        n = self.hi - self.lo
        local = self._buf("local_rows%d" % (g & 1), n, torch.int32)
        count = self._buf("local_count%d" % (g & 1), 1, torch.int32)
        D.order(n, self.lo, inv_u8, self.lineage_frames, self.order_by_length, local, count, self.ws)
        return local, count

    def _evaluate_fused(self, g: int, rows: torch.Tensor, order, sched=None) -> torch.Tensor:
        lo, hi = self.lo, self.hi
        n = self._n_eval
        local, count = order
        if sched is None:
            kind, opp, mult = self.eval_schedule(g, rows=local, out=self._sched_bufs(g, n))
        else:
            kind, opp, mult = sched
        opponents = self._opponents(self.store, self.hof_n)
        opp = self._opp_slots(opp, self.hof_n)
        out = self.last if (self.last is not None and self.last.fitness.shape[0] == n) else None
        if self.eval_events is not None:
            self.eval_events[0].record()
        res, _ = self.ev.evaluate(rows, kind, opp, mult, opponents=opponents, out=out, validate=False,
                                  hard_log=self.hard_log, rows=local, n_active=count,
                                  prep="all" if sched is None else "rest")
        if self.eval_events is not None:
            self.eval_events[1].record()
        self.last, self.last_rows, self.last_count = res, local, count
        if self.on_evaluate is not None:
            self.on_evaluate(g, rows, self._opponents_by_position(self.hof_n), res)
        if self._balanced():
            return self._gather_dealt(res, local, count)
        shard = self._buf("shard_fit", n, torch.float64)
        D.scatter_fitness(res, n, lo, local, count, shard, self.lineage_frames)
        if not dist.is_initialized():
            return shard
        both = torch.stack([shard, self.lineage_frames[lo:hi].double()], dim=1)
        full = PD.gather_fitness(both, self.P, self.group)
        self.lineage_frames.copy_(full[:, 1].float())
        return full[:, 0].contiguous()

    def _merge(self, fit: torch.Tensor, inv: Optional[torch.Tensor], inherited: Optional[torch.Tensor],
               worst: Optional[float]):
        new_fit, cand, cand_fit, ev = self._merge_start(fit, inv, inherited, worst)
        return (new_fit, cand, cand_fit) + self._merge_finish(ev)

    def _merge_start(self, fit, inv, inherited, worst):
        new_fit = self._fit_alt
        cand = self._buf("cand", self.P, torch.int32)
        cand_fit = self._buf("cand_fit", self.P, torch.float64)
        summ = self._buf("summary", 8, torch.float64)
        D.merge_fitness(fit, inv, inherited, new_fit, worst, cand, cand_fit, summ, self.ws)
        self._summary_h.copy_(summ, non_blocking=True)
        ev = torch.cuda.Event()
        ev.record()
        return new_fit, cand, cand_fit, ev

    def _merge_finish(self, ev):
        ev.synchronize()
        v = self._summary_h.tolist()
        if v[0]:
            raise ZeroDivisionError("float division by zero (calculate_reward with total_frames == 0)")
        self._fit_alt = self.fitness
        return v[1:5], int(v[5]), int(v[6])

    def _hof_update_fused(self, rows: torch.Tensor, cand: torch.Tensor, cand_fit: torch.Tensor, k: int,
                          dst: torch.Tensor, overlap=None):
        if self.H == 0:
            if overlap:
                overlap()
            return
        old_n = self.hof_n
        in_place = self._in_place()
        if k == 0:
            if not in_place:
                dst[:old_n] = self.store[:old_n]
            if overlap:
                overlap()
            return
        if self.profile is not None:
            self.profile["hof_candidates"] = self.profile.get("hof_candidates", 0) + k
        main = torch.cuda.current_stream(self.device)
        side = ready = None
        if overlap and self.side_stream:
            if self._side is None:
                self._side = torch.cuda.Stream(self.device)
            side = self._side
            ready = torch.cuda.Event()
            ready.record(main)
            if not self.prepare_first:
                side.wait_event(ready)
                with torch.cuda.stream(side):
                    overlap()
                self._keep_on(main)
                overlap = None
        n = old_n + k
        cand, cand_fit = cand[:k], cand_fit[:k]
        cand_hash = self._buf("cand_hash", k, torch.int64)
        packed = self._buf("packed", n + k, torch.int64)
        D.hof_prepare_cand(self.hof_fitness[:old_n], self.hof_hash[:old_n], cand, cand_fit, rows, self.G, cand_hash,
                           packed, self.ws)
        packed_h = self._pin("packed", n + k, torch.int64)
        packed_h.copy_(packed, non_blocking=True)
        copied = torch.cuda.Event()
        copied.record()
        self._mark("hof_prepare", sub=True)
        if overlap and side is not None:
            side.wait_event(ready)
            with torch.cuda.stream(side):
                overlap()
            self._keep_on(main)
        elif overlap:
            overlap()
        if overlap:
            self._mark("next_select_vary", sub=True)
        copied.synchronize()
        M = max(self.H, 1)
        self._up_flip ^= 1
        up = self._pin("up%d" % self._up_flip, 4 * M, torch.int32)
        res = D.hof_update_packed(self.H, self._hof_fit_host, packed_h.numpy(), k, out=up.numpy(),
                                  slot_in=self._hof_slot_h if in_place else None, slots=in_place)
        src, new_fit = res[0], res[1]
        self._mark("hof_scan", sub=True)
        m = src.shape[0]
        up_d = self._up_dev
        up_d.copy_(up, non_blocking=True)
        src_d, fit_d = up_d[2 * M:2 * M + m], up_d[: 2 * M].view(torch.float64)[:m]
        if in_place:
            slot_d = up_d[3 * M:3 * M + m]
            D.hof_commit(self._hall_buf, None, rows, cand, src_d, old_n, self.G, self.hof_hash, cand_hash,
                         self._hof_hash_alt, fit_d, self._hof_fitness_alt, dst_slot=slot_d)
            self._hof_slot_h = res[2]
            self._slots_identity = False
        else:
            D.hof_commit(dst, self.store, rows, cand, src_d, old_n, self.G, self.hof_hash, cand_hash,
                         self._hof_hash_alt, fit_d, self._hof_fitness_alt)
        self.hof_hash, self._hof_hash_alt = self._hof_hash_alt, self.hof_hash
        self.hof_fitness, self._hof_fitness_alt = self._hof_fitness_alt, self.hof_fitness
        self.hof_n = int(m)
        self._hof_fit_host = new_fit
        self._up_keep = up
        if side is not None:
            main.wait_stream(side)

    def _pin(self, name: str, n: int, dtype) -> torch.Tensor:
        buf = self._pinned.get(name)
        if buf is None or buf.shape[0] < n or buf.dtype != dtype:
            buf = torch.empty(max(n, 1), dtype=dtype, pin_memory=True)
            self._pinned[name] = buf
        return buf[:n]

    def _keep_on(self, stream):
        if self._next is None:
            return
        for t in self._next[1:]:
            for x in (t if isinstance(t, tuple) else (t,)):
                if isinstance(x, torch.Tensor) and x.is_cuda:
                    x.record_stream(stream)

    def _step_fused(self) -> dict:
        worst = float(self._hof_fit_host[-1]) if (self.H and self.hof_n >= self.H) else None
        if self.generation < 0:
            inv = (~self.valid).to(torch.uint8)
            fit = self._evaluate_fused(0, self._rows, self._deal(inv, 0) if self._balanced() else self._order(inv))
            new_fit, cand, cand_fit, stats, nevals, k = self._merge(fit, inv, self.fitness, worst)
            self.fitness, self.valid = new_fit, torch.ones_like(self.valid)
            self._hof_update_fused(self._rows, cand, cand_fit, k, self.spare,
                                   overlap=lambda: self._next_gen_prep(1, self._rows, new_fit, self.spare))
            if not self._in_place():
                self.store[: self.hof_n] = self.spare[: self.hof_n]
            self.generation = 0
            return self._record(0, nevals, stats)
        g = self.generation + 1
        self._mark(None)
        off = self.spare[self.H:]
        if self._next is None or self._next[0] != g:
            self._next_gen_prep(g, self._rows, self.fitness, self.spare)
        _, inv, inherited, order, sched = self._next
# ... 81 lines not shown
```

Baseline: 13.10 billion.

## Fuse lane-record packing into the variation kernel and index records by row

The variation kernel now stages each offspring pair's genes in LDS and builds the split evaluator's per-lane f32 records, including certification error bounds, straight into the eval workspace. The evaluator then reads these records by genome row, so the separate genome prep pass before evaluation is skipped. This removes one kernel and a re-read of the f64 genomes each generation. In exchange it adds LDS use and shuffle work to vary, supports only the [6,33..64,3] 8-lane untraced shape, and bumps the ABI.

```diff
diff --git a/include/pong_ga.h b/include/pong_ga.h
--- a/include/pong_ga.h
+++ b/include/pong_ga.h
@@ -8,7 +8,7 @@
 extern "C" {
 #endif
 
-#define PG_ABI_VERSION 12
+#define PG_ABI_VERSION 13
 #define PG_MAX_NODES 9
 
 typedef enum pg_status {
@@ -91,7 +91,22 @@
   int32_t horizon;
   int32_t timeout_thresh;
   int32_t win_score;
+  int32_t rec_by_row;
 } pg_eval_args;
+
+typedef struct pg_vary_records {
+  uint32_t struct_size;
+  int32_t hidden;
+  int32_t bias;
+  int32_t lanes;
+  int32_t units;
+  int32_t outputs;
+  int32_t rec_floats;
+  int32_t row_base;
+  int32_t rows;
+  size_t offset;
+  float *recs;
+} pg_vary_records;
 
 
 typedef struct pg_forward_args {
@@ -159,6 +174,7 @@
   const int32_t *pair_list;
   const int32_t *pair_count;
   int32_t pair_cap;
+  const struct pg_vary_records *records;
 } pg_ga_args;
 
 typedef struct pg_select_args {
@@ -261,6 +277,7 @@
 int32_t pg_device_count(void);
 size_t pg_eval_workspace_bytes(const pg_eval_args *args);
 int32_t pg_gene_count(const pg_net *net);
+int32_t pg_eval_vary_records(const pg_eval_args *args, pg_vary_records *out);
 
 int32_t pg_eval_population(const pg_eval_args *args, void *stream);
 int32_t pg_forward(const pg_forward_args *args, void *stream);
diff --git a/neuro-genetic-pong-self-play_amd/csrc/pg_eval.hpp b/neuro-genetic-pong-self-play_amd/csrc/pg_eval.hpp
--- a/neuro-genetic-pong-self-play_amd/csrc/pg_eval.hpp
+++ b/neuro-genetic-pong-self-play_amd/csrc/pg_eval.hpp
@@ -42,6 +42,7 @@
   int nodes[PG_MAX_NODES];
   int n_nodes, bias, max_width;
   float *recs;
+  int rec_by_row;
   int horizon;
   int timeout_thresh;
   int win_score;
diff --git a/neuro-genetic-pong-self-play_amd/csrc/pg_service.hpp b/neuro-genetic-pong-self-play_amd/csrc/pg_service.hpp
--- a/neuro-genetic-pong-self-play_amd/csrc/pg_service.hpp
+++ b/neuro-genetic-pong-self-play_amd/csrc/pg_service.hpp
@@ -149,7 +149,12 @@
   }
   NetP<U, O> n;
   load_net_pk<HL, U, O, WT>(n, g, p.nodes[1], p.bias, hl, flip);
-  store_rec<U, O>(n, p.recs + (net * HL + hl) * F);
+  long rec = net;
+  if (p.rec_by_row && net < p.n_genomes) {
+    rec = genome_row(p, (int)net);
+    if (rec < 0 || rec >= p.n_genomes) return;
+  }
+  store_rec<U, O>(n, p.recs + (rec * HL + hl) * F);
 }
 
 #ifdef PG_PROBE_EXTRA
@@ -170,7 +175,7 @@
 }
 #endif
 
-template <int L, int U, int O, typename WT, bool kUntraced = false, bool kHorizon = false>
+template <int L, int U, int O, typename WT, bool kUntraced = false, bool kHorizon = false, bool kByRow = false>
 __global__ __launch_bounds__(svc_threads<U>()) void k_service(EvalParams p) {
   constexpr int kSvcThreads = svc_threads<U>();
   constexpr bool kInline = inline_service<L, U, kHorizon>();
@@ -383,7 +388,7 @@
       const bool nn = side && kind == kOppNN && p.n_opponents > 0;
       const int oj = nn ? min(max(p.opp[w], 0), p.n_opponents - 1) : 0;
       gm = nn ? opponents + (long)oj * p.ostride : gr;
-      const int rec = nn ? p.n_genomes + oj : i;
+      const int rec = nn ? p.n_genomes + oj : (kByRow ? genome_row(p, i) : i);
       load_rec<U, O>(net, p.recs + ((long)rec * HL + hl) * rec_floats<U, O>());
       const int sx = slot_me();
       if (kInline && hl == 0) slots[sx].rec = rec;
@@ -836,7 +841,14 @@
     PG_HIP(hipGetLastError());
     return PG_OK;
   }
-  if (kSplitTrace && p.horizon > 0)
+  if (p.rec_by_row) {
+    if constexpr (kSplitTrace) {
+      if (p.trace || p.horizon > 0) return fail(PG_ERR_UNSUPPORTED, "rec_by_row: untraced launches without a horizon only");
+      hipLaunchKernelGGL((k_service<L, U, O, WT, true, false, true>), dim3(grid), dim3(kSvcThreads), lds, s, p);
+    } else {
+      return fail(PG_ERR_UNSUPPORTED, "rec_by_row: [6, 33..64, 3] networks on 8-lane groups only");
+    }
+  } else if (kSplitTrace && p.horizon > 0)
     hipLaunchKernelGGL((k_service<L, U, O, WT, true, true>), dim3(grid), dim3(kSvcThreads), lds, s, p);
   else if (kSplitTrace && !p.trace)
     hipLaunchKernelGGL((k_service<L, U, O, WT, true>), dim3(grid), dim3(kSvcThreads), lds, s, p);
diff --git a/neuro-genetic-pong-self-play_amd/csrc/pong_ga.hip b/neuro-genetic-pong-self-play_amd/csrc/pong_ga.hip
--- a/neuro-genetic-pong-self-play_amd/csrc/pong_ga.hip
+++ b/neuro-genetic-pong-self-play_amd/csrc/pong_ga.hip
@@ -335,24 +335,110 @@
   return (double)(splitmix64(key ^ b) >> 11) * 0x1.0p-53;
 }
 
-template <typename WT>
-__device__ __forceinline__ void vary_pair(const pg_ga_args &a, int pair);
-
-template <typename WT>
-__global__ __launch_bounds__(256) void k_vary(pg_ga_args a) {
+struct VaryRec {
+  float *recs;
+  int row_base, rows;
+  int H, b;
+};
+constexpr int kVaryHL = 4, kVaryU = 16, kVaryO = 3;
+__host__ __device__ constexpr int vary_row_floats(long genes) { return (int)((genes + 3) / 4 * 4); }
+__host__ __device__ constexpr int vary_wave_floats(long genes) {
+  return 2 * vary_row_floats(genes) + 2 * kVaryHL * rec_floats<kVaryU, kVaryO>();
+}
+
+template <int HL, int U, int O>
+__device__ __forceinline__ void rec_from_lds(const float *g, int H, int b, int hl, int p, int lane, float *r) {
+  constexpr int P = NetP<U, O>::P;
+  constexpr int F = rec_floats<U, O>();
+  static_assert(2 * HL * P == 64 && U == 2 * P, "one lane per (pair, child, lane record)");
+  constexpr float kScaleX = -1.4426950408889634f / 320.f;
+  constexpr float kScaleB = -1.4426950408889634f;
+  const int cols = 6 + b;
+  const int off2 = H * cols;
+  float rs[2], aw[2][O], t[2][O];
+#pragma unroll
+  for (int h = 0; h < 2; ++h) {
+    const int u = 2 * p + h;
+    const int j = hl + HL * u;
+    const bool ok = u < U && j < H;
+    const int jj = ok ? j : 0;
+    float raw[7 + O];
+#pragma unroll
+    for (int i = 0; i < 7; ++i) raw[i] = g[jj * cols + ((i < 6 || b) ? i : 0)];
+#pragma unroll
+    for (int o = 0; o < O; ++o) raw[7 + o] = g[off2 + o * (H + b) + jj];
+    rs[h] = 0.f;
+#pragma unroll
+    for (int i = 0; i < 7; ++i) {
+      const float wf = raw[i] * ((ok && (i < 6 || b)) ? 1.f : 0.f);
+      rs[h] += fabsf(wf);
+      r[(p * 7 + i) * 2 + h] = wf * (i < 6 ? kScaleX : kScaleB);
+    }
+#pragma unroll
+    for (int o = 0; o < O; ++o) {
+      const float w = raw[7 + o] * (ok ? 1.f : 0.f);
+      r[P * 14 + (p * O + o) * 2 + h] = w;
+      aw[h][o] = fabsf(w);
+      t[h][o] = fabsf(w) * (3.f * rs[h] + 5.f + (float)out_roundings<HL, U>());
+    }
+  }
+  float acc[O];
+  float big = 0.f;
+#pragma unroll
+  for (int o = 0; o < O; ++o) acc[o] = 0.f;
+  const int lane0 = lane & (2 * HL - 1);
+#pragma unroll
+  for (int q = 0; q < P; ++q) {
+#pragma unroll
+    for (int h = 0; h < 2; ++h) {
+      big += __shfl(rs[h], lane0 + 2 * HL * q, 64);
+#pragma unroll
+      for (int o = 0; o < O; ++o) {
+        acc[o] += __shfl(t[h][o], lane0 + 2 * HL * q, 64);
+        big += __shfl(aw[h][o], lane0 + 2 * HL * q, 64);
+      }
+    }
+  }
+  float c[O];
+#pragma unroll
+  for (int o = 0; o < O; ++o) {
+    c[o] = g[off2 + o * (H + b) + (b ? H : 0)] * (b ? 1.f : 0.f);
+    big += fabsf(c[o]);
+  }
+  float e = 0.f;
+#pragma unroll
+  for (int o = 0; o < O; ++o)
+    e = fmaxf(e, 2.f * kU * (group_sum<HL>(acc[o]) + (float)out_roundings<HL, U>() * fabsf(c[o])));
+  e = group_sum<HL>(weights_ok(big) ? 0.f : 1.f) > 0.f ? __builtin_inff() : e;
+  if (p == 0) {
+#pragma unroll
+    for (int o = 0; o < O; ++o) r[P * 14 + P * O * 2 + o] = c[o];
+    r[P * 14 + P * O * 2 + O] = e;
+#pragma unroll
+    for (int f = P * 14 + P * O * 2 + O + 1; f < F; ++f) r[f] = 0.f;
+  }
+}
+
+template <typename WT, bool kRec>
+__device__ __forceinline__ void vary_pair(const pg_ga_args &a, const VaryRec &vr, int pair);
+
+template <typename WT, bool kRec = false>
+__global__ __launch_bounds__(256) void k_vary(pg_ga_args a, VaryRec vr) {
   const int wave = (int)blockIdx.x * 4 + __builtin_amdgcn_readfirstlane((int)(threadIdx.x >> 6));
-  if (a.pair_list) {
+  if (!kRec && a.pair_list) {
     const int count = __builtin_amdgcn_readfirstlane(*a.pair_count);
     const int waves = (int)gridDim.x * 4;
 #pragma unroll 1
-    for (int w = wave; w < count; w += waves) vary_pair<WT>(a, __builtin_amdgcn_readfirstlane(a.pair_list[w]));
+    for (int w = wave; w < count; w += waves)
+      vary_pair<WT, false>(a, vr, __builtin_amdgcn_readfirstlane(a.pair_list[w]));
     return;
   }
-  vary_pair<WT>(a, wave);
-}
-
-template <typename WT>
-__device__ __forceinline__ void vary_pair(const pg_ga_args &a, int pair) {
+  vary_pair<WT, kRec>(a, vr, wave);
+}
+
+template <typename WT, bool kRec>
+__device__ __forceinline__ void vary_pair(const pg_ga_args &a, const VaryRec &vr, int pair) {
+  extern __shared__ __attribute__((aligned(16))) float vary_lds[];
   const int pairs = (a.n + 1) / 2;
   if (pair >= pairs) return;
   const int lane = threadIdx.x & 63;
@@ -373,6 +459,8 @@
   const WT *p2 = (const WT *)a.parents + (long)(has1 ? a.chosen[i1] : a.chosen[i0]) * a.stride;
   WT *o1 = (WT *)a.offspring + (long)i0 * a.stride;
   WT *o2 = (WT *)a.offspring + (long)i1 * a.stride;
+  const int row_floats = vary_row_floats(a.genes);
+  float *stage = vary_lds + (kRec ? (int)(threadIdx.x >> 6) * vary_wave_floats(a.genes) : 0);
   const auto one = [&](long gene, double x1, double x2) {
     if (cx) {
       const double u = rng_u01(k3, (uint64_t)gene);
@@ -397,6 +485,10 @@
     }
     o1[gene] = (WT)x1;
     if (has1) o2[gene] = (WT)x2;
+    if constexpr (kRec) {
+      stage[gene] = (float)(WT)x1;
+      stage[row_floats + gene] = (float)(WT)x2;
+    }
   };
   constexpr int kVaryChunk = 4;
   for (long g0 = 0; g0 < a.genes; g0 += 128 * kVaryChunk) {
@@ -418,6 +510,23 @@
         const long g = g0 + c * 128 + h * 64 + lane;
         if (g < a.genes) one(g, x[c][h][0], x[c][h][1]);
       }
+    }
+  }
+  if constexpr (kRec) {
+    constexpr int kRecFloats = kVaryHL * rec_floats<kVaryU, kVaryO>();
+    float *img = stage + 2 * row_floats;
+    wave_lds_sync();
+    const int c = (lane >> 2) & 1, hl = lane & (kVaryHL - 1);
+    rec_from_lds<kVaryHL, kVaryU, kVaryO>(stage + c * row_floats, vr.H, vr.b, hl, lane >> 3, lane,
+                                          img + (c * kVaryHL + hl) * rec_floats<kVaryU, kVaryO>());
+    wave_lds_sync();
+#pragma unroll
+    for (int k = 0; k < 2; ++k) {
+      const int row = i0 + k - vr.row_base;
+      if ((k == 1 && !has1) || row < 0 || row >= vr.rows) continue;
+      const float4 *src = reinterpret_cast<const float4 *>(img + k * kRecFloats);
+      float4 *dst = reinterpret_cast<float4 *>(vr.recs + (long)row * kRecFloats);
+      for (int q = lane; q < kRecFloats / 4; q += 64) dst[q] = src[q];
     }
   }
 }
@@ -675,6 +784,35 @@
   if (kernel == PG_KERNEL_SPLIT) n += split_records_bytes(a);
   if (kernel == PG_KERNEL_WIDE && wide_shape_ok(a->net, a->n_games)) n += (wide_workspace_bytes(a) + 255) / 256 * 256;
   return n;
+}
+
+int32_t pg_eval_vary_records(const pg_eval_args *a, pg_vary_records *out) {
+  if (!a || !out) return fail(PG_ERR_INVALID, "args or out is NULL");
+  int32_t rc = check_struct_size(a);
+  if (rc != PG_OK) return rc;
+  if (out->struct_size != sizeof(pg_vary_records))
+    return fail(PG_ERR_INVALID, "pg_vary_records.struct_size=%u, this library's struct is %zu bytes (ABI %d)",
+                out->struct_size, sizeof(pg_vary_records), PG_ABI_VERSION);
+  rc = check_net(a->net, true);
+  if (rc != PG_OK) return rc;
+  if (a->n_genomes < 0 || a->n_games < 1) return fail(PG_ERR_INVALID, "n_genomes < 0 or n_games < 1");
+  const int H = a->net.n_nodes == 3 ? a->net.nodes[1] : 0;
+  const int L = a->group_lanes > 0 ? a->group_lanes : choose_split_lanes(H);
+  if (resolve_kernel(a) != PG_KERNEL_SPLIT || !resident_shape_ok(a->net) || a->precision != PG_PREC_CERTIFIED ||
+      L != 2 * kVaryHL || service_units(L, H) != kVaryU || a->net.nodes[2] != kVaryO || a->trace || a->horizon > 0)
+    return fail(PG_ERR_UNSUPPORTED, "no fused records: a variation writes lane records only for the split kernel's "
+                                    "[6, 33..64, 3] layout on 8-lane groups (untraced, no horizon)");
+  out->hidden = H;
+  out->bias = a->net.bias ? 1 : 0;
+  out->lanes = kVaryHL;
+  out->units = kVaryU;
+  out->outputs = kVaryO;
+  out->rec_floats = rec_floats<kVaryU, kVaryO>();
+  out->row_base = 0;
+  out->rows = a->n_genomes;
+  out->offset = eval_base_workspace(a);
+  out->recs = a->workspace ? (float *)((char *)a->workspace + out->offset) : nullptr;
+  return PG_OK;
 }
 
 int32_t pg_gene_count(const pg_net *net) {
@@ -757,6 +895,7 @@
   p.max_width = max_width(a->net);
 
   p.prep = a->prep;
+  p.rec_by_row = a->rec_by_row ? 1 : 0;
   p.horizon = a->horizon;
   p.timeout_thresh = a->timeout_thresh > 0 ? a->timeout_thresh : kTimeoutThresh;
   p.win_score = a->win_score > 0 ? (a->win_score < kDoneScore ? a->win_score : kDoneScore) : kWinScore;
@@ -988,10 +1127,40 @@
   if (a->pair_list && waves > kListWaves) waves = kListWaves;
   if (waves == 0) return PG_OK;
   const dim3 grid((unsigned)((waves + 3) / 4));
+  VaryRec vr;
+  memset(&vr, 0, sizeof(vr));
+  if (a->records && !a->pair_list) {
+    const pg_vary_records *r = a->records;
+    if (r->struct_size != sizeof(pg_vary_records))
+      return fail(PG_ERR_INVALID, "pg_vary_records.struct_size=%u, this library's struct is %zu bytes (ABI %d)",
+                  r->struct_size, sizeof(pg_vary_records), PG_ABI_VERSION);
+    if (r->lanes != kVaryHL || r->units != kVaryU || r->outputs != kVaryO ||
+        r->rec_floats != rec_floats<kVaryU, kVaryO>() || service_units(2 * kVaryHL, r->hidden) != kVaryU)
+      return fail(PG_ERR_UNSUPPORTED, "varAnd: no fused records for lanes=%d units=%d outputs=%d hidden=%d", r->lanes,
+                  r->units, r->outputs, r->hidden);
+    const int b = r->bias ? 1 : 0;
+    if (a->genes != (int64_t)(6 + b) * r->hidden + (int64_t)(r->hidden + b) * kVaryO)
+      return fail(PG_ERR_INVALID, "varAnd: records of a [6, %d, %d] network need its gene count, not genes=%lld", r->hidden,
+                  kVaryO, (long long)a->genes);
+    if (!r->recs || r->rows < 0 || ((uintptr_t)r->recs & 15))
+      return fail(PG_ERR_INVALID, "varAnd: records need a 16-byte aligned region and rows >= 0");
+    vr.recs = r->recs;
+    vr.row_base = r->row_base;
+    vr.rows = r->rows;
+    vr.H = r->hidden;
+    vr.b = b;
+    const size_t lds = 4 * (size_t)vary_wave_floats(a->genes) * sizeof(float);
+    if (a->dtype == PG_F64)
+      hipLaunchKernelGGL((k_vary<double, true>), grid, dim3(256), lds, (hipStream_t)stream, *a, vr);
+    else
+      hipLaunchKernelGGL((k_vary<float, true>), grid, dim3(256), lds, (hipStream_t)stream, *a, vr);
+    PG_HIP(hipGetLastError());
+    return PG_OK;
+  }
   if (a->dtype == PG_F64)
-    hipLaunchKernelGGL(k_vary<double>, grid, dim3(256), 0, (hipStream_t)stream, *a);
+    hipLaunchKernelGGL((k_vary<double, false>), grid, dim3(256), 0, (hipStream_t)stream, *a, vr);
   else
-    hipLaunchKernelGGL(k_vary<float>, grid, dim3(256), 0, (hipStream_t)stream, *a);
+    hipLaunchKernelGGL((k_vary<float, false>), grid, dim3(256), 0, (hipStream_t)stream, *a, vr);
   PG_HIP(hipGetLastError());
   return PG_OK;
 }
diff --git a/neuro-genetic-pong-self-play_amd/pong_amd/_lib.py b/neuro-genetic-pong-self-play_amd/pong_amd/_lib.py
--- a/neuro-genetic-pong-self-play_amd/pong_amd/_lib.py
+++ b/neuro-genetic-pong-self-play_amd/pong_amd/_lib.py
@@ -10,7 +10,7 @@
 LIB_PATH = os.environ.get("PONG_GA_LIB") or os.path.join(PKG_DIR, LIB_NAME)
 HEADER_PATH = os.path.join(REPO_DIR, "include", "pong_ga.h")
 
-PG_ABI_VERSION = 12
+PG_ABI_VERSION = 13
 PG_MAX_NODES = 9
 
 PG_OK, PG_ERR_INVALID, PG_ERR_HIP, PG_ERR_UNSUPPORTED = 0, -1, -2, -3
@@ -52,11 +52,25 @@
         ("n_active", _vp),
         ("prep", ctypes.c_int32), ("horizon", ctypes.c_int32),
         ("timeout_thresh", ctypes.c_int32), ("win_score", ctypes.c_int32),
+        ("rec_by_row", ctypes.c_int32),
     ]
 
     def __init__(self, *args, **kw):
         super().__init__(*args, **kw)
         self.struct_size = ctypes.sizeof(PgEvalArgs)
+
+
+class PgVaryRecords(ctypes.Structure):
+    _fields_ = [
+        ("struct_size", ctypes.c_uint32),
+        ("hidden", ctypes.c_int32), ("bias", ctypes.c_int32), ("lanes", ctypes.c_int32), ("units", ctypes.c_int32),
+        ("outputs", ctypes.c_int32), ("rec_floats", ctypes.c_int32), ("row_base", ctypes.c_int32),
+        ("rows", ctypes.c_int32), ("offset", ctypes.c_size_t), ("recs", _vp),
+    ]
+
+    def __init__(self, *args, **kw):
+        super().__init__(*args, **kw)
+        self.struct_size = ctypes.sizeof(PgVaryRecords)
 
 
 class PgForwardArgs(ctypes.Structure):
@@ -91,6 +105,7 @@
         ("mu", ctypes.c_double), ("sigma", ctypes.c_double), ("indpb", ctypes.c_double),
         ("seed", ctypes.c_uint64), ("generation", ctypes.c_uint64), ("pair_mask", _vp),
         ("pair_list", _vp), ("pair_count", _vp), ("pair_cap", ctypes.c_int32),
+        ("records", ctypes.POINTER(PgVaryRecords)),
     ]
 
 
@@ -185,6 +200,7 @@
     "pg_device_count": (ctypes.c_int32, []),
     "pg_eval_workspace_bytes": (ctypes.c_size_t, [ctypes.POINTER(PgEvalArgs)]),
     "pg_gene_count": (ctypes.c_int32, [ctypes.POINTER(PgNet)]),
+    "pg_eval_vary_records": (ctypes.c_int32, [ctypes.POINTER(PgEvalArgs), ctypes.POINTER(PgVaryRecords)]),
     "pg_eval_population": (ctypes.c_int32, [ctypes.POINTER(PgEvalArgs), _vp]),
     "pg_forward": (ctypes.c_int32, [ctypes.POINTER(PgForwardArgs), _vp]),
     "pg_decide": (ctypes.c_int32, [ctypes.POINTER(PgDecideArgs), _vp]),
diff --git a/neuro-genetic-pong-self-play_amd/pong_amd/device.py b/neuro-genetic-pong-self-play_amd/pong_amd/device.py
--- a/neuro-genetic-pong-self-play_amd/pong_amd/device.py
+++ b/neuro-genetic-pong-self-play_amd/pong_amd/device.py
@@ -84,6 +84,7 @@
         self.net = L.make_net(self.nodes, self.bias, DTYPES[dtype])
         self._ws = None
         self._prep_key = self._prep_ws = None
+        self._rec_key = self._rec_ws = None
 
     def selfplay_schedule(self, n: int, n_opponents: int, offset: int = 0):
         dev = self.device
@@ -105,7 +106,8 @@
                  out: Optional[EvalResult] = None, precision: Optional[str] = None,
                  kernel: Optional[str] = None, group_lanes: Optional[int] = None, validate: bool = True,
                  hard_log: Optional[torch.Tensor] = None, rows: Optional[torch.Tensor] = None,
-                 n_active: Optional[torch.Tensor] = None, prep: str = "all", horizon: Optional[int] = None):
+                 n_active: Optional[torch.Tensor] = None, prep: str = "all", horizon: Optional[int] = None,
+                 rec_by_row: bool = False):
         dev = self.device
         n = genomes.shape[0] if rows is None else rows.shape[0]
         games = self.n_games
@@ -172,7 +174,14 @@
                 raise ValueError("hard_log must be [cap, 8] int32")
             a.hard_log, a.hard_cap = _ptr(hard_log), hard_log.shape[0]
         a.prep = PREPS[prep]
-        if prep == "rest" and n and self._prep_key != self._prep_of(genomes, rows, n_active, n):
+        by_row = bool(rec_by_row)
+        if by_row:
+            a.rec_by_row = 1
+        if prep == "rest" and n and by_row:
+            if self._rec_key != self._rec_of(genomes, 0, n):
+                raise ValueError("prep='rest' with rec_by_row needs the records of a variation into these genome "
+                                 "rows (vary_records with the same rows on this evaluator)")
+        elif prep == "rest" and n and self._prep_key != self._prep_of(genomes, rows, n_active, n):
             raise ValueError("prep='rest' needs a preceding prep='genomes' call with the same genomes, rows, "
                              "n_active and row count on this evaluator")
         a.horizon = self.horizon if horizon is None else int(horizon)
@@ -181,13 +190,55 @@
         a.group_lanes = self.group_lanes if group_lanes is None else int(group_lanes)
         ws = self._workspace(a)
         a.workspace, a.workspace_bytes = _ptr(ws), ws.numel()
-        if prep == "rest" and n and self._prep_ws != ws.data_ptr():
+        if prep == "rest" and n and (self._rec_ws if by_row else self._prep_ws) != ws.data_ptr():
             raise ValueError("prep='rest': the workspace holding the genome records was reallocated")
         with torch.cuda.device(dev):
             L.check("pg_eval_population", L.lib().pg_eval_population(ctypes.byref(a), _stream(dev)))
-        self._prep_key = self._prep_of(genomes, rows, n_active, n) if prep == "genomes" else None
-        self._prep_ws = ws.data_ptr() if prep == "genomes" else None
+        self._prep_key = self._prep_of(genomes, rows, n_active, n) if prep == "genomes" and not by_row else None
+        self._prep_ws = ws.data_ptr() if prep == "genomes" and not by_row else None
+        self._rec_key = self._rec_ws = None
         return out, trace
+
+    @staticmethod
+    def _rec_of(genomes, row_base, n):
+        return (genomes.data_ptr() + int(row_base) * genomes.stride(0) * genomes.element_size(), genomes.stride(0), int(n))
+
+    def _records_args(self, n: int, n_opponents: int) -> L.PgEvalArgs:
+        a = L.PgEvalArgs()
+        a.net = self.net
+        a.n_genomes, a.n_games = int(n), self.n_games
+        if n_opponents > 0:
+            a.opponents, a.n_opponents = 1, int(n_opponents)
+        a.precision = PRECISIONS[self.precision]
+        a.kernel = KERNELS[self.kernel]
+        a.group_lanes = self.group_lanes
+        a.horizon = self.horizon
+        return a
+
+    def vary_records(self, genomes: torch.Tensor, n: int, row_base: int = 0, n_opponents: int = 0):
+        a = self._records_args(n, n_opponents)
+        r = L.PgVaryRecords()
+        rc = L.lib().pg_eval_vary_records(ctypes.byref(a), ctypes.byref(r))
+        if rc == L.PG_ERR_UNSUPPORTED or n <= 0:
+            return None
+        L.check("pg_eval_vary_records", rc)
+        ws = self._workspace(a)
+        r.recs = ws.data_ptr() + r.offset
+        r.row_base, r.rows = int(row_base), int(n)
+        self._rec_key, self._rec_ws = self._rec_of(genomes, row_base, n), ws.data_ptr()
+        self._prep_key = self._prep_ws = None
+        return r
+
+    def has_records(self, genomes: torch.Tensor, n: int, row_base: int = 0) -> bool:
+        return (self._rec_key is not None and self._rec_key == self._rec_of(genomes, row_base, n)
+                and self._ws is not None and self._rec_ws == self._ws.data_ptr())
+
+    def records_region(self, n: int, n_opponents: int = 0) -> torch.Tensor:
+        a = self._records_args(n, n_opponents)
+        r = L.PgVaryRecords()
+        L.check("pg_eval_vary_records", L.lib().pg_eval_vary_records(ctypes.byref(a), ctypes.byref(r)))
+        ws = self._workspace(a)
+        return ws[r.offset:r.offset + n * r.lanes * r.rec_floats * 4]
 
     @staticmethod
     def _prep_of(genomes, rows, n_active, n):
@@ -326,7 +377,7 @@
 def vary(parents: torch.Tensor, chosen: torch.Tensor, genes: int, cxpb: float, mutpb: float, alpha: float,
          mu: float, sigma: float, indpb: float, seed: int, generation: int, out: Optional[torch.Tensor] = None,
          pair_mask: Optional[torch.Tensor] = None, invalid: Optional[torch.Tensor] = None,
-         pair_list: Optional[tuple] = None):
+         pair_list: Optional[tuple] = None, records=None):
     dev = parents.device
     n = chosen.shape[0]
     _need(chosen, "chosen", torch.int32, dev, (n,))
@@ -349,6 +400,8 @@
         _need(lst, "pair_list", torch.int32, dev)
         _need(cnt, "pair_count", torch.int32, dev, (1,))
         a.pair_list, a.pair_count, a.pair_cap = _ptr(lst), _ptr(cnt), int(min(cap, lst.numel()))
+    if records is not None:
+        a.records = ctypes.pointer(records)
     if out.stride(0) != parents.stride(0):
         raise ValueError("offspring and parents must share the row stride")
     with torch.cuda.device(dev):
diff --git a/neuro-genetic-pong-self-play_amd/pong_amd/evolve.py b/neuro-genetic-pong-self-play_amd/pong_amd/evolve.py
--- a/neuro-genetic-pong-self-play_amd/pong_amd/evolve.py
+++ b/neuro-genetic-pong-self-play_amd/pong_amd/evolve.py
@@ -1,5 +1,6 @@
 from __future__ import annotations
 
+import os
 from typing import Optional
 
 import numpy as np
@@ -75,6 +76,7 @@
         self._t_mark = self._t_sub = 0.0
         self._next = None
         self.early_prep = True
+        self.vary_records = os.environ.get("PG_NO_VARY_RECORDS") != "1"
         self.hard_log = None
         self.on_evaluate = None
         self.order_by_length = True
@@ -494,10 +496,15 @@
             prev = self._dealt.get((g - 1) & 1)
             self._complete(g - 1, parents, store[self.H:], chosen, "parents",
                            exclude=cand_pairs if prev is None else (cand_pairs | prev))
+        off = store[self.H:]
+        rec = None
+        if self.vary_records and not self._balanced() and self.hi > self.lo:
+            rec = self.ev.vary_records(off, self.hi - self.lo, self.lo, n_opponents=self.H)
         _, inv = D.vary(parents, chosen, self.G, self.cxpb, self.mutpb, self.alpha, self.mu, self.sigma, self.indpb,
-                        seed=self.seed, generation=g, out=store[self.H:],
+                        seed=self.seed, generation=g, out=off,
                         pair_mask=self._shard_mask() if self._sharded() else None,
-                        invalid=self._buf("invalid%d" % (g & 1), self.P, torch.uint8) if self.persistent_bufs else None)
+                        invalid=self._buf("invalid%d" % (g & 1), self.P, torch.uint8) if self.persistent_bufs else None,
+                        records=rec)
         inherited = self._buf("inherited", self.P, torch.float64)
         D.inherit(chosen, fitness, inherited, self.lineage_frames, self._lineage_alt)
         self.lineage_frames, self._lineage_alt = self._lineage_alt, self.lineage_frames
@@ -507,15 +514,17 @@
                 self._dealt[g & 1] = self._complete(g, store[self.H:], parents, order[0], "dealt%d" % (g & 1))
         else:
             order = self._order(inv, g)
-        self._next = (g, inv, inherited, order, self._early_prep(g, store[self.H:], order))
-
-    def _early_prep(self, g: int, off: torch.Tensor, order):
+        self._next = (g, inv, inherited, order, self._early_prep(g, off, order, records=rec is not None))
+
+    def _early_prep(self, g: int, off: torch.Tensor, order, records: bool = False):
         n = self._n_eval
         if (not self.early_prep or self.schedule != "selfplay" or self.H == 0 or self.hof_n != self.H or self.last is None
                 or self.last.fitness.shape[0] != n):
             return None
         local, count = order
         sched = self.eval_schedule(g, n_hof=self.H, rows=local, out=self._sched_bufs(g, n))
+        if records:
+            return sched
         opponents = self._hall_buf[: self.H] if self._in_place() else self._opponents(self.spare, self.H)
         if self._in_place() and self._sliced(self.H):
             opponents = self._hall_buf[self._slice:self.H:self.hof_slices]
@@ -543,9 +552,18 @@
         out = self.last if (self.last is not None and self.last.fitness.shape[0] == n) else None
         if self.eval_events is not None:
             self.eval_events[0].record()
-        res, _ = self.ev.evaluate(rows, kind, opp, mult, opponents=opponents, out=out, validate=False,
-                                  hard_log=self.hard_log, rows=local, n_active=count,
-                                  prep="all" if sched is None else "rest")
+        by_row = not self._balanced() and self.ev.has_records(rows, n, lo)
+        if by_row:
+            shard_rows, shard_local = rows[lo:hi], local
+            if lo:
+                shard_local = torch.sub(local, lo, out=self._buf("local_rel%d" % (g & 1), n, torch.int32))
+            res, _ = self.ev.evaluate(shard_rows, kind, opp, mult, opponents=opponents, out=out, validate=False,
+                                      hard_log=self.hard_log, rows=shard_local, n_active=count, prep="rest",
+                                      rec_by_row=True)
+        else:
+            res, _ = self.ev.evaluate(rows, kind, opp, mult, opponents=opponents, out=out, validate=False,
+                                      hard_log=self.hard_log, rows=local, n_active=count,
+                                      prep="all" if sched is None else "rest")
         if self.eval_events is not None:
             self.eval_events[1].record()
         self.last, self.last_rows, self.last_count = res, local, count
```

Result: no change. 13.21 billion (median of 6 runs) (+0.8%).
